# APRIL-ZJU/Gaussian-LIC

Measured on AMD Instinct MI355X. Metric: rendered views/sec (fwd+bwd) at 1080p, 2M Gaussians, higher is better.
Workload: dtype f32; 1 GPU; BASELINE config 3: 2000000 Gaussians (random scene, seed 0), 1920x1080, SH degree 3, render fwd + 0.8*L1+0.2*(1-fused-SSIM) + bwd + sparse Adam per view (fused entry points: activations and loss inside the kernels); learning rates x0.01 (stationary synthetic scene); map rows kept in Morton order by the library (bit-identical results; `insertion_order` beside it with --extras); mode=train, parallelism=single, math=strict, map_order=morton, binning=atomic (auto)

## Files before the change

gaussian-lic_amd/_lib.py:

```python
import ctypes
import os

import torch

_HERE = os.path.dirname(os.path.abspath(__file__))
LIB_PATH = os.environ.get("GSLIC_HIP_LIB") or os.path.join(_HERE, "libgslic_hip.so")

ALLOC_FN = ctypes.CFUNCTYPE(ctypes.c_void_p, ctypes.c_void_p, ctypes.c_size_t)


class RasterParams(ctypes.Structure):
    _fields_ = [("P", ctypes.c_int32), ("D", ctypes.c_int32), ("M", ctypes.c_int32), ("width", ctypes.c_int32),
                ("height", ctypes.c_int32), ("tan_fovx", ctypes.c_float), ("tan_fovy", ctypes.c_float),
                ("limx_neg", ctypes.c_float), ("limx_pos", ctypes.c_float), ("limy_neg", ctypes.c_float),
                ("limy_pos", ctypes.c_float), ("scale_modifier", ctypes.c_float), ("prefiltered", ctypes.c_int32),
                ("debug", ctypes.c_int32), ("no_color", ctypes.c_int32), ("raw_params", ctypes.c_int32), ("tie_rank", ctypes.c_void_p)]


class AdamGroup(ctypes.Structure):
    _fields_ = [("param", ctypes.c_void_p), ("grad", ctypes.c_void_p), ("exp_avg", ctypes.c_void_p),
                ("exp_avg_sq", ctypes.c_void_p), ("lr", ctypes.c_float), ("M", ctypes.c_uint32)]


class AdamFused(ctypes.Structure):
    _fields_ = [("param", ctypes.c_void_p * 6), ("exp_avg", ctypes.c_void_p * 6), ("exp_avg_sq", ctypes.c_void_p * 6),
                ("lr", ctypes.c_float * 6), ("b1", ctypes.c_float), ("b2", ctypes.c_float), ("eps", ctypes.c_float), ("visible_out", ctypes.c_void_p)]


EXPORTS = [
    "gslic_rasterize_forward", "gslic_rasterize_backward", "gslic_rasterize_backward_adam", "gslic_rasterize_backward_camera", "gslic_adam_update", "gslic_adam_update_groups",
    "gslic_fusedssim_forward", "gslic_fusedssim_backward", "gslic_knn_mean_dist2", "gslic_abi_version",
    "gslic_last_error", "gslic_geom_bytes", "gslic_img_bytes", "gslic_binning_bytes", "gslic_sample_bytes",
    "gslic_profile_enable", "gslic_profile_reset", "gslic_profile_collect", "gslic_profile_num_kernels",
    "gslic_profile_kernel_name", "gslic_profile_get", "gslic_debug_export", "gslic_extend_select", "gslic_extend_emit", "gslic_loss_partials_count", "gslic_l1_ssim_loss_forward", "gslic_l1_ssim_loss_forward_backward",
    "gslic_l1_ssim_loss_backward", "gslic_set_math_mode", "gslic_set_binning_mode", "gslic_rasterize_forward_capacity", "gslic_rasterize_backward_rgb",
    "gslic_rasterize_backward_rgb_rows", "gslic_sh_grad_from_rgb", "gslic_sh_grad_from_rgb_adam", "gslic_rasterize_backward_rgb_payload",
    "gslic_sh_grad_from_rgb_adam_all", "gslic_get_binning_path", "gslic_scratch_round_up",
    "gslic_rasterize_forward_depth", "gslic_rasterize_backward_depth",
    "gslic_rasterize_forward_depth_capacity", "gslic_rasterize_backward_depth_adam", "gslic_depth_l1_loss_partials_count",
    "gslic_depth_l1_loss_forward_backward", "gslic_img_bytes_depth", "gslic_binning_bytes_depth", "gslic_sample_bytes_depth",
    "gslic_rasterize_backward_depth_camera",
]

_lib = None


class GslicError(RuntimeError):
    pass


def lib():
    global _lib
    if _lib is not None:
        return _lib
    if not os.path.exists(LIB_PATH):
        raise GslicError(f"{LIB_PATH} is missing: run `python gaussian-lic_amd/build.py` (hipcc, gfx950). "
                         "There is no CPU fallback.")
    L = ctypes.CDLL(LIB_PATH, mode=ctypes.RTLD_GLOBAL)
    vp, i32, f32, u32 = ctypes.c_void_p, ctypes.c_int32, ctypes.c_float, ctypes.c_uint32
    L.gslic_last_error.restype = ctypes.c_char_p
    L.gslic_profile_kernel_name.restype = ctypes.c_char_p
    L.gslic_profile_kernel_name.argtypes = [i32]
    L.gslic_profile_get.argtypes = [i32, ctypes.POINTER(ctypes.c_double), ctypes.POINTER(ctypes.c_int64)]
    for n in ("gslic_geom_bytes", "gslic_img_bytes", "gslic_binning_bytes", "gslic_sample_bytes", "gslic_img_bytes_depth", "gslic_binning_bytes_depth",
              "gslic_sample_bytes_depth"):
        getattr(L, n).restype = ctypes.c_size_t
    L.gslic_geom_bytes.argtypes = [i32]
    L.gslic_img_bytes.argtypes = [i32, i32]
    L.gslic_binning_bytes.argtypes = [i32, i32]
    L.gslic_sample_bytes.argtypes = [i32]
    L.gslic_img_bytes_depth.argtypes = [i32, i32]
    L.gslic_binning_bytes_depth.argtypes = [i32]
    L.gslic_sample_bytes_depth.argtypes = [i32]
    L.gslic_rasterize_forward_depth_capacity.argtypes = (
        [ctypes.POINTER(RasterParams)] + [vp, ctypes.c_size_t] * 4 + [vp] * 12 + [vp, vp, vp, vp] +
        [ctypes.POINTER(i32), ctypes.POINTER(i32), vp, vp])
    L.gslic_rasterize_backward_depth_adam.argtypes = (
        [ctypes.POINTER(RasterParams), i32, i32] + [vp] * 12 + [vp] * 4 + [vp, vp] + [vp] * 6 + [f32, ctypes.POINTER(AdamFused), vp])
    L.gslic_depth_l1_loss_partials_count.restype = ctypes.c_int64
    L.gslic_depth_l1_loss_partials_count.argtypes = [i32, i32]
    L.gslic_depth_l1_loss_forward_backward.argtypes = [i32, i32, f32, vp, vp, vp, vp, vp, vp]
    L.gslic_rasterize_forward.argtypes = (
        [ctypes.POINTER(RasterParams)] + [ALLOC_FN, vp] * 4 + [vp] * 12 + [vp, vp, vp] +
        [ctypes.POINTER(i32), ctypes.POINTER(i32), vp])
    L.gslic_rasterize_forward_capacity.argtypes = (
        [ctypes.POINTER(RasterParams)] + [vp, ctypes.c_size_t] * 4 + [vp] * 12 + [vp, vp, vp] +
        [ctypes.POINTER(i32), ctypes.POINTER(i32), vp, vp])
    L.gslic_rasterize_backward.argtypes = (
        [ctypes.POINTER(RasterParams), i32, i32] + [vp] * 12 + [vp] * 4 + [vp] + [vp] * 10 + [f32, vp])
    L.gslic_rasterize_forward_depth.argtypes = (
        [ctypes.POINTER(RasterParams)] + [ALLOC_FN, vp] * 4 + [vp] * 12 + [vp, vp, vp, vp] +
        [ctypes.POINTER(i32), ctypes.POINTER(i32), vp])
    L.gslic_rasterize_backward_depth.argtypes = (
        [ctypes.POINTER(RasterParams), i32, i32] + [vp] * 12 + [vp] * 4 + [vp, vp] + [vp] * 10 + [f32, vp])
    L.gslic_rasterize_backward_adam.argtypes = (
        [ctypes.POINTER(RasterParams), i32, i32] + [vp] * 12 + [vp] * 4 + [vp] + [vp] * 6 + [f32, ctypes.POINTER(AdamFused), vp])
    L.gslic_rasterize_backward_camera.argtypes = (
        [ctypes.POINTER(RasterParams), i32, i32] + [vp] * 12 + [vp] * 4 + [vp] + [vp] * 10 + [f32, vp, vp, vp, vp])
    L.gslic_rasterize_backward_depth_camera.argtypes = (
        [ctypes.POINTER(RasterParams), i32, i32] + [vp] * 12 + [vp] * 4 + [vp, vp] + [vp] * 10 + [f32, vp, vp, vp, vp])
    L.gslic_rasterize_backward_rgb.argtypes = (
        [ctypes.POINTER(RasterParams), i32, i32] + [vp] * 12 + [vp] * 4 + [vp] + [vp] * 5 + [f32, vp])
    L.gslic_rasterize_backward_rgb_rows.argtypes = (
        [ctypes.POINTER(RasterParams), i32, i32] + [vp] * 12 + [vp] * 4 + [vp] + [vp] * 5 + [f32, i32, i32, i32, vp])
    L.gslic_rasterize_backward_rgb_payload.argtypes = (
        [ctypes.POINTER(RasterParams), i32, i32] + [vp] * 12 + [vp] * 4 + [vp] + [vp] * 5 + [f32, vp, vp, vp])
    L.gslic_sh_grad_from_rgb_adam_all.argtypes = [i32, i32, i32, i32, vp, vp, vp, i32, vp, ctypes.c_int64, vp, ctypes.POINTER(AdamFused), vp, vp, vp, vp,
                                                  ctypes.c_int64, vp]
    L.gslic_sh_grad_from_rgb.argtypes = [i32, i32, i32, i32, vp, vp, vp, i32, vp, vp, ctypes.c_int64, vp]
    L.gslic_sh_grad_from_rgb_adam.argtypes = [i32, i32, i32, i32, vp, vp, vp, i32, vp, ctypes.POINTER(AdamFused), vp, vp, ctypes.c_int64, vp]
    L.gslic_adam_update.argtypes = [vp, vp, vp, vp, vp, f32, f32, f32, f32, u32, u32, vp]
    L.gslic_adam_update_groups.argtypes = [ctypes.POINTER(AdamGroup), i32, vp, f32, f32, f32, u32, vp]
    L.gslic_fusedssim_forward.argtypes = [i32, i32, i32, i32, f32, f32] + [vp] * 6 + [vp]
    L.gslic_fusedssim_backward.argtypes = [i32, i32, i32, i32, f32, f32] + [vp] * 7 + [vp]
    L.gslic_knn_mean_dist2.argtypes = [i32, vp, vp, ALLOC_FN, vp, vp]
    L.gslic_extend_select.argtypes = [i32, vp, vp, vp, vp, f32, f32, f32, f32, i32, i32, vp, ALLOC_FN, vp,
                                      ctypes.POINTER(vp), ctypes.POINTER(vp), ctypes.POINTER(i32), vp]
    L.gslic_extend_emit.argtypes = [i32, vp, vp, vp, vp, vp, f32, f32, i32, vp, vp, vp, vp, vp, vp, vp]
    L.gslic_debug_export.argtypes = [ctypes.POINTER(RasterParams), i32, i32] + [vp] * 4 + [vp] * 10 + [vp]
    L.gslic_loss_partials_count.restype = ctypes.c_int64
    L.gslic_loss_partials_count.argtypes = [i32, i32, i32, i32]
    L.gslic_l1_ssim_loss_forward.argtypes = [i32, i32, i32, i32, f32, f32] + [vp] * 7 + [vp]
    L.gslic_l1_ssim_loss_backward.argtypes = [i32, i32, i32, i32, f32] + [vp] * 6 + [vp]
    L.gslic_l1_ssim_loss_forward_backward.argtypes = [i32, i32, i32, i32, f32, f32, f32] + [vp] * 8 + [vp]
    L.gslic_set_math_mode.argtypes = [i32]
    L.gslic_set_binning_mode.argtypes = [i32]
    L.gslic_get_binning_path.argtypes = [ctypes.POINTER(u32), ctypes.POINTER(u32)]
    L.gslic_scratch_round_up.restype = ctypes.c_size_t
    L.gslic_scratch_round_up.argtypes = [ctypes.c_size_t]
    if L.gslic_abi_version() != 8:
        raise GslicError("libgslic_hip.so ABI version mismatch")
    _lib = L
    return L


def set_math_mode(strict):
    return bool(lib().gslic_set_math_mode(int(bool(strict))))


def set_binning_mode(mode):
    names = ("auto", "radix", "atomic")
    return names[lib().gslic_set_binning_mode(names.index(mode))]


def binning_path():
    a, n = ctypes.c_uint32(0), ctypes.c_uint32(0)
    path = lib().gslic_get_binning_path(ctypes.byref(a), ctypes.byref(n))
    return ("none", "radix", "atomic")[path], a.value, n.value


def check(rc):
    if rc != 0:
        raise GslicError(f"libgslic_hip error {rc}: {lib().gslic_last_error().decode()}")


def ptr(t):
    if t is None or t.numel() == 0:
        return None
    return ctypes.c_void_p(t.data_ptr())


def current_stream_ptr():
    return ctypes.c_void_p(torch.cuda.current_stream().cuda_stream)


class _AllocBox:
    __slots__ = ("device", "tensor", "__weakref__")

    def __init__(self, device):
        self.device = device
        self.tensor = torch.empty(0, dtype=torch.uint8, device=device)


class TensorAllocator:

    GRANULE = 32 << 20

    def __init__(self, device):
        box = self._box = _AllocBox(device)
        round_up = lib().gslic_scratch_round_up

        def _alloc(_ctx, nbytes):
            box.tensor = torch.empty(int(round_up(int(nbytes))), dtype=torch.uint8, device=box.device)
            return box.tensor.data_ptr()

        self.cb = ALLOC_FN(_alloc)

    @property
    def device(self):
        return self._box.device

    @property
    def tensor(self):
        return self._box.tensor


def profile_enable(on=True, only=None):
    L = lib()
    if not on:
        check(L.gslic_profile_enable(0))
        return
    if only is None:
        check(L.gslic_profile_enable(1))
        return
    names = [L.gslic_profile_kernel_name(i).decode() for i in range(L.gslic_profile_num_kernels())]
    mask = 0
    for n in only:
        mask |= 1 << names.index(n)
    check(L.gslic_profile_enable(mask if mask not in (0, 1) else (mask | (1 << 30))))


def profile_reset():
    check(lib().gslic_profile_reset())


def profile_collect():
    L = lib()
    check(L.gslic_profile_collect())
    out = {}
    for i in range(L.gslic_profile_num_kernels()):
        ms, n = ctypes.c_double(0), ctypes.c_int64(0)
        check(L.gslic_profile_get(i, ctypes.byref(ms), ctypes.byref(n)))
        if n.value:
            out[L.gslic_profile_kernel_name(i).decode()] = (ms.value, n.value)
    return out
# ... 1 lines not shown
```

gaussian-lic_amd/build.py:

```python
import os
import subprocess
import sys
from concurrent.futures import ThreadPoolExecutor

HERE = os.path.dirname(os.path.abspath(__file__))
CSRC = os.path.join(HERE, "csrc")
OBJ = os.path.join(CSRC, "build")
LIB = os.path.join(HERE, "libgslic_hip.so")
HIPCC = os.environ.get("HIPCC", "/opt/rocm/bin/hipcc")
ARCH = "gfx950"

SOURCES = {
    "api.hip": [],
    "scan.hip": [],
    "radix_sort.hip": [],
    "tile_bin.hip": [],
    "preprocess.hip": ["-ffp-contract=off"],
    "render.hip": ["-fno-slp-vectorize"],
    "render_bwd_scan.hip": ["-fno-slp-vectorize"],
    "preprocess_bwd.hip": [],
    "adam.hip": [],
    "ssim.hip": ["-ffp-contract=off"],
    "depth_loss.hip": [],
    "knn.hip": [],
    "extend.hip": ["-ffp-contract=off"],
}
COMMON = [f"--offload-arch={ARCH}", "-O3", "-std=c++17", "-fPIC", "-fno-fast-math", "-Wno-inline-asm",
          "-fhip-fp32-correctly-rounded-divide-sqrt", "-Wall", "-Wno-unused-function"]
HEADERS = ["gslic_common.h", "kernels.h", "render_fwd_body.inc", "preprocess_bwd_body.inc", os.path.join("..", "..", "include", "gslic_hip.h")]


def _newer(a, b):
    return (not os.path.exists(b)) or os.path.getmtime(a) > os.path.getmtime(b)


def build(force=False, verbose=False):
    global OBJ, LIB
    extra_all = os.environ.get("GSLIC_BUILD_EXTRA", "").split()
    if os.environ.get("GSLIC_BUILD_LIB"):
        LIB = os.path.abspath(os.environ["GSLIC_BUILD_LIB"])
        OBJ = os.path.join(CSRC, "build_" + os.path.splitext(os.path.basename(LIB))[0])
        force = True
    os.makedirs(OBJ, exist_ok=True)
    hdr_paths = [os.path.join(CSRC, h) for h in HEADERS] + [os.path.abspath(__file__)]
    jobs = []
    for src, extra in SOURCES.items():
        s = os.path.join(CSRC, src)
        o = os.path.join(OBJ, src.replace(".hip", ".o"))
        if force or _newer(s, o) or any(_newer(h, o) for h in hdr_paths):
            jobs.append((s, o, [HIPCC] + COMMON + extra + extra_all + ["-c", s, "-o", o]))

    def run(job):
        s, o, cmd = job
        if verbose:
            print(" ".join(cmd), flush=True)
        r = subprocess.run(cmd, capture_output=True, text=True)
        return s, r

    with ThreadPoolExecutor(max_workers=min(8, max(1, len(jobs)))) as ex:
        for s, r in ex.map(run, jobs):
            if r.returncode != 0:
                sys.stderr.write(r.stdout + r.stderr)
                raise RuntimeError(f"hipcc failed on {s}")
            if verbose and r.stderr.strip():
                sys.stderr.write(r.stderr)
    objs = [os.path.join(OBJ, s.replace(".hip", ".o")) for s in SOURCES]
    if force or jobs or not os.path.exists(LIB):
        cmd = [HIPCC, f"--offload-arch={ARCH}", "-shared", "-fPIC", "-o", LIB] + objs
        if verbose:
            print(" ".join(cmd), flush=True)
        r = subprocess.run(cmd, capture_output=True, text=True)
        if r.returncode != 0:
            sys.stderr.write(r.stdout + r.stderr)
            raise RuntimeError("link of libgslic_hip.so failed")
    return LIB


if __name__ == "__main__":
    print(build(force="--force" in sys.argv, verbose="--verbose" in sys.argv))
```

gaussian-lic_amd/csrc/api.hip:

```cpp
#include "gslic_common.h"
#include "kernels.h"
#include <atomic>
#include <chrono>
#include <mutex>

#include <stdarg.h>
#include <stdio.h>
#include <stdlib.h>
#include <string.h>
#include <vector>

namespace gslic {

static thread_local char g_err[512] = "";
int set_error(int code, const char* fmt, ...)
{
    va_list ap;
    va_start(ap, fmt);
    vsnprintf(g_err, sizeof(g_err), fmt, ap);
    va_end(ap);
    return code;
}

bool g_prof_on = false;
int g_strict_math = [] {
    const char* s = getenv("GSLIC_STRICT_MATH");
    if (s) return atoi(s) != 0 ? 1 : 0;
    const char* f = getenv("GSLIC_FAST_MATH");
    return (f && atoi(f) != 0) ? 0 : 1;
}();
static uint32_t g_prof_mask = 0xffffffffu;
static bool g_prof_cur_on = false;
static const char* const k_names[K_COUNT] = {
    "preprocess", "scan_reduce", "scan_spine", "scan_apply", "keybuild", "sort_hist", "sort_scatter", "finalize_lists",
    "bucket_count", "render_fwd", "render_bwd", "preprocess_bwd", "adam", "ssim_fwd", "ssim_bwd", "knn_minmax", "knn_morton",
    "knn_boxes", "knn_search", "debug_export", "extend", "dsort_hist", "dsort_scatter", "sh_grad_from_rgb", "tile_lsort", "tile_hist", "tile_bin", "tile_scan", "tile_lsort_long", "depth_loss"};
uint32_t g_lds_pad[K_COUNT] = {0};
static const bool g_lds_pad_parsed = [] {
    const char* e = getenv("GSLIC_LDS_PAD");
    while (e && *e) {
        const char* eq = strchr(e, '=');
        if (!eq) break;
        for (int k = 0; k < K_COUNT; k++)
            if (strlen(k_names[k]) == (size_t)(eq - e) && strncmp(k_names[k], e, (size_t)(eq - e)) == 0) g_lds_pad[k] = (uint32_t)atoi(eq + 1);
        const char* c = strchr(eq, ',');
        e = c ? c + 1 : nullptr;
    }
    return true;
}();
struct ProfRec { int id; hipEvent_t a, b; };
static std::vector<ProfRec> g_pending;
static std::vector<hipEvent_t> g_pool;
static double g_total_ms[K_COUNT];
static int64_t g_launches[K_COUNT];
static hipEvent_t g_cur = nullptr;

static hipEvent_t ev_get()
{
    if (!g_pool.empty()) { hipEvent_t e = g_pool.back(); g_pool.pop_back(); return e; }
    hipEvent_t e = nullptr;
    (void)hipEventCreate(&e);
    return e;
}
void prof_begin(int id, hipStream_t s)
{
    g_prof_cur_on = (g_prof_mask >> id) & 1u;
    if (!g_prof_cur_on) return;
    g_cur = ev_get();
    (void)hipEventRecord(g_cur, s);
}
void prof_end(int id, hipStream_t s)
{
    if (!g_prof_cur_on) return;
    hipEvent_t b = ev_get();
    (void)hipEventRecord(b, s);
    g_pending.push_back({id, g_cur, b});
    g_cur = nullptr;
}

GeomState GeomState::carve(const void* base, size_t P, size_t* bytes)
{
    Carver c(base);
    GeomState g;
    g.rec = c.take<float4>(GS_REC_F4 * P);
    g.tiles_touched = c.take<uint32_t>(P);
    g.cam_scratch = c.take<float>(128 * ((P + 255) / 256) + 64);
    g.point_offsets = c.take<uint32_t>(P);
    g.gauss_start = c.take<uint32_t>(P);
    g.flags = c.take<uint32_t>(64);
    g.scan_state = c.take<char>(scan_state_bytes(P));
    g.zero_bytes = 64 * sizeof(uint32_t) + scan_state_bytes(P);
    if (bytes) *bytes = c.used(base) + 256;
    return g;
}
ImageState ImageState::carve(const void* base, size_t T, size_t* bytes, bool depth)
{
    Carver c(base);
    ImageState g;
    g.ranges = c.take<uint2>(T);
    g.bucket_offsets = c.take<uint32_t>(T);
    g.max_contrib = c.take<uint32_t>(T);
    g.pix_final = c.take<float4>(T * GS_TILE_PIX);
    g.pix_depth = depth ? c.take<float>(T * GS_TILE_PIX) : nullptr;
    if (bytes) *bytes = c.used(base) + 256;
    return g;
}
BinningState BinningState::carve(const void* base, size_t R, int end_bit, bool no_color, size_t* bytes, bool depth)
{
    Carver c(base);
    BinningState g;
    g.plan = sort_plan(R, end_bit);
    for (int i = 0; i < 2; i++) {
        g.tile_keys[i] = c.take<uint32_t>(R);
        g.slots[i] = c.take<uint32_t>(R);
        g.gauss[i] = c.take<uint32_t>(R);
    }
    g.sort_scratch = c.take<char>(sort_scratch_bytes(g.plan));
    g.partials = no_color ? nullptr : c.take<float>((size_t)GS_PROW * R);
    g.dead = no_color ? nullptr : c.take<uint8_t>(R);
    uint32_t* const ls = no_color ? c.take<uint32_t>(4 * R) : reinterpret_cast<uint32_t*>(g.partials);
    for (int i = 0; i < 4; i++) g.lsort[i] = ls + (size_t)i * R;
    g.partials_z = depth ? c.take<float>(R) : nullptr;
    if (bytes) *bytes = c.used(base) + 256;
    return g;
}
SampleState SampleState::carve(const void* base, size_t B, size_t* bytes, bool depth)
{
    Carver c(base);
    SampleState g;
    g.bucket_to_tile = c.take<uint32_t>(B);
    g.ckpt = c.take<float4>(B * GS_TILE_PIX);
    g.hit = c.take<uint64_t>(B * GS_TILE_PIX);
    g.ckpt_depth = depth ? c.take<float>(B * GS_TILE_PIX) : nullptr;
    if (bytes) *bytes = c.used(base) + 256;
    return g;
}

struct Mailbox {
    volatile uint32_t* host = nullptr;
    uint32_t* dev = nullptr;
    uint32_t seq = 0;
};
static constexpr int kMaxDevices = 16;
struct MailboxSet {
    Mailbox box[kMaxDevices];
    ~MailboxSet()
    {
        for (auto& m : box)
            if (m.host) (void)hipHostFree(const_cast<uint32_t*>(m.host));
    }
};
static thread_local MailboxSet t_mbox;
static uint32_t* g_status_word[kMaxDevices];
uint32_t* device_status_word()
{
    int dev = 0;
    if (hipGetDevice(&dev) != hipSuccess || dev < 0 || dev >= kMaxDevices) return nullptr;
    uint32_t* w = __atomic_load_n(&g_status_word[dev], __ATOMIC_ACQUIRE);
    if (w) return w;
    void* p = nullptr;
    if (hipMalloc(&p, 256) != hipSuccess || !p) { (void)hipGetLastError(); return nullptr; }
    (void)hipMemset(p, 0, 256);
    uint32_t* expected = nullptr;
    if (!__atomic_compare_exchange_n(&g_status_word[dev], &expected, static_cast<uint32_t*>(p), false, __ATOMIC_ACQ_REL, __ATOMIC_ACQUIRE)) {
        (void)hipFree(p);
        return expected;
    }
    return static_cast<uint32_t*>(p);
}
__global__ void publish_kernel(const uint32_t* __restrict__ v0, const uint32_t* __restrict__ v1, const uint32_t* __restrict__ v2, uint32_t* status,
                               uint32_t* box, uint32_t seq)
{
    const uint32_t st = status ? atomicExch(status, 0u) : 0u;
    __hip_atomic_store(box + 0, v0 ? *v0 : 0u, __ATOMIC_RELAXED, __HIP_MEMORY_SCOPE_SYSTEM);
// ... 328 lines not shown
        t_last_path = use_bin ? GSLIC_BINNING_PATH_ATOMIC : GSLIC_BINNING_PATH_RADIX;
        t_last_sample[0] = t_last_sample[1] = 0u;
        const int pp = bin.plan.passes & 1;
        KeybuildArgs ka;
        ka.P = P; ka.gx = gx; ka.gy = gy; ka.rec = geom.rec; ka.order = nullptr; ka.offsets = geom.point_offsets;
        ka.gauss_start = geom.gauss_start; ka.cap = R; ka.status = geom.flags;
        ka.tile_keys = bin.tile_keys[0];
        ka.gauss = use_bin ? bin.gauss[pp] : bin.gauss[0];
        ka.depth = use_bin ? bin.slots[pp] : bin.lsort[0];
        GS_TRY(launch_keybuild(ka, s));
        DEBUG_SYNC(prm, s);
        TileDepthSortArgs ts;
        ts.T = T; ts.ranges = img.ranges; ts.tie_rank = prm->tie_rank; ts.status = geom.flags; ts.long_tiles = img.bucket_offsets;
        ts.gauss_out = bin.gauss[pp ^ 1]; ts.slot_out = bin.slots[pp ^ 1];
        if (use_bin) {
            TileBinArgs tb;
            tb.T = T; tb.n_cap = R; tb.n_dev = R_dev; tb.tile = ka.tile_keys; tb.gid = ka.gauss; tb.depth = ka.depth; tb.tie_rank = prm->tie_rank;
            tb.ranges = img.ranges; tb.binned = bin.binned(); tb.dead = bin.dead; tb.status = geom.flags;
            tb.bucket_offsets = no_color ? nullptr : img.bucket_offsets; tb.max_contrib = img.max_contrib;
            ts.long_tiles = reinterpret_cast<uint32_t*>(bin.sort_scratch);
            GS_TRY(launch_tile_bin(tb, s));
            DEBUG_SYNC(prm, s);
            ts.binned = bin.binned(); ts.depth = nullptr; ts.gauss_in = nullptr; ts.slot_in = nullptr;
            ts.key_a = bin.tile_keys[0]; ts.key_b = bin.tile_keys[1]; ts.idx_a = bin.gauss[pp]; ts.idx_b = bin.slots[pp];
        } else {
            SortBuffers sb;
            for (int i = 0; i < 2; i++) { sb.keys[i] = bin.tile_keys[i]; sb.v0[i] = bin.slots[i]; sb.v1[i] = bin.gauss[i]; sb.v2[i] = bin.lsort[i]; }
            sb.v0_identity = true;
            GS_TRY(radix_sort_u32(sb, bin.plan, bin.sort_scratch, (onesweep_mask() & 2) != 0, K_SORT_HIST, K_SORT_SCATTER, s, R_dev, geom.flags + GS_FLAG_FAULT));
            DEBUG_SYNC(prm, s);
            GS_TRY(launch_finalize_ranges(R, R_dev, bin.tile_keys[pp], img.ranges, bin.dead, s));
            DEBUG_SYNC(prm, s);
            ts.binned = nullptr; ts.depth = bin.lsort[pp]; ts.gauss_in = bin.gauss[pp]; ts.slot_in = bin.slots[pp];
            ts.key_a = bin.lsort[pp ^ 1]; ts.key_b = bin.tile_keys[pp ^ 1]; ts.idx_a = bin.lsort[2]; ts.idx_b = bin.lsort[3];
        }
        GS_TRY(launch_tile_depth_sort(ts, s));
        DEBUG_SYNC(prm, s);
    }

    SampleState smp;
    memset(&smp, 0, sizeof(smp));
    uint32_t B = 0;
    if (!no_color) {
        if (!use_bin) GS_TRY(launch_bucket_scan(T, img.ranges, img.bucket_offsets, img.max_contrib, s));
        if (cap) {
            B = capacity_for(cap->sample_bytes, [&](uint32_t b) { size_t n; SampleState::carve(nullptr, (size_t)b, &n, depth); return n; });
        } else {
            uint32_t bin_sample[2] = {0, 0};
            GS_TRY(fetch_counts(img.bucket_offsets + (T - 1), nullptr, hostbuf, s, geom.flags + GS_FLAG_FAULT,
                                use_bin ? geom.flags + GS_FLAG_BIN_ATOMICS : nullptr, bin_sample));
            if (hostbuf[1] & 2u) return set_error(GSLIC_ERR_HIP, "a sort look-back / chained-scan wait timed out (device preempted?): the forward was abandoned");
            B = hostbuf[0];
            binning_feedback(prm->tie_rank != nullptr, use_bin, bin_sample[0], bin_sample[1]);
        }
        size_t smp_bytes;
        SampleState::carve(nullptr, (size_t)B, &smp_bytes, depth);
        char* smp_base = cap ? cap->sample : sample_alloc(sample_ctx, smp_bytes);
        if (!smp_base) return set_error(GSLIC_ERR_ALLOC, "sample allocator returned NULL for %zu bytes", smp_bytes);
        smp = SampleState::carve(align256(smp_base), (size_t)B, nullptr, depth);
    }

    RenderFwdArgs ra;
    ra.W = prm->width; ra.H = prm->height; ra.gx = gx; ra.gy = gy; ra.no_color = prm->no_color;
    ra.ranges = img.ranges; ra.point_list = bin.point_list(); ra.rec = geom.rec; ra.bucket_offsets = img.bucket_offsets;
    ra.bucket_to_tile = smp.bucket_to_tile; ra.ckpt = smp.ckpt; ra.hit = smp.hit; ra.pix_final = img.pix_final; ra.max_contrib = img.max_contrib;
    ra.out_color = out_color; ra.out_final_T = out_final_T; ra.capB = B; ra.status = geom.flags; ra.tail4_from = T;
    ra.out_depth = depth ? out_depth : nullptr; ra.ckpt_depth = smp.ckpt_depth; ra.pix_depth = img.pix_depth;
    GS_TRY(launch_render_fwd(ra, s));
    note_depth(geom.flags, depth);
    DEBUG_SYNC(prm, s);
    if (cap) {
        hipLaunchKernelGGL(forward_status_kernel, dim3(1), dim3(1), 0, s, (const uint32_t*)(geom.point_offsets + (P - 1)),
                           no_color ? (const uint32_t*)nullptr : (const uint32_t*)(img.bucket_offsets + (T - 1)), geom.flags, geom.flags + GS_FLAG_FAULT,
                           cap->status_out);
        GS_HIP(hipGetLastError());
    }

    *num_rendered = (int32_t)R;
    *num_buckets = (int32_t)B;
    return GSLIC_OK;
}

extern "C" {
int gslic_set_binning_mode(int32_t mode)
{
    if (mode < 0 || mode > 2) return g_binning_mode.load(std::memory_order_relaxed);
    const int old = g_binning_mode.exchange(mode, std::memory_order_relaxed);
    g_binning_epoch.fetch_add(1u, std::memory_order_release);
    return old;
}
int gslic_get_binning_path(uint32_t* sampled_atomics, uint32_t* sampled_instances)
{
    if (sampled_atomics) *sampled_atomics = t_last_sample[0];
    if (sampled_instances) *sampled_instances = t_last_sample[1];
    return t_last_path;
}
size_t gslic_scratch_round_up(size_t n)
{
    if (n <= (size_t(1) << 20)) return n;
    size_t g = size_t(32) << 20;
    if (n > (size_t(64) << 20)) {
        size_t p = 1;
        while ((p << 1) <= n && (p << 1) != 0) p <<= 1;
        const size_t half = p >> 1, cap = size_t(256) << 20;
        g = half > cap ? cap : (half > g ? half : g);
    }
    return (n + g - 1) / g * g;
}
int gslic_rasterize_forward(const gslic_raster_params* prm, gslic_alloc_fn geom_alloc, void* geom_ctx, gslic_alloc_fn binning_alloc,
                            void* binning_ctx, gslic_alloc_fn img_alloc, void* img_ctx, gslic_alloc_fn sample_alloc,
                            void* sample_ctx, const float* background, const float* means3D, const float* dc, const float* shs,
                            const float* colors_precomp, const float* opacities, const float* scales, const float* rotations,
                            const float* cov3D_precomp, const float* viewmatrix, const float* projmatrix, const float* cam_pos,
                            float* out_color, float* out_final_T, int32_t* radii, int32_t* num_rendered, int32_t* num_buckets,
                            void* stream)
{
    return rasterize_forward_impl(prm, geom_alloc, geom_ctx, binning_alloc, binning_ctx, img_alloc, img_ctx, sample_alloc, sample_ctx, nullptr,
                                  background, means3D, dc, shs, colors_precomp, opacities, scales, rotations, cov3D_precomp, viewmatrix, projmatrix,
                                  cam_pos, out_color, out_final_T, radii, num_rendered, num_buckets, stream);
}

int gslic_rasterize_forward_depth(const gslic_raster_params* prm, gslic_alloc_fn geom_alloc, void* geom_ctx, gslic_alloc_fn binning_alloc,
                                  void* binning_ctx, gslic_alloc_fn img_alloc, void* img_ctx, gslic_alloc_fn sample_alloc,
                                  void* sample_ctx, const float* background, const float* means3D, const float* dc, const float* shs,
                                  const float* colors_precomp, const float* opacities, const float* scales, const float* rotations,
                                  const float* cov3D_precomp, const float* viewmatrix, const float* projmatrix, const float* cam_pos,
                                  float* out_color, float* out_final_T, float* out_depth, int32_t* radii, int32_t* num_rendered,
                                  int32_t* num_buckets, void* stream)
{
    return rasterize_forward_impl(prm, geom_alloc, geom_ctx, binning_alloc, binning_ctx, img_alloc, img_ctx, sample_alloc, sample_ctx, nullptr,
                                  background, means3D, dc, shs, colors_precomp, opacities, scales, rotations, cov3D_precomp, viewmatrix, projmatrix,
                                  cam_pos, out_color, out_final_T, radii, num_rendered, num_buckets, stream, out_depth, true);
}

int gslic_rasterize_forward_capacity(const gslic_raster_params* prm, char* geom_buffer, size_t geom_bytes, char* binning_buffer,
                                     size_t binning_bytes, char* img_buffer, size_t img_bytes, char* sample_buffer, size_t sample_bytes,
                                     const float* background, const float* means3D, const float* dc, const float* shs,
                                     const float* colors_precomp, const float* opacities, const float* scales, const float* rotations,
                                     const float* cov3D_precomp, const float* viewmatrix, const float* projmatrix, const float* cam_pos,
                                     float* out_color, float* out_final_T, int32_t* radii, int32_t* capacity_R, int32_t* capacity_B,
                                     uint32_t* status, void* stream)
{
    ForwardCapacity cap{geom_buffer, binning_buffer, img_buffer, sample_buffer, geom_bytes, binning_bytes, img_bytes, sample_bytes, status};
    return rasterize_forward_impl(prm, nullptr, nullptr, nullptr, nullptr, nullptr, nullptr, nullptr, nullptr, &cap, background, means3D, dc, shs,
                                  colors_precomp, opacities, scales, rotations, cov3D_precomp, viewmatrix, projmatrix, cam_pos, out_color,
                                  out_final_T, radii, capacity_R, capacity_B, stream);
}

int gslic_rasterize_forward_depth_capacity(const gslic_raster_params* prm, char* geom_buffer, size_t geom_bytes, char* binning_buffer,
                                           size_t binning_bytes, char* img_buffer, size_t img_bytes, char* sample_buffer, size_t sample_bytes,
                                           const float* background, const float* means3D, const float* dc, const float* shs,
                                           const float* colors_precomp, const float* opacities, const float* scales, const float* rotations,
                                           const float* cov3D_precomp, const float* viewmatrix, const float* projmatrix, const float* cam_pos,
                                           float* out_color, float* out_final_T, float* out_depth, int32_t* radii, int32_t* capacity_R,
                                           int32_t* capacity_B, uint32_t* status, void* stream)
{
    ForwardCapacity cap{geom_buffer, binning_buffer, img_buffer, sample_buffer, geom_bytes, binning_bytes, img_bytes, sample_bytes, status};
    return rasterize_forward_impl(prm, nullptr, nullptr, nullptr, nullptr, nullptr, nullptr, nullptr, nullptr, &cap, background, means3D, dc, shs,
                                  colors_precomp, opacities, scales, rotations, cov3D_precomp, viewmatrix, projmatrix, cam_pos, out_color,
                                  out_final_T, radii, capacity_R, capacity_B, stream, out_depth, true);
}

static int rasterize_backward_impl(const gslic_raster_params* prm, int32_t R, int32_t B, const float* background, const float* means3D,
                             const float* dc, const float* shs, const float* colors_precomp, const float* scales,
                             const float* rotations, const float* cov3D_precomp, const float* viewmatrix, const float* projmatrix,
                             const float* cam_pos, const int32_t* radii, char* geom_buffer, char* binning_buffer, char* img_buffer,
                             char* sample_buffer, const float* dL_dpix, float* dL_dmean2D, float* dL_dconic, float* dL_dopacity,
                             float* dL_dcolor, float* dL_dmean3D, float* dL_dcov3D, float* dL_ddc, float* dL_dsh, float* dL_dscale,
                             float* dL_drot, float lambda_erank, const gslic_adam_fused* adam, float* const dL_dcam[3], void* stream,
                             float* dL_drgb = nullptr, int32_t row_begin = 0, int32_t row_end = -1, bool skip_blend = false, uint8_t* vis_out = nullptr,
                             float* campos_out = nullptr, const float* dL_ddepth = nullptr)
{
    (void)background; (void)dc;
    GS_TRY(check_params(prm));
    const int P = prm->P;
    if (P == 0) return GSLIC_OK;
    if (colors_precomp || cov3D_precomp)
        return set_error(GSLIC_ERR_UNSUPPORTED, "colors_precomp / cov3D_precomp are not supported");
    if (prm->no_color) return set_error(GSLIC_ERR_INVALID_ARG, "backward of a no_color forward is undefined (no checkpoints were stored)");
    if (R < 0 || B < 0) return set_error(GSLIC_ERR_INVALID_ARG, "negative R / B");
    if (!means3D || !scales || !rotations || !viewmatrix || !projmatrix || !cam_pos || !radii || !geom_buffer || !binning_buffer ||
        !img_buffer || !sample_buffer || !dL_dpix || (prm->M > 0 && !shs))
        return set_error(GSLIC_ERR_INVALID_ARG, "required tensor pointer is NULL");
    if (!adam && !dL_drgb && (!dL_dopacity || !dL_dmean3D || !dL_ddc || !dL_dscale || !dL_drot || (prm->M > 0 && !dL_dsh)))
        return set_error(GSLIC_ERR_INVALID_ARG, "required gradient output pointer is NULL");
    if (dL_drgb && (adam || dL_ddc || dL_dsh || !dL_dopacity || !dL_dmean3D || !dL_dscale || !dL_drot))
        return set_error(GSLIC_ERR_INVALID_ARG, "dL_drgb mode: dL_ddc / dL_dsh / adam must be NULL, the four other parameter gradients are required");
    if (adam) {
        if (!prm->raw_params) return set_error(GSLIC_ERR_INVALID_ARG, "fused Adam needs raw_params = 1 (it updates the raw parameters)");
        for (int g = 0; g < 6; g++) {
            if (g == 2 && prm->M == 0) continue;
            if (!adam->param[g] || !adam->exp_avg[g] || !adam->exp_avg_sq[g]) return set_error(GSLIC_ERR_INVALID_ARG, "fused Adam: group %d has a NULL pointer", g);
        }
        if (adam->param[0] != means3D || adam->param[4] != scales || adam->param[5] != rotations || (prm->M > 0 && adam->param[2] != shs))
            return set_error(GSLIC_ERR_INVALID_ARG, "fused Adam: param[] must alias the tensors passed as means3D / shs / scales / rotations");
    }
    {
        const int re = row_end < 0 ? P : row_end;
        if (row_begin < 0 || re > P || row_begin > re || (row_begin & 63))
            return set_error(GSLIC_ERR_INVALID_ARG, "row range [%d, %d) of %d Gaussians (row_begin must be a multiple of 64)", row_begin, re, P);
    }
    hipStream_t s = (hipStream_t)stream;
    int gx, gy;
    const int T = tile_grid(prm->width, prm->height, gx, gy);
    const bool depth = dL_ddepth != nullptr;
    GeomState geom = GeomState::carve(align256(geom_buffer), (size_t)P, nullptr);
    if (depth) {
        int known = known_depth(geom.flags);
        if (known < 0) {
            uint32_t depth_flag = 0u;
            GS_HIP(hipMemcpyAsync(&depth_flag, geom.flags + GS_FLAG_DEPTH, sizeof(uint32_t), hipMemcpyDeviceToHost, s));
            GS_HIP(hipStreamSynchronize(s));
            known = depth_flag == 1u ? 1 : 0;
        }
        if (known != 1)
            return set_error(GSLIC_ERR_INVALID_ARG, "depth backward: these buffers come from a forward that rendered no depth (use gslic_rasterize_forward_depth)");
    }
    ImageState img = ImageState::carve(align256(img_buffer), (size_t)T, nullptr, depth);
    BinningState bin = BinningState::carve(align256(binning_buffer), (size_t)R, sort_end_bit(T), false, nullptr, depth);
    SampleState smp = SampleState::carve(align256(sample_buffer), (size_t)B, nullptr, depth);

    RenderBwdArgs rb;
    rb.W = prm->width; rb.H = prm->height; rb.gx = gx; rb.B = B;
    rb.ranges = img.ranges; rb.point_list = bin.point_list(); rb.inst_slot = bin.inst_slot(); rb.rec = geom.rec;
    rb.bucket_offsets = img.bucket_offsets; rb.bucket_to_tile = smp.bucket_to_tile; rb.ckpt = smp.ckpt; rb.hit = smp.hit; rb.pix_final = img.pix_final;
    rb.max_contrib = img.max_contrib; rb.dL_dpix = dL_dpix; rb.partials = bin.partials; rb.dead = bin.dead; rb.status = geom.flags; rb.T = T;
    rb.dL_ddepth = dL_ddepth; rb.ckpt_depth = smp.ckpt_depth; rb.pix_depth = img.pix_depth; rb.partials_z = bin.partials_z;
    if (!skip_blend) GS_TRY(launch_render_bwd(rb, s));
    DEBUG_SYNC(prm, s);

    PreprocessBwdArgs pb;
    pb.P = P; pb.D = prm->D; pb.M = prm->M; pb.W = prm->width; pb.H = prm->height; pb.raw = prm->raw_params;
    pb.row_begin = row_begin; pb.row_end = row_end < 0 ? P : row_end;
    pb.focal_y = prm->height / (2.0f * prm->tan_fovy);
    pb.focal_x = prm->width / (2.0f * prm->tan_fovx);
    pb.limx_neg = prm->limx_neg; pb.limx_pos = prm->limx_pos; pb.limy_neg = prm->limy_neg; pb.limy_pos = prm->limy_pos;
    pb.scale_modifier = prm->scale_modifier; pb.lambda_erank = lambda_erank;
    pb.means = means3D; pb.scales = scales; pb.rots = rotations; pb.dc = dc; pb.shs = shs; pb.view = viewmatrix; pb.proj = projmatrix;
    pb.campos = cam_pos; pb.radii = radii; pb.rec = geom.rec; pb.tiles_touched = geom.tiles_touched; pb.gauss_start = geom.gauss_start; pb.partials = bin.partials; pb.dead = bin.dead;
    pb.dL_dmean2D = dL_dmean2D; pb.dL_dconic = dL_dconic; pb.dL_dopacity = dL_dopacity; pb.dL_dcolor = dL_dcolor;
    pb.dL_dmean3D = dL_dmean3D; pb.dL_dcov3D = dL_dcov3D; pb.dL_ddc = dL_ddc; pb.dL_dsh = dL_dsh; pb.dL_dscale = dL_dscale;
    pb.dL_drot = dL_drot; pb.dL_drgb = dL_drgb;
    memset(&pb.adam, 0, sizeof(pb.adam));
    if (adam) {
        for (int g = 0; g < 6; g++) { pb.adam.p[g] = adam->param[g]; pb.adam.m[g] = adam->exp_avg[g]; pb.adam.v[g] = adam->exp_avg_sq[g]; pb.adam.lr[g] = adam->lr[g]; }
        pb.adam.b1 = adam->b1; pb.adam.b2 = adam->b2; pb.adam.eps = adam->eps; pb.adam.on = 1;
    }
    pb.status = geom.flags;
    pb.cam_partials = nullptr; pb.cam_out = nullptr;
    pb.partials_z = depth ? bin.partials_z : nullptr;
    pb.vis_out = vis_out; pb.campos_out = campos_out;
    if (dL_dcam) {
        pb.cam_partials = geom.cam_scratch;
        pb.cam_out = geom.cam_scratch + 128 * (((size_t)P + 255) / 256);
    }
    GS_TRY(launch_preprocess_bwd(pb, s));
    if (dL_dcam) {
        GS_HIP(hipMemcpyAsync(dL_dcam[0], pb.cam_out, 16 * sizeof(float), hipMemcpyDeviceToDevice, s));
        GS_HIP(hipMemcpyAsync(dL_dcam[1], pb.cam_out + 16, 16 * sizeof(float), hipMemcpyDeviceToDevice, s));
        GS_HIP(hipMemcpyAsync(dL_dcam[2], pb.cam_out + 32, 3 * sizeof(float), hipMemcpyDeviceToDevice, s));
    }
    DEBUG_SYNC(prm, s);
    return GSLIC_OK;
}

int gslic_rasterize_backward(const gslic_raster_params* prm, int32_t R, int32_t B, const float* background, const float* means3D,
                             const float* dc, const float* shs, const float* colors_precomp, const float* scales,
                             const float* rotations, const float* cov3D_precomp, const float* viewmatrix, const float* projmatrix,
                             const float* cam_pos, const int32_t* radii, char* geom_buffer, char* binning_buffer, char* img_buffer,
                             char* sample_buffer, const float* dL_dpix, float* dL_dmean2D, float* dL_dconic, float* dL_dopacity,
                             float* dL_dcolor, float* dL_dmean3D, float* dL_dcov3D, float* dL_ddc, float* dL_dsh, float* dL_dscale,
                             float* dL_drot, float lambda_erank, void* stream)
{
    return rasterize_backward_impl(prm, R, B, background, means3D, dc, shs, colors_precomp, scales, rotations, cov3D_precomp, viewmatrix,
                                   projmatrix, cam_pos, radii, geom_buffer, binning_buffer, img_buffer, sample_buffer, dL_dpix, dL_dmean2D,
                                   dL_dconic, dL_dopacity, dL_dcolor, dL_dmean3D, dL_dcov3D, dL_ddc, dL_dsh, dL_dscale, dL_drot,
                                   lambda_erank, nullptr, nullptr, stream);
}

int gslic_rasterize_backward_depth(const gslic_raster_params* prm, int32_t R, int32_t B, const float* background, const float* means3D,
                                   const float* dc, const float* shs, const float* colors_precomp, const float* scales,
                                   const float* rotations, const float* cov3D_precomp, const float* viewmatrix, const float* projmatrix,
                                   const float* cam_pos, const int32_t* radii, char* geom_buffer, char* binning_buffer, char* img_buffer,
                                   char* sample_buffer, const float* dL_dpix, const float* dL_ddepth, float* dL_dmean2D, float* dL_dconic,
                                   float* dL_dopacity, float* dL_dcolor, float* dL_dmean3D, float* dL_dcov3D, float* dL_ddc, float* dL_dsh,
                                   float* dL_dscale, float* dL_drot, float lambda_erank, void* stream)
{
    GS_TRY(check_params(prm));
    if (prm->P == 0) return GSLIC_OK;
    if (prm->no_color) return set_error(GSLIC_ERR_INVALID_ARG, "depth backward: no_color = 1 (no depth forward renders without colour)");
    if (!dL_ddepth) return set_error(GSLIC_ERR_INVALID_ARG, "depth backward: dL_ddepth is NULL (gslic_rasterize_backward is the colour-only backward)");
    return rasterize_backward_impl(prm, R, B, background, means3D, dc, shs, colors_precomp, scales, rotations, cov3D_precomp, viewmatrix,
                                   projmatrix, cam_pos, radii, geom_buffer, binning_buffer, img_buffer, sample_buffer, dL_dpix, dL_dmean2D,
                                   dL_dconic, dL_dopacity, dL_dcolor, dL_dmean3D, dL_dcov3D, dL_ddc, dL_dsh, dL_dscale, dL_drot,
                                   lambda_erank, nullptr, nullptr, stream, nullptr, 0, -1, false, nullptr, nullptr, dL_ddepth);
}

int gslic_rasterize_backward_rgb(const gslic_raster_params* prm, int32_t R, int32_t B, const float* background, const float* means3D,
                                 const float* dc, const float* shs, const float* colors_precomp, const float* scales,
                                 const float* rotations, const float* cov3D_precomp, const float* viewmatrix, const float* projmatrix,
                                 const float* cam_pos, const int32_t* radii, char* geom_buffer, char* binning_buffer, char* img_buffer,
                                 char* sample_buffer, const float* dL_dpix, float* dL_dopacity, float* dL_dmean3D, float* dL_drgb,
                                 float* dL_dscale, float* dL_drot, float lambda_erank, void* stream)
{
    if (!dL_drgb) return set_error(GSLIC_ERR_INVALID_ARG, "gslic_rasterize_backward_rgb: dL_drgb is NULL");
    return rasterize_backward_impl(prm, R, B, background, means3D, dc, shs, colors_precomp, scales, rotations, cov3D_precomp, viewmatrix,
                                   projmatrix, cam_pos, radii, geom_buffer, binning_buffer, img_buffer, sample_buffer, dL_dpix, nullptr,
                                   nullptr, dL_dopacity, nullptr, dL_dmean3D, nullptr, nullptr, nullptr, dL_dscale, dL_drot, lambda_erank,
                                   nullptr, nullptr, stream, dL_drgb);
}

int gslic_rasterize_backward_rgb_payload(const gslic_raster_params* prm, int32_t R, int32_t B, const float* background, const float* means3D,
                                         const float* dc, const float* shs, const float* colors_precomp, const float* scales,
                                         const float* rotations, const float* cov3D_precomp, const float* viewmatrix, const float* projmatrix,
                                         const float* cam_pos, const int32_t* radii, char* geom_buffer, char* binning_buffer, char* img_buffer,
                                         char* sample_buffer, const float* dL_dpix, float* dL_dopacity, float* dL_dmean3D, float* dL_drgb,
                                         float* dL_dscale, float* dL_drot, float lambda_erank, uint8_t* vis_out, float* campos_out, void* stream)
{
    if (!dL_drgb) return set_error(GSLIC_ERR_INVALID_ARG, "gslic_rasterize_backward_rgb_payload: dL_drgb is NULL");
    return rasterize_backward_impl(prm, R, B, background, means3D, dc, shs, colors_precomp, scales, rotations, cov3D_precomp, viewmatrix,
                                   projmatrix, cam_pos, radii, geom_buffer, binning_buffer, img_buffer, sample_buffer, dL_dpix, nullptr,
                                   nullptr, dL_dopacity, nullptr, dL_dmean3D, nullptr, nullptr, nullptr, dL_dscale, dL_drot, lambda_erank,
                                   nullptr, nullptr, stream, dL_drgb, 0, -1, false, vis_out, campos_out);
}

int gslic_rasterize_backward_rgb_rows(const gslic_raster_params* prm, int32_t R, int32_t B, const float* background, const float* means3D,
                                      const float* dc, const float* shs, const float* colors_precomp, const float* scales,
                                      const float* rotations, const float* cov3D_precomp, const float* viewmatrix, const float* projmatrix,
                                      const float* cam_pos, const int32_t* radii, char* geom_buffer, char* binning_buffer, char* img_buffer,
                                      char* sample_buffer, const float* dL_dpix, float* dL_dopacity, float* dL_dmean3D, float* dL_drgb,
                                      float* dL_dscale, float* dL_drot, float lambda_erank, int32_t row_begin, int32_t row_end, int32_t skip_blend,
                                      void* stream)
{
    if (!dL_drgb) return set_error(GSLIC_ERR_INVALID_ARG, "gslic_rasterize_backward_rgb_rows: dL_drgb is NULL");
// ... 396 lines not shown
```

gaussian-lic_amd/csrc/gslic_common.h:

```cpp
#pragma once
#include <hip/hip_runtime.h>
#include <stdint.h>
#include <stddef.h>
#include "../../include/gslic_hip.h"

#define GS_TILE 16
#define GS_TILE_PIX 256
#ifndef GS_REC_F4
#define GS_REC_F4 3
#endif
#ifndef GS_PROW
#define GS_PROW 9
#endif
#define GS_BUCKET 64
#define GS_WAVE 64

namespace gslic {

int set_error(int code, const char* fmt, ...);
#define GS_HIP(call)                                                                                       \
    do {                                                                                                   \
        hipError_t e__ = (call);                                                                           \
        if (e__ != hipSuccess)                                                                             \
            return ::gslic::set_error(GSLIC_ERR_HIP, "%s: %s (%s:%d)", #call, hipGetErrorString(e__),      \
                                      __FILE__, __LINE__);                                                 \
    } while (0)
#define GS_TRY(expr)                                                                                       \
    do {                                                                                                   \
        int rc__ = (expr);                                                                                 \
        if (rc__ != GSLIC_OK) return rc__;                                                                 \
    } while (0)

enum KernelId {
    K_PREPROCESS = 0,
    K_SCAN_REDUCE,
    K_SCAN_SPINE,
    K_SCAN_APPLY,
    K_KEYBUILD,
    K_SORT_HIST,
    K_SORT_SCATTER,
    K_FINALIZE_LISTS,
    K_BUCKET_COUNT,
    K_RENDER_FWD,
    K_RENDER_BWD,
    K_PREPROCESS_BWD,
    K_ADAM,
    K_SSIM_FWD,
    K_SSIM_BWD,
    K_KNN_MINMAX,
    K_KNN_MORTON,
    K_KNN_BOXES,
    K_KNN_SEARCH,
    K_DEBUG_EXPORT,
    K_EXTEND,
    K_DSORT_HIST,
    K_DSORT_SCATTER,
    K_SH_REBUILD,
    K_TILE_LSORT,
    K_TILE_HIST,
    K_TILE_BIN,
    K_TILE_SCAN,
    K_TILE_LSORT_LONG,
    K_DEPTH_LOSS,
    K_COUNT
};
void prof_begin(int id, hipStream_t s);
void prof_end(int id, hipStream_t s);
extern bool g_prof_on;
#define GS_FLAG_HITBITS 4
#define GS_FLAG_DEPTH 12
#define GS_FLAG_BIN_ATOMICS 10
#define GS_FLAG_LONG 9
#define GS_FLAG_FAULT 8
extern int g_strict_math;

extern uint32_t g_lds_pad[];
#define GS_LAUNCH(id, kernel, grid, block, shmem, stream, ...)                                             \
    do {                                                                                                   \
        if (::gslic::g_prof_on) ::gslic::prof_begin(id, stream);                                           \
        hipLaunchKernelGGL(kernel, grid, block, (shmem) + ::gslic::g_lds_pad[id], stream, __VA_ARGS__);    \
        if (::gslic::g_prof_on) ::gslic::prof_end(id, stream);                                             \
        GS_HIP(hipGetLastError());                                                                         \
    } while (0)

struct Carver {
    uintptr_t p;
    explicit Carver(const void* base) : p(reinterpret_cast<uintptr_t>(base)) {}
    template <typename T>
    T* take(size_t count)
    {
        p = (p + 255) & ~uintptr_t(255);
        T* r = reinterpret_cast<T*>(p);
        p += count * sizeof(T);
        return r;
    }
    size_t used(const void* base) const { return p - reinterpret_cast<uintptr_t>(base); }
};

static inline int div_up(int a, int b) { return (a + b - 1) / b; }
static inline size_t div_up_sz(size_t a, size_t b) { return (a + b - 1) / b; }

static inline uint32_t higher_msb(uint32_t n)
{
    uint32_t bits = 0;
    while (bits < 32 && (n >> bits) != 0) ++bits;
    return bits == 0 ? 1 : bits;
}

uint32_t* device_status_word();

size_t scan_temp_elems(size_t n);
int scan_u32(const uint32_t* in, uint32_t* out, size_t n, bool exclusive, uint32_t* temp, hipStream_t s);
size_t scan_state_bytes(size_t n);
int scan_u32_chained(const uint32_t* in, const uint32_t* gather, uint32_t* out, size_t n, bool exclusive, void* zeroed_state, hipStream_t s,
                     uint32_t* fault = nullptr);

#define GS_SORT_ITEMS 16
#define GS_SORT_BLOCK 256
#define GS_SORT_TILE (GS_SORT_ITEMS * GS_SORT_BLOCK)
struct SortPlan {
    size_t n;
    int passes;
    size_t nblk;
    size_t hist_elems;
};
SortPlan sort_plan(size_t n, int end_bit);
struct SortBuffers {
    uint32_t* keys[2];
    uint32_t* v0[2];
    uint32_t* v1[2];
    uint32_t* v2[2];
    bool v0_identity;
};
size_t sort_scratch_bytes(const SortPlan& plan);
int radix_sort_u32(const SortBuffers& b, const SortPlan& plan, void* scratch, bool onesweep, int id_hist, int id_scatter, hipStream_t s,
                   const uint32_t* n_dev = nullptr, uint32_t* fault = nullptr);
struct TileBinArgs {
    int T;
    uint32_t n_cap;
    const uint32_t* n_dev;
    const uint32_t* tile;
    const uint32_t* gid;
    const uint32_t* depth;
    const uint32_t* tie_rank;
    uint2* ranges;
    uint4* binned;
    uint8_t* dead;
    uint32_t* bucket_offsets;
    uint32_t* max_contrib;
    uint32_t* status;
};
static constexpr int GS_TILE_BIN_MAX_T = 36864;
int launch_tile_bin(const TileBinArgs& a, hipStream_t s);
bool tile_bin_lds_ok(int T);

struct TileDepthSortArgs {
    int T;
    const uint2* ranges;
    const uint4* binned;
    const uint32_t* depth;
    uint32_t* key_a;
    uint32_t* key_b;
    uint32_t* idx_a;
    uint32_t* idx_b;
    const uint32_t* gauss_in;
    const uint32_t* slot_in;
    uint32_t* gauss_out;
    uint32_t* slot_out;
    const uint32_t* tie_rank;
    uint32_t* status;
    uint32_t* long_tiles;
};
int launch_tile_depth_sort(const TileDepthSortArgs& a, hipStream_t s);

struct GeomState {
    float4* rec;
    uint32_t* tiles_touched;
    float* cam_scratch;
    uint32_t* point_offsets;
    uint32_t* gauss_start;
    uint32_t* flags;
    void* scan_state;
    size_t zero_bytes;
    static GeomState carve(const void* base, size_t P, size_t* bytes);
};
struct ImageState {
    uint2* ranges;
    uint32_t* bucket_offsets;
    uint32_t* max_contrib;
    float4* pix_final;
    float* pix_depth;
    static ImageState carve(const void* base, size_t T, size_t* bytes, bool depth = false);
};
struct BinningState {
    uint32_t* tile_keys[2];
    uint32_t* slots[2];
    uint32_t* gauss[2];
    uint32_t* lsort[4];
    void* sort_scratch;
    float* partials;
    uint8_t* dead;
    float* partials_z;
    SortPlan plan;
    uint32_t* point_list() const { return gauss[(plan.passes & 1) ^ 1]; }
    uint32_t* inst_slot() const { return slots[(plan.passes & 1) ^ 1]; }
    uint4* binned() const { return reinterpret_cast<uint4*>(lsort[0]); }
    static BinningState carve(const void* base, size_t R, int end_bit, bool no_color, size_t* bytes, bool depth = false);
};
struct SampleState {
    uint32_t* bucket_to_tile;
    float4* ckpt;
    uint64_t* hit;
    float* ckpt_depth;
    static SampleState carve(const void* base, size_t B, size_t* bytes, bool depth = false);
};

}

#if defined(__HIPCC__)
namespace gslic {

__device__ __forceinline__ int lane_id() { return __builtin_amdgcn_mbcnt_hi(~0u, __builtin_amdgcn_mbcnt_lo(~0u, 0u)); }

__device__ __forceinline__ int tile_pix_x(int i) { return ((i >> 6) & 1) * 8 + (i & 7); }
__device__ __forceinline__ int tile_pix_y(int i) { return (i >> 7) * 8 + ((i >> 3) & 7); }
__device__ __forceinline__ int tile_pix_index(int x, int y) { return ((y >> 3) * 2 + (x >> 3)) * 64 + (y & 7) * 8 + (x & 7); }


__device__ __forceinline__ uint32_t wave_inclusive_scan(uint32_t v)
{
    const int lane = lane_id();
#pragma unroll
    for (int d = 1; d < 64; d <<= 1) {
        uint32_t o = __shfl_up(v, d, 64);
        if (lane >= d) v += o;
    }
    return v;
}
__device__ __forceinline__ uint32_t block256_exclusive_prefix(uint32_t thread_sum, uint32_t& block_total, uint32_t* lds)
{
    const int lane = threadIdx.x & 63, wave = threadIdx.x >> 6;
    const uint32_t inc = wave_inclusive_scan(thread_sum);
    if (lane == 63) lds[wave] = inc;
    __syncthreads();
    uint32_t wave_base = 0, total = 0;
#pragma unroll
    for (int w = 0; w < 4; w++) {
        const uint32_t s = lds[w];
        if (w < wave) wave_base += s;
        total += s;
    }
    __syncthreads();
    block_total = total;
    return wave_base + inc - thread_sum;
}
__device__ __forceinline__ float readlane_f(float v, int l) { return __int_as_float(__builtin_amdgcn_readlane(__float_as_int(v), l)); }
__device__ __forceinline__ uint32_t readlane_u(uint32_t v, int l) { return (uint32_t)__builtin_amdgcn_readlane((int)v, l); }
#ifndef GSLIC_NT
#define GSLIC_NT 1
#endif
typedef float gs_v4f __attribute__((ext_vector_type(4)));
typedef float gs_v4f_u __attribute__((ext_vector_type(4), aligned(4)));
__device__ __forceinline__ float4 ld_stream(const float4* p)
{
#if GSLIC_NT
// ... 97 lines not shown
```

gaussian-lic_amd/csrc/kernels.h:

```cpp
#pragma once
#include "gslic_common.h"

namespace gslic {

struct PreprocessArgs {
    int P, D, M, W, H, gx, gy;
    float focal_x, focal_y;
    float limx_neg, limx_pos, limy_neg, limy_pos, scale_modifier;
    int prefiltered, no_color, raw;
    const float *means, *scales, *rots, *opac, *dc, *shs, *view, *proj, *campos;
    int32_t* radii;
    float4* rec;
    uint32_t* tiles_touched;
    uint32_t* depth_keys;
    uint2* ranges;
    uint32_t* flags;
};
int launch_preprocess(const PreprocessArgs& a, hipStream_t s);

struct KeybuildArgs {
    int P, gx, gy;
    const float4* rec;
    const uint32_t* order;
    const uint32_t* offsets;
// ... 5 lines not shown
    uint32_t* status;
};
int launch_keybuild(const KeybuildArgs& a, hipStream_t s);
int launch_finalize_ranges(uint32_t R, const uint32_t* R_dev, const uint32_t* sorted_tiles, uint2* ranges, uint8_t* dead, hipStream_t s);
int launch_bucket_scan(int T, const uint2* ranges, uint32_t* bucket_offsets, uint32_t* max_contrib , hipStream_t s);

struct RenderFwdArgs {
    int W, H, gx, gy, no_color;
    const uint2* ranges;
    const uint32_t* point_list;
    const float4* rec;
    const uint32_t* bucket_offsets;
    uint32_t* bucket_to_tile;
    float4* ckpt;
    uint64_t* hit;
    float4* pix_final;
    uint32_t* max_contrib;
    float* out_color;
    float* out_final_T;
    uint32_t capB;
    uint32_t* status;
    int tail4_from;
    float* out_depth;
    float* ckpt_depth;
    float* pix_depth;
};
int launch_render_fwd(const RenderFwdArgs& a, hipStream_t s);

struct RenderBwdArgs {
    int W, H, gx, B;
    const uint2* ranges;
    const uint32_t* point_list;
    const uint32_t* inst_slot;
    const float4* rec;
    const uint32_t* bucket_offsets;
    const uint32_t* bucket_to_tile;
    const float4* ckpt;
    const uint64_t* hit;
    const float4* pix_final;
    const uint32_t* max_contrib;
    const float* dL_dpix;
    float* partials;
    uint8_t* dead;
    const uint32_t* status;
    int T;
    int xcd_lg;
    int skip_if_bits;
    const float* dL_ddepth;
    const float* ckpt_depth;
    const float* pix_depth;
    float* partials_z;
};
int launch_render_bwd(const RenderBwdArgs& a, hipStream_t s);
int launch_render_bwd_scan(const RenderBwdArgs& b, unsigned grid, hipStream_t s);

struct AdamFusedArgs {
    float *p[6], *m[6], *v[6];
    float lr[6];
    float b1, b2, eps;
    int on;
};

struct PreprocessBwdArgs {
    int P, D, M, W, H, raw;
    int row_begin, row_end;
    float focal_x, focal_y;
    float limx_neg, limx_pos, limy_neg, limy_pos, scale_modifier, lambda_erank;
    const float *means, *scales, *rots, *dc, *shs, *view, *proj, *campos;
    const int32_t* radii;
    const float4* rec;
    const uint32_t* tiles_touched;
    const uint32_t* gauss_start;
    const float* partials;
    const uint8_t* dead;
    float *dL_dmean2D, *dL_dconic, *dL_dopacity, *dL_dcolor, *dL_dmean3D, *dL_dcov3D, *dL_ddc, *dL_dsh, *dL_dscale, *dL_drot;
    float* dL_drgb;
    AdamFusedArgs adam;
    const uint32_t* status;
    uint8_t* vis_out;
    float* campos_out;
    float* cam_partials;
    float* cam_out;
    const float* partials_z;
};
int launch_preprocess_bwd(const PreprocessBwdArgs& a, hipStream_t s);

struct ShGradFromRgbArgs {
    int P, D, M, n_views, input_is_ddc;
    size_t rgb_stride, campos_stride;
    const float *means3D, *campos_all, *rgb_all;
    float *dL_ddc, *dL_dsh;
    const uint8_t* visible;
    size_t vis_stride;
    uint8_t* vis_out;
    const float* g_small[4];
    AdamFusedArgs adam;
};
int launch_sh_grad_from_rgb(const ShGradFromRgbArgs& a, hipStream_t s);

}
```

gaussian-lic_amd/csrc/preprocess_bwd.hip:

```cpp
#include "gslic_common.h"
#include "kernels.h"
#include <stdlib.h>

namespace gslic {

#define SHC0 0.28209479177387814f
#define SHC1 0.4886025119029199f
__constant__ float b_SH_C2[5] = {1.0925484305920792f, -1.0925484305920792f, 0.31539156525252005f, -1.0925484305920792f,
                                 0.5462742152960396f};
__constant__ float b_SH_C3[7] = {-0.5900435899266435f, 2.890611442640554f, -0.4570457994644658f, 0.3731763325901154f,
                                 -0.4570457994644658f, 1.445305721320277f, -0.5900435899266435f};

__device__ __forceinline__ void sh_dir(float px, float py, float pz, const float* __restrict__ campos, float& dox, float& doy, float& doz, float& x,
                                       float& y, float& z)
{
#pragma clang fp contract(off)
    dox = px - campos[0]; doy = py - campos[1]; doz = pz - campos[2];
    const float len = sqrtf(dox * dox + doy * doy + doz * doz);
    x = dox / len; y = doy / len; z = doz / len;
}

__device__ __forceinline__ void sh_coefs(int D, float x, float y, float z, float (&c)[15])
{
#pragma clang fp contract(off)
#pragma unroll
    for (int k = 0; k < 15; k++) c[k] = 0.f;
    if (D > 0) {
        c[0] = -SHC1 * y; c[1] = SHC1 * z; c[2] = -SHC1 * x;
        if (D > 1) {
            const float xx = x * x, yy = y * y, zz = z * z, xy = x * y, yz = y * z, xz = x * z;
            c[3] = b_SH_C2[0] * xy; c[4] = b_SH_C2[1] * yz; c[5] = b_SH_C2[2] * (2.f * zz - xx - yy);
            c[6] = b_SH_C2[3] * xz; c[7] = b_SH_C2[4] * (xx - yy);
            if (D > 2) {
                c[8] = b_SH_C3[0] * y * (3.f * xx - yy); c[9] = b_SH_C3[1] * xy * z; c[10] = b_SH_C3[2] * y * (4.f * zz - xx - yy);
                c[11] = b_SH_C3[3] * z * (2.f * zz - 3.f * xx - 3.f * yy); c[12] = b_SH_C3[4] * x * (4.f * zz - xx - yy);
                c[13] = b_SH_C3[5] * z * (xx - yy); c[14] = b_SH_C3[6] * x * (xx - 3.f * yy);
            }
        }
    }
}

struct ShOut {
    float x, y, z, dR, dG, dB;
    bool on;
};

struct PartialSums { float mx, my, cx, cy, cw, op, r, g, b; };

__device__ __forceinline__ bool bwd_gather(const PreprocessBwdArgs& a, const int idx, const bool staged, PartialSums& ps);
template <bool CAM, bool DEFER_XYZ = false>
__device__ __forceinline__ void bwd_rest(const PreprocessBwdArgs& a, const int idx, const PartialSums& ps, const float* sh_row, const float* sk_row,
                                         ShOut& so, float* sg, float* cg);

template <int BS, bool DEFER_XYZ = false>
__device__ __forceinline__ void small_groups_sink(const AdamFusedArgs& A, float* const (&gout)[5], const float* lds_g, const uint8_t* lds_vis, int row0,
                                                  int rows)
{
    constexpr int NG = 5;
    constexpr int gid[NG] = {0, 1, 3, 4, 5};
    constexpr int wid[NG] = {3, 3, 1, 3, 4};
    constexpr int off[NG] = {0, 3 * BS, 6 * BS, 7 * BS, 10 * BS};
    const int t = threadIdx.x;
    if (rows == BS) {
        float4 g[NG], p[NG], m[NG], v[NG];
        bool on[NG], vis[NG][4];
#pragma unroll
        for (int k = 0; k < NG; k++) {
            on[k] = false;
            if (t < BS * wid[k] / 4) {
                g[k] = reinterpret_cast<const float4*>(lds_g + off[k])[t];
                if (gout[k]) reinterpret_cast<float4*>(gout[k] + (size_t)row0 * wid[k])[t] = g[k];
                if (A.on && !(DEFER_XYZ && k == 0)) {
                    const int e = 4 * t;
#pragma unroll
                    for (int c = 0; c < 4; c++) vis[k][c] = lds_vis[(e + c) / wid[k]];
                    on[k] = vis[k][0] | vis[k][1] | vis[k][2] | vis[k][3];
                }
            }
            if (on[k]) {
                const size_t base = (size_t)row0 * wid[k];
                p[k] = reinterpret_cast<const float4*>(A.p[gid[k]] + base)[t];
                m[k] = ld_stream(reinterpret_cast<const float4*>(A.m[gid[k]] + base) + t);
                v[k] = ld_stream(reinterpret_cast<const float4*>(A.v[gid[k]] + base) + t);
            }
        }
#pragma unroll
        for (int k = 0; k < NG; k++) {
            if (!on[k]) continue;
            const float lr = A.lr[gid[k]];
            if (vis[k][0]) adam_scalar(p[k].x, g[k].x, m[k].x, v[k].x, lr, A.b1, A.b2, A.eps);
            if (vis[k][1]) adam_scalar(p[k].y, g[k].y, m[k].y, v[k].y, lr, A.b1, A.b2, A.eps);
            if (vis[k][2]) adam_scalar(p[k].z, g[k].z, m[k].z, v[k].z, lr, A.b1, A.b2, A.eps);
            if (vis[k][3]) adam_scalar(p[k].w, g[k].w, m[k].w, v[k].w, lr, A.b1, A.b2, A.eps);
            const size_t base = (size_t)row0 * wid[k];
            st_stream(reinterpret_cast<float4*>(A.p[gid[k]] + base) + t, p[k]);
            st_stream(reinterpret_cast<float4*>(A.m[gid[k]] + base) + t, m[k]);
            st_stream(reinterpret_cast<float4*>(A.v[gid[k]] + base) + t, v[k]);
        }
    } else {
#pragma unroll
        for (int k = 0; k < NG; k++) {
            const size_t base = (size_t)row0 * wid[k];
            for (int i = t; i < rows * wid[k]; i += BS) {
                if (gout[k]) gout[k][base + i] = lds_g[off[k] + i];
                if (A.on && !(DEFER_XYZ && k == 0) && lds_vis[i / wid[k]])
                    adam_scalar(A.p[gid[k]][base + i], lds_g[off[k] + i], A.m[gid[k]][base + i], A.v[gid[k]][base + i], A.lr[gid[k]], A.b1, A.b2, A.eps);
            }
        }
    }
}

#ifndef GS_PBWD_U
#define GS_PBWD_U 4
#endif
#ifndef GS_SHT
#define GS_SHT 19
#endif
static constexpr int SHT = GS_SHT;

__device__ __forceinline__ int div3_small(int rem) { return (rem * 43) >> 7; }

template <int BS>
__device__ __forceinline__ void sh_columns_pass(const PreprocessBwdArgs& a, const float* __restrict__ tab, float* __restrict__ sk,
                                                const uint8_t* __restrict__ lds_vis, const int row0)
{
#pragma clang fp contract(off)
    constexpr int NE = BS * 45, NV = NE / 4, U = GS_PBWD_U;
    const AdamFusedArgs& A = a.adam;
    const size_t base = (size_t)row0 * 45;
    const float* __restrict__ P = a.shs + base;
    const bool store_g = a.dL_dsh != nullptr;
    for (int i0 = threadIdx.x; i0 < NV; i0 += BS * U) {
        float4 x[U], m[U], v[U];
        float2 nx[U];
        int r0[U], rem0[U];
        bool any[U], upd[U], vis[U][4];
#pragma unroll
        for (int u = 0; u < U; u++) {
            const int i = i0 + BS * u;
            any[u] = upd[u] = false;
            if (i < NV) {
                const int e = 4 * i;
                r0[u] = e / 45; rem0[u] = e - 45 * r0[u];
                const int r1 = (r0[u] + 1 < BS) ? r0[u] + 1 : r0[u];
                const bool v0 = lds_vis[r0[u]] != 0, v1 = lds_vis[r1] != 0;
#pragma unroll
                for (int c = 0; c < 4; c++) vis[u][c] = (rem0[u] + c < 45) ? v0 : v1;
                any[u] = v0 | v1;
                upd[u] = A.on & (vis[u][0] | vis[u][3]);
                x[u] = make_float4(0.f, 0.f, 0.f, 0.f); nx[u] = make_float2(0.f, 0.f);
                if (any[u]) {
                    x[u] = reinterpret_cast<const float4*>(P)[i];
                    if (e + 4 < NE) nx[u] = *reinterpret_cast<const float2*>(P + e + 4);
                }
                if (upd[u]) {
                    m[u] = ld_stream(reinterpret_cast<const float4*>(A.m[2] + base) + i);
                    v[u] = ld_stream(reinterpret_cast<const float4*>(A.v[2] + base) + i);
                }
            }
        }
#pragma unroll
        for (int u = 0; u < U; u++) {
            const int i = i0 + BS * u;
            if (i >= NV) continue;
            const float xe[6] = {x[u].x, x[u].y, x[u].z, x[u].w, nx[u].x, nx[u].y};
            float pr[6], g[4];
#pragma unroll
            for (int c = 0; c < 6; c++) {
                int r = r0[u], rem = rem0[u] + c;
                if (rem >= 45) { rem -= 45; r += 1; }
                if (r >= BS) r = BS - 1;
                const int k = div3_small(rem), ch = rem - 3 * k;
                const float d = tab[r * SHT + 15 + ch];
                pr[c] = xe[c] * d;
                if (c < 4) g[c] = tab[r * SHT + k] * d;
            }
            const int ch0 = rem0[u] - 3 * div3_small(rem0[u]);
            const int c0 = ch0 == 0 ? 0 : 3 - ch0;
            const float t0 = c0 == 0 ? pr[0] : (c0 == 1 ? pr[1] : pr[2]);
            const float t1 = c0 == 0 ? pr[1] : (c0 == 1 ? pr[2] : pr[3]);
            const float t2 = c0 == 0 ? pr[2] : (c0 == 1 ? pr[3] : pr[4]);
            const int f = (4 * i + c0) / 3;
            sk[f] = (t0 + t1) + t2;
            if (c0 == 0) sk[f + 1] = (pr[3] + pr[4]) + pr[5];
            const float4 g4 = make_float4(g[0], g[1], g[2], g[3]);
            if (store_g) reinterpret_cast<float4*>(a.dL_dsh + base)[i] = g4;
            if (upd[u]) {
                if (vis[u][0]) adam_scalar(x[u].x, g4.x, m[u].x, v[u].x, A.lr[2], A.b1, A.b2, A.eps);
                if (vis[u][1]) adam_scalar(x[u].y, g4.y, m[u].y, v[u].y, A.lr[2], A.b1, A.b2, A.eps);
                if (vis[u][2]) adam_scalar(x[u].z, g4.z, m[u].z, v[u].z, A.lr[2], A.b1, A.b2, A.eps);
                if (vis[u][3]) adam_scalar(x[u].w, g4.w, m[u].w, v[u].w, A.lr[2], A.b1, A.b2, A.eps);
                st_stream(reinterpret_cast<float4*>(A.p[2] + base) + i, x[u]);
                st_stream(reinterpret_cast<float4*>(A.m[2] + base) + i, m[u]);
                st_stream(reinterpret_cast<float4*>(A.v[2] + base) + i, v[u]);
            }
        }
    }
}

#ifndef GS_PBWD_STRICT_CHAIN
#define GS_PBWD_STRICT_CHAIN 0
#endif
#ifndef GS_PBWD_WPE
#define GS_PBWD_WPE 4
#endif
#define GS_PBWD_OCC __attribute__((amdgpu_waves_per_eu(GS_PBWD_WPE, GS_PBWD_WPE)))
template <bool LDS_SH, int BS, bool CAM>
__global__ __launch_bounds__(BS) GS_PBWD_OCC void preprocess_bwd_kernel(PreprocessBwdArgs a)
{
    constexpr bool DEFER_XYZ = false;
#include "preprocess_bwd_body.inc"
}
template <bool LDS_SH, int BS>
__global__ __launch_bounds__(BS) GS_PBWD_OCC void preprocess_bwd_defer_xyz_kernel(PreprocessBwdArgs a)
{
    constexpr bool CAM = false;
    constexpr bool DEFER_XYZ = true;
#include "preprocess_bwd_body.inc"
}

__device__ __forceinline__ bool bwd_gather(const PreprocessBwdArgs& a, const int idx, const bool staged, PartialSums& ps)
{
    ps.mx = ps.my = ps.cx = ps.cy = ps.cw = ps.op = ps.r = ps.g = ps.b = 0.f;
    const bool visible = a.radii[idx] > 0;

    if (!visible) {
        if (a.dL_dmean2D) { a.dL_dmean2D[3 * idx] = 0; a.dL_dmean2D[3 * idx + 1] = 0; a.dL_dmean2D[3 * idx + 2] = 0; }
        if (a.dL_dconic) reinterpret_cast<float4*>(a.dL_dconic)[idx] = make_float4(0, 0, 0, 0);
        if (a.dL_dcolor) { a.dL_dcolor[3 * idx] = 0; a.dL_dcolor[3 * idx + 1] = 0; a.dL_dcolor[3 * idx + 2] = 0; }
        if (a.dL_dcov3D)
            for (int k = 0; k < 6; k++) a.dL_dcov3D[6 * idx + k] = 0;
        if (staged) return false;
        if (a.dL_dopacity) a.dL_dopacity[idx] = 0;
        if (a.dL_dmean3D) { a.dL_dmean3D[3 * idx] = 0; a.dL_dmean3D[3 * idx + 1] = 0; a.dL_dmean3D[3 * idx + 2] = 0; }
        if (a.dL_ddc) { a.dL_ddc[3 * idx] = 0; a.dL_ddc[3 * idx + 1] = 0; a.dL_ddc[3 * idx + 2] = 0; }
        if (a.dL_drgb) { a.dL_drgb[3 * idx] = 0; a.dL_drgb[3 * idx + 1] = 0; a.dL_drgb[3 * idx + 2] = 0; }
        if (a.dL_dscale) { a.dL_dscale[3 * idx] = 0; a.dL_dscale[3 * idx + 1] = 0; a.dL_dscale[3 * idx + 2] = 0; }
        if (a.dL_drot) reinterpret_cast<float4*>(a.dL_drot)[idx] = make_float4(0, 0, 0, 0);
        return false;
    }

    float s_mx = 0, s_my = 0, s_cx = 0, s_cy = 0, s_cw = 0, s_op = 0, s_r = 0, s_g = 0, s_b = 0;
    {
        const uint32_t u0 = a.gauss_start[idx];
        const uint32_t u1 = u0 + a.tiles_touched[idx];
        constexpr int UP = 4;
        for (uint32_t u = u0; u < u1; u += UP) {
            uint32_t flags;
            __builtin_memcpy(&flags, a.dead + u, 4);
            bool live[UP];
#pragma unroll
            for (int j = 0; j < UP; j++) live[j] = (u + j < u1) & (((flags >> (8 * j)) & 0xffu) == 0u);
            gs_v4f_u q0[UP], q1[UP];
            float q2[UP];
#pragma unroll
            for (int j = 0; j < UP; j++) {
                if (live[j]) {
                    const float* p = a.partials + GS_PROW * (size_t)(u + j);
                    q0[j] = *reinterpret_cast<const gs_v4f_u*>(p);
                    q1[j] = *reinterpret_cast<const gs_v4f_u*>(p + 4);
                    q2[j] = p[8];
                }
            }
#pragma unroll
            for (int j = 0; j < UP; j++) {
                if (live[j]) {
                    s_mx += q0[j].x; s_my += q0[j].y; s_cx += q0[j].z; s_cy += q0[j].w;
                    s_cw += q1[j].x; s_op += q1[j].y; s_r += q1[j].z; s_g += q1[j].w;
                    s_b += q2[j];
                }
            }
        }
    }
    if (a.dL_dmean2D) { a.dL_dmean2D[3 * idx] = s_mx; a.dL_dmean2D[3 * idx + 1] = s_my; a.dL_dmean2D[3 * idx + 2] = 0; }
    if (a.dL_dconic) reinterpret_cast<float4*>(a.dL_dconic)[idx] = make_float4(s_cx, s_cy, 0.f, s_cw);
    if (a.dL_dcolor) { a.dL_dcolor[3 * idx] = s_r; a.dL_dcolor[3 * idx + 1] = s_g; a.dL_dcolor[3 * idx + 2] = s_b; }
    ps.mx = s_mx; ps.my = s_my; ps.cx = s_cx; ps.cy = s_cy; ps.cw = s_cw; ps.op = s_op; ps.r = s_r; ps.g = s_g; ps.b = s_b;
    return true;
}

template <bool CAM, bool DEFER_XYZ>
__device__ __forceinline__ void bwd_rest(const PreprocessBwdArgs& a, const int idx, const PartialSums& ps, const float* sh_row, const float* sk_row,
                                         ShOut& so, float* sg, float* cg)
{
#if GS_PBWD_STRICT_CHAIN
#pragma clang fp contract(off)
#endif
    const float s_mx = ps.mx, s_my = ps.my, s_cx = ps.cx, s_cy = ps.cy, s_cw = ps.cw, s_op = ps.op, s_r = ps.r, s_g = ps.g, s_b = ps.b;
    const float* __restrict__ V = a.view;
    const float* __restrict__ Pm = a.proj;
    const float mx3 = a.means[3 * idx], my3 = a.means[3 * idx + 1], mz3 = a.means[3 * idx + 2];

    float qr = a.rots[4 * idx], qx = a.rots[4 * idx + 1], qy = a.rots[4 * idx + 2], qz = a.rots[4 * idx + 3];
    const float4 qraw = make_float4(qr, qx, qy, qz);
    if (a.raw) {
        const float nrm = fmaxf(sqrtf(qr * qr + qx * qx + qy * qy + qz * qz), 1e-12f);
        qr = qr / nrm; qx = qx / nrm; qy = qy / nrm; qz = qz / nrm;
    }
    float Rm[3][3];
    Rm[0][0] = 1.f - 2.f * (qy * qy + qz * qz); Rm[0][1] = 2.f * (qx * qy - qr * qz); Rm[0][2] = 2.f * (qx * qz + qr * qy);
    Rm[1][0] = 2.f * (qx * qy + qr * qz); Rm[1][1] = 1.f - 2.f * (qx * qx + qz * qz); Rm[1][2] = 2.f * (qy * qz - qr * qx);
    Rm[2][0] = 2.f * (qx * qz - qr * qy); Rm[2][1] = 2.f * (qy * qz + qr * qx); Rm[2][2] = 1.f - 2.f * (qx * qx + qy * qy);
    float sc[3] = {a.scales[3 * idx], a.scales[3 * idx + 1], a.scales[3 * idx + 2]};
    if (a.raw) { sc[0] = expf(sc[0]); sc[1] = expf(sc[1]); sc[2] = expf(sc[2]); }
    const float s[3] = {a.scale_modifier * sc[0], a.scale_modifier * sc[1], a.scale_modifier * sc[2]};
    float Mk[3][3];
#pragma unroll
// ... 294 lines not shown
                                                           const float* __restrict__ V, const uint32_t* __restrict__ status, float* __restrict__ dL_dmean3D,
                                                           AdamFusedArgs A)
{
    if (status[2] != 0u) return;
    const int idx = row_begin + (int)(blockIdx.x * 256u + threadIdx.x);
    if (idx >= row_end || radii[idx] <= 0) return;
    depth_mean3d_row<ADAM>(idx, gauss_start, tiles_touched, dead, partials_z, V, dL_dmean3D, A);
}

__global__ __launch_bounds__(256) void depth_mean3d_cam_kernel(int row_begin, int row_end, const int32_t* __restrict__ radii,
                                                               const uint32_t* __restrict__ gauss_start, const uint32_t* __restrict__ tiles_touched,
                                                               const uint8_t* __restrict__ dead, const float* __restrict__ partials_z,
                                                               const float* __restrict__ V, const uint32_t* __restrict__ status, const float* __restrict__ means,
                                                               float* __restrict__ dL_dmean3D, float* __restrict__ cam_partials)
{
#pragma clang fp contract(off)
    if (status[2] != 0u) return;
    const int idx = row_begin + (int)(blockIdx.x * 256u + threadIdx.x);
    float c[4] = {0.f, 0.f, 0.f, 0.f};
    if (idx < row_end && radii[idx] > 0) {
        AdamFusedArgs none;
        none.on = 0;
        const float dz = depth_mean3d_row<false>(idx, gauss_start, tiles_touched, dead, partials_z, V, dL_dmean3D, none);
        c[0] = dz * means[3 * idx]; c[1] = dz * means[3 * idx + 1]; c[2] = dz * means[3 * idx + 2]; c[3] = dz;
    }
#pragma unroll
    for (int k = 0; k < 4; k++) {
        float v = c[k];
#pragma unroll
        for (int d = 32; d >= 1; d >>= 1) v += __shfl_xor(v, d, 64);
        c[k] = v;
    }
    if ((threadIdx.x & 63) == 0) {
        float* row = cam_partials + 32 * ((size_t)blockIdx.x * 4 + (threadIdx.x >> 6));
#pragma unroll
        for (int k = 0; k < 4; k++) row[27 + k] = c[k];
    }
}

__global__ __launch_bounds__(256) void cam_reduce_depth_kernel(size_t rows, const float* __restrict__ partials, const uint32_t* __restrict__ status,
                                                               float* __restrict__ out)
{
    __shared__ float red[256], redz[256];
    if (status[2] != 0u) return;
    const int k = blockIdx.x;
    const bool direct = k < 12 && (k % 3) == 2;
    const int kz = 27 + k / 3;
    float s = 0.f, sz = 0.f;
    for (size_t r = threadIdx.x; r < rows; r += 256) {
        s += partials[32 * r + k];
        if (direct) sz += partials[32 * r + kz];
    }
    red[threadIdx.x] = s;
    redz[threadIdx.x] = sz;
    __syncthreads();
    for (int d = 128; d >= 1; d >>= 1) {
        if ((int)threadIdx.x < d) {
            red[threadIdx.x] += red[threadIdx.x + d];
            redz[threadIdx.x] += redz[threadIdx.x + d];
        }
        __syncthreads();
    }
    if (threadIdx.x == 0) {
        int dst;
        if (k < 12) dst = 4 * (k / 3) + (k % 3);
        else if (k < 24) { const int kk = k - 12; const int r = kk % 3; dst = 16 + 4 * (kk / 3) + (r == 2 ? 3 : r); }
        else dst = 32 + (k - 24);
        out[dst] = direct ? red[0] + redz[0] : red[0];
    }
}

int launch_preprocess_bwd(const PreprocessBwdArgs& a, hipStream_t s)
{
    if (a.partials_z && (a.dL_drgb || !a.dL_dmean3D))
        return set_error(GSLIC_ERR_INVALID_ARG, "depth backward: no dL_drgb output, and dL_dmean3D is required");
    if (a.partials_z && a.cam_partials && (a.adam.on || a.row_begin != 0))
        return set_error(GSLIC_ERR_INVALID_ARG, "depth camera backward: no fused Adam and no row range");
    const bool defer = a.partials_z && a.adam.on;
    const bool cam = a.cam_partials != nullptr;
    const int nrows = a.row_end - a.row_begin;
    if (nrows <= 0) return GSLIC_OK;
    if (cam) GS_HIP(hipMemsetAsync(a.cam_out, 0, 35 * sizeof(float), s));
    if (a.M == 15 && a.shs && (a.dL_dsh || a.adam.on || a.dL_drgb)) {
        if (cam) GS_LAUNCH(K_PREPROCESS_BWD, (preprocess_bwd_kernel<true, 64, true>), dim3(div_up(nrows, 64)), dim3(64), 0, s, a);
        else if (defer) GS_LAUNCH(K_PREPROCESS_BWD, (preprocess_bwd_defer_xyz_kernel<true, 64>), dim3(div_up(nrows, 64)), dim3(64), 0, s, a);
        else GS_LAUNCH(K_PREPROCESS_BWD, (preprocess_bwd_kernel<true, 64, false>), dim3(div_up(nrows, 64)), dim3(64), 0, s, a);
    } else {
        if (cam) GS_LAUNCH(K_PREPROCESS_BWD, (preprocess_bwd_kernel<false, 256, true>), dim3(div_up(nrows, 256)), dim3(256), 0, s, a);
        else if (defer) GS_LAUNCH(K_PREPROCESS_BWD, (preprocess_bwd_defer_xyz_kernel<false, 256>), dim3(div_up(nrows, 256)), dim3(256), 0, s, a);
        else GS_LAUNCH(K_PREPROCESS_BWD, (preprocess_bwd_kernel<false, 256, false>), dim3(div_up(nrows, 256)), dim3(256), 0, s, a);
    }
    if (defer)
        GS_LAUNCH(K_PREPROCESS_BWD, depth_mean3d_kernel<true>, dim3(div_up(nrows, 256)), dim3(256), 0, s, a.row_begin, a.row_end, a.radii, a.gauss_start,
                  a.tiles_touched, a.dead, a.partials_z, a.view, a.status, a.dL_dmean3D, a.adam);
    else if (a.partials_z && cam)
        GS_LAUNCH(K_PREPROCESS_BWD, depth_mean3d_cam_kernel, dim3(div_up(nrows, 256)), dim3(256), 0, s, a.row_begin, a.row_end, a.radii, a.gauss_start,
                  a.tiles_touched, a.dead, a.partials_z, a.view, a.status, a.means, a.dL_dmean3D, a.cam_partials);
    else if (a.partials_z)
        GS_LAUNCH(K_PREPROCESS_BWD, depth_mean3d_kernel<false>, dim3(div_up(nrows, 256)), dim3(256), 0, s, a.row_begin, a.row_end, a.radii, a.gauss_start,
                  a.tiles_touched, a.dead, a.partials_z, a.view, a.status, a.dL_dmean3D, a.adam);
    if (cam) {
        const size_t rows = (a.M == 15 && a.shs && (a.dL_dsh || a.adam.on || a.dL_drgb)) ? (size_t)div_up(a.P, 64) : (size_t)div_up(a.P, 256) * 4;
        if (a.partials_z) GS_LAUNCH(K_PREPROCESS_BWD, cam_reduce_depth_kernel, dim3(27), dim3(256), 0, s, rows, (const float*)a.cam_partials, a.status, a.cam_out);
        else GS_LAUNCH(K_PREPROCESS_BWD, cam_reduce_kernel, dim3(27), dim3(256), 0, s, rows, (const float*)a.cam_partials, a.cam_out);
    }
    return GSLIC_OK;
}

static constexpr int SGR = 32;
template <bool ADAM>
__global__ __launch_bounds__(64) void sh_grad_from_rgb_kernel(ShGradFromRgbArgs a)
{
#pragma clang fp contract(off)
    __shared__ __attribute__((aligned(16))) float lds_rows[SGR * 48];
    const int t = threadIdx.x;
    const int row0 = blockIdx.x * SGR;
    const int idx = t < SGR ? row0 + t : a.P;
    const int rows = (a.P - row0) < SGR ? (a.P - row0) : SGR;
    float acc[45], adc[3] = {0.f, 0.f, 0.f};
#pragma unroll
    for (int k = 0; k < 45; k++) acc[k] = 0.f;
    if (idx < a.P) {
        const float px = a.means3D[3 * (size_t)idx], py = a.means3D[3 * (size_t)idx + 1], pz = a.means3D[3 * (size_t)idx + 2];
        for (int v = 0; v < a.n_views; v++) {
            const float* g = a.rgb_all + (size_t)v * a.rgb_stride + (size_t)idx * 3;
            float d[3] = {g[0], g[1], g[2]};
            if (d[0] == 0.f && d[1] == 0.f && d[2] == 0.f) continue;
            float dc_v[3];
            if (a.input_is_ddc) {
#pragma unroll
                for (int ch = 0; ch < 3; ch++) { dc_v[ch] = d[ch]; d[ch] = d[ch] * (1.0f / SHC0); }
            } else {
#pragma unroll
                for (int ch = 0; ch < 3; ch++) dc_v[ch] = SHC0 * d[ch];
            }
            float dox, doy, doz, x, y, z, c[15];
            sh_dir(px, py, pz, a.campos_all + (size_t)v * a.campos_stride, dox, doy, doz, x, y, z);
            sh_coefs(a.D, x, y, z, c);
#pragma unroll
            for (int ch = 0; ch < 3; ch++) adc[ch] = adc[ch] + dc_v[ch];
#pragma unroll
            for (int k = 0; k < 15; k++) {
#pragma unroll
                for (int ch = 0; ch < 3; ch++) {
                    const float prod = c[k] * d[ch];
                    acc[3 * k + ch] = acc[3 * k + ch] + prod;
                }
            }
        }
    }
    if (t < SGR) {
#pragma unroll
        for (int ch = 0; ch < 3; ch++) lds_rows[3 * t + ch] = adc[ch];
#pragma unroll
        for (int k = 0; k < 45; k++) lds_rows[3 * SGR + 45 * t + k] = acc[k];
    }
    __builtin_amdgcn_fence(__ATOMIC_RELEASE, "wavefront");
    __builtin_amdgcn_wave_barrier();
    if (a.dL_ddc)
        for (int i = t; i < rows * 3; i += 64) a.dL_ddc[(size_t)row0 * 3 + i] = lds_rows[i];
    if (a.dL_dsh) {
        if (a.M == 15) {
            for (int i = t; i < rows * 45; i += 64) a.dL_dsh[(size_t)row0 * 45 + i] = lds_rows[3 * SGR + i];
        } else if (a.M > 0 && idx < a.P) {
            for (int k = 0; k < 3 * a.M; k++) a.dL_dsh[(size_t)3 * a.M * idx + k] = k < 45 ? lds_rows[3 * SGR + 45 * t + k] : 0.f;
        }
    }
    if constexpr (ADAM) {
        __shared__ uint8_t lds_vis[64];
        uint8_t myvis = 0;
// ... 86 lines not shown
```

gaussian-lic_amd/csrc/preprocess_bwd_body.inc:

```
    __shared__ __attribute__((aligned(16))) float lds_tab[LDS_SH ? BS * SHT : 4];
    __shared__ float lds_sk[LDS_SH ? BS * 15 : 4];
    __shared__ uint8_t lds_vis[BS];
    float* const lds_g = lds_tab;
    if (a.status[2] != 0u) return;
    const int idx = a.row_begin + blockIdx.x * BS + threadIdx.x;
    const int M = a.M;
    const int row0 = a.row_begin + blockIdx.x * BS;
    const int rows = (a.row_end - row0) < BS ? (a.row_end - row0) : BS;
    ShOut so;
    so.x = so.y = so.z = so.dR = so.dG = so.dB = 0.f;
    so.on = false;
    float sg[14];
#pragma unroll
    for (int k = 0; k < 14; k++) sg[k] = 0.f;
    float cg[CAM ? 27 : 1];
    if constexpr (CAM) {
#pragma unroll
        for (int k = 0; k < 27; k++) cg[k] = 0.f;
    }
    PartialSums ps;
    bool visible = false;
    if (idx < a.row_end) visible = bwd_gather(a, idx, LDS_SH, ps);
    lds_vis[threadIdx.x] = visible ? 1 : 0;
    if (a.vis_out && idx < a.row_end) a.vis_out[idx] = visible ? 1 : 0;
    if (a.campos_out && blockIdx.x == 0 && threadIdx.x < 3) a.campos_out[threadIdx.x] = a.campos[threadIdx.x];
    if constexpr (LDS_SH) {
        float trow[18];
#pragma unroll
        for (int k = 0; k < 18; k++) trow[k] = 0.f;
        if (visible) {
            const uint32_t clamp_bits = __float_as_uint(a.rec[GS_REC_F4 * (size_t)idx + 2].z);
            float dox, doy, doz, x, y, z;
            sh_dir(a.means[3 * idx], a.means[3 * idx + 1], a.means[3 * idx + 2], a.campos, dox, doy, doz, x, y, z);
            float c[15];
            sh_coefs(a.D, x, y, z, c);
#pragma unroll
            for (int k = 0; k < 15; k++) trow[k] = c[k];
            trow[15] = (clamp_bits & 1u) ? 0.f : ps.r; trow[16] = (clamp_bits & 2u) ? 0.f : ps.g; trow[17] = (clamp_bits & 4u) ? 0.f : ps.b;
        }
#pragma unroll
        for (int k = 0; k < 18; k++) lds_tab[threadIdx.x * SHT + k] = trow[k];
        __syncthreads();
        const bool sh_sink = a.dL_dsh || a.adam.on;
        if (rows == BS) {
            sh_columns_pass<BS>(a, lds_tab, lds_sk, lds_vis, row0);
        } else {
            const size_t base = (size_t)row0 * 45;
            if ((int)threadIdx.x < rows) {
#pragma clang fp contract(off)
                const float* __restrict__ sh = a.shs + base + 45 * threadIdx.x;
                const float* __restrict__ tr = lds_tab + threadIdx.x * SHT;
#pragma unroll
                for (int k = 0; k < 15; k++) lds_sk[threadIdx.x * 15 + k] = (sh[3 * k] * tr[15] + sh[3 * k + 1] * tr[16]) + sh[3 * k + 2] * tr[17];
            }
            __syncthreads();
            const AdamFusedArgs& A = a.adam;
            if (sh_sink)
                for (int i = threadIdx.x; i < rows * 45; i += BS) {
                    const int r = i / 45, rem = i - 45 * r, k = rem / 3, ch = rem - 3 * k;
                    const float g = lds_tab[r * SHT + k] * lds_tab[r * SHT + 15 + ch];
                    if (a.dL_dsh) a.dL_dsh[base + i] = g;
                    if (A.on && lds_vis[r]) adam_scalar(A.p[2][base + i], g, A.m[2][base + i], A.v[2][base + i], A.lr[2], A.b1, A.b2, A.eps);
                }
        }
        __syncthreads();
        if (visible) bwd_rest<CAM, DEFER_XYZ>(a, idx, ps, nullptr, lds_sk + threadIdx.x * 15, so, sg, cg);
    } else {
        const float* sh_row = a.shs ? a.shs + (size_t)3 * M * idx : nullptr;
        if (visible) bwd_rest<CAM, DEFER_XYZ>(a, idx, ps, sh_row, nullptr, so, nullptr, cg);
    }
    if constexpr (CAM) {
#pragma unroll
        for (int k = 0; k < 27; k++) {
            float v = cg[k];
#pragma unroll
            for (int d = 32; d >= 1; d >>= 1) v += __shfl_xor(v, d, 64);
            cg[k] = v;
        }
        if ((threadIdx.x & 63) == 0) {
            float* row = a.cam_partials + 32 * ((size_t)blockIdx.x * (BS / 64) + (threadIdx.x >> 6));
#pragma unroll
            for (int k = 0; k < 27; k++) row[k] = cg[k];
        }
    }
    if constexpr (LDS_SH) {
        const int t = threadIdx.x;
        lds_g[3 * t] = sg[0]; lds_g[3 * t + 1] = sg[1]; lds_g[3 * t + 2] = sg[2];
        lds_g[3 * BS + 3 * t] = sg[3]; lds_g[3 * BS + 3 * t + 1] = sg[4]; lds_g[3 * BS + 3 * t + 2] = sg[5];
        lds_g[6 * BS + t] = sg[6];
        lds_g[7 * BS + 3 * t] = sg[7]; lds_g[7 * BS + 3 * t + 1] = sg[8]; lds_g[7 * BS + 3 * t + 2] = sg[9];
        reinterpret_cast<float4*>(lds_g + 10 * BS)[t] = make_float4(sg[10], sg[11], sg[12], sg[13]);
        __syncthreads();
        float* const gout[5] = {a.dL_dmean3D, a.dL_drgb ? a.dL_drgb : a.dL_ddc, a.dL_dopacity, a.dL_dscale, a.dL_drot};
        small_groups_sink<BS, DEFER_XYZ>(a.adam, gout, lds_g, lds_vis, row0, rows);
    } else if (idx < a.row_end && M > 0 && (a.dL_dsh || a.adam.on)) {
        const AdamFusedArgs& A = a.adam;
        float c[15];
        sh_coefs(a.D, so.x, so.y, so.z, c);
        const int nk = M < 15 ? M : 15;
        const float dR[3] = {so.dR, so.dG, so.dB};
        const size_t rb = (size_t)3 * M * idx;
        for (int k = 0; k < 3 * M; k++) {
            const float g = (so.on && k < 3 * nk) ? c[k / 3] * dR[k % 3] : 0.f;
            if (a.dL_dsh) a.dL_dsh[rb + k] = g;
            if (A.on && lds_vis[threadIdx.x]) adam_scalar(A.p[2][rb + k], g, A.m[2][rb + k], A.v[2][rb + k], A.lr[2], A.b1, A.b2, A.eps);
        }
// ... 2 lines not shown
```

gaussian-lic_amd/csrc/render.hip:

```cpp
#include "gslic_common.h"
#include "kernels.h"
#include <stdlib.h>
#include <mutex>

namespace gslic {

__device__ __forceinline__ float strip_max_p2(float hA, float hC, float nB, float gx, float gy, float x0, float x1, float y0, float y1)
{
    const bool in_x = gx >= x0 && gx <= x1, in_y = gy >= y0 && gy <= y1;
    if (in_x && in_y) return 0.0f;
    float best = -3.0e38f;
    if (!in_y) {
        const float ye = gy < y0 ? y0 : y1;
        const float dy = gy - ye;
        float dx = -(nB * dy) / (2.0f * hA);
        dx = fminf(fmaxf(dx, gx - x1), gx - x0);
        best = fmaxf(best, (hA * dx) * dx + (hC * dy) * dy + (nB * dx) * dy);
    }
    if (!in_x) {
        const float xe = gx < x0 ? x0 : x1;
        const float dx = gx - xe;
        float dy = -(nB * dx) / (2.0f * hC);
        dy = fminf(fmaxf(dy, gy - y1), gy - y0);
        best = fmaxf(best, (hA * dx) * dx + (hC * dy) * dy + (nB * dx) * dy);
    }
    const float DX = fmaxf(fabsf(gx - x0), fabsf(gx - x1)), DY = fmaxf(fabsf(gy - y0), fabsf(gy - y1));
    return best + 1.0e-5f * (fabsf(hA) * DX * DX + fabsf(hC) * DY * DY + fabsf(nB) * DX * DY) + 1.0e-6f;
}

#ifndef GS_FWD_SKIP
#define GS_FWD_SKIP 0
#endif
#ifndef GS_FWD_TAIL4_DEFAULT
#define GS_FWD_TAIL4_DEFAULT 0.10f
#endif
#ifndef GS_FWD_WAVES
#define GS_FWD_WAVES 7
#endif
#ifndef GS_FWD_WAVES_DEPTH
#define GS_FWD_WAVES_DEPTH 6
#endif
template <bool STRICT, int SPLIT, bool DEPTH>
__global__ __launch_bounds__(64, SPLIT >= 2 ? (DEPTH ? GS_FWD_WAVES_DEPTH : GS_FWD_WAVES) : 5) void render_fwd_kernel(RenderFwdArgs a)
{
    __shared__ float4 s_rec[3 * GS_BUCKET];
    const uint32_t grp = blockIdx.x / (8u * SPLIT), rem = blockIdx.x % (8u * SPLIT);
    const int tile = (int)(grp * 8u + (rem & 7u));
    if (tile >= a.gx * a.gy) return;
    const int q0 = (int)(rem >> 3) * (4 / SPLIT);
#define GS_BODY_SPLIT SPLIT
#include "render_fwd_body.inc"
#undef GS_BODY_SPLIT
}

template <bool STRICT, bool DEPTH>
__global__ __launch_bounds__(64, DEPTH ? GS_FWD_WAVES_DEPTH : GS_FWD_WAVES) void render_fwd_tail_kernel(RenderFwdArgs a)
{
    __shared__ float4 s_rec[3 * GS_BUCKET];
    const uint32_t n2 = 2u * (uint32_t)a.tail4_from;
    if (blockIdx.x < n2) {
        const uint32_t grp = blockIdx.x / 16u, rem = blockIdx.x % 16u;
        const int tile = (int)(grp * 8u + (rem & 7u));
        const int q0 = (int)(rem >> 3) * 2;
#define GS_BODY_SPLIT 2
#include "render_fwd_body.inc"
#undef GS_BODY_SPLIT
    } else {
        const uint32_t bb = blockIdx.x - n2, grp = bb / 32u, rem = bb % 32u;
        const int tile = a.tail4_from + (int)(grp * 8u + (rem & 7u));
        if (tile >= a.gx * a.gy) return;
        const int q0 = (int)(rem >> 3);
#define GS_BODY_SPLIT 4
#include "render_fwd_body.inc"
#undef GS_BODY_SPLIT
    }
}

typedef float v2f __attribute__((ext_vector_type(2)));
typedef float v4f __attribute__((ext_vector_type(4)));
#define GS_PK_FMA(a, b, c) __builtin_elementwise_fma((a), (b), (c))
#define GS_SPLAT(x) ((v2f){(x), (x)})

struct BwdLane {
    v2f d0, hAC, col_rg;
    float nB, lop, colb;
// ... 204 lines not shown
    v2f acc_S = {0.f, 0.f}, acc_cxy = {0.f, 0.f}, acc_rg = {0.f, 0.f};
    float acc_cw = 0, acc_op = 0, acc_b = 0, acc_z = 0;
    float T1 = 0.f, A1 = 0.f, T2, A2;
    float4 Ra, Rb;
    uint2 Ha = make_uint2(0u, 0u), Hb = make_uint2(0u, 0u);
    float Ga = 0.f, Gb = 0.f;
    int off = -8 * lane, kzero_i = 0, khi = 8 * (int)ninj, keight = 8;
    asm volatile("" : "+v"(off), "+v"(kzero_i), "+v"(khi), "+v"(keight));
#define GS_BW_LOOP(USE_BITS)                                                                                         \
    GS_BW_PREFETCH(USE_BITS, T2, A2, Ra, Ha, Ga);                                                                    \
    for (uint32_t sidx = 0; sidx < nsteps; sidx += 2) {                                                              \
        GS_BW_SHIFT_INJ(T2, A2, T1, A1);                                                          \
        GS_BW_PREFETCH(USE_BITS, T1, A1, Rb, Hb, Gb);                                                                \
        GS_BW_BODY(USE_BITS, T2, A2, Ra, Ha, Ga);                                                                    \
        GS_BW_SHIFT_INJ(T1, A1, T2, A2);                                                          \
        GS_BW_PREFETCH(USE_BITS, T2, A2, Ra, Ha, Ga);                                                                \
        GS_BW_BODY(USE_BITS, T1, A1, Rb, Hb, Gb);                                                                    \
    }
    if (use_bits) { GS_BW_LOOP(true) } else { GS_BW_LOOP(false) }
#undef GS_BW_LOOP

    if (valid) {
        const float kx = 0.5f * (float)a.W / LOG2E, ky = 0.5f * (float)a.H / LOG2E;
        const float gx = __builtin_fmaf(2.0f * L.hAC.x, acc_S.x, L.nB * acc_S.y) * kx;
        const float gy = __builtin_fmaf(2.0f * L.hAC.y, acc_S.y, L.nB * acc_S.x) * ky;
        float* o = a.partials + GS_PROW * (size_t)slot;
        *reinterpret_cast<gs_v4f_u*>(o) = (gs_v4f_u){gx, gy, -0.5f * acc_cxy.x, -0.5f * acc_cxy.y};
        *reinterpret_cast<gs_v4f_u*>(o + 4) = (gs_v4f_u){-0.5f * acc_cw, acc_op * rop, acc_rg.x, acc_rg.y};
        o[8] = acc_b;
        if constexpr (DEPTH) a.partials_z[slot] = acc_z;
    }
}

static std::mutex g_fwd_note_mu;
static struct { const void* hit; bool strict; } g_fwd_note[64];
static unsigned g_fwd_note_next = 0;
static void note_forward(const void* hit, bool strict)
{
    std::lock_guard<std::mutex> lk(g_fwd_note_mu);
    for (auto& e : g_fwd_note)
        if (e.hit == hit) { e.strict = strict; return; }
    g_fwd_note[g_fwd_note_next++ & 63u] = {hit, strict};
}
static bool forward_known_strict(const void* hit)
{
    std::lock_guard<std::mutex> lk(g_fwd_note_mu);
    for (auto& e : g_fwd_note)
        if (e.hit == hit) return e.strict;
    return false;
}

template <bool DEPTH>
static int launch_render_fwd_t(const RenderFwdArgs& a, hipStream_t s)
{
    if (!a.no_color && a.hit) note_forward(a.hit, g_strict_math != 0);
    static const int forced = [] { const char* e = getenv("GSLIC_FWD_SPLIT"); const int v = e ? atoi(e) : 0; return (v == 1 || v == 2 || v == 4) ? v : 0; }();
    const unsigned T = (unsigned)(a.gx * a.gy);
    const int split = forced ? forced : 2;
    const unsigned groups = (T + 7u) / 8u;
    static const float tail4 = [] { const char* e = getenv("GSLIC_FWD_TAIL4"); const float v = e ? (float)atof(e) : GS_FWD_TAIL4_DEFAULT; return v < 0.f ? 0.f : (v > 1.f ? 1.f : v); }();
    if (split == 2 && tail4 > 0.f) {
        RenderFwdArgs b = a;
        static const bool tail4_env = getenv("GSLIC_FWD_TAIL4") != nullptr;
        unsigned tail_tiles = (unsigned)(tail4 * (float)T);
        if (!tail4_env && tail_tiles > 896u) tail_tiles = 896u;
        b.tail4_from = (int)(T - tail_tiles) & ~7;
        const unsigned grid = 2u * (unsigned)b.tail4_from + 32u * ((T - (unsigned)b.tail4_from + 7u) / 8u);
        if (g_strict_math) GS_LAUNCH(K_RENDER_FWD, (render_fwd_tail_kernel<true, DEPTH>), dim3(grid), dim3(64), 0, s, b);
        else GS_LAUNCH(K_RENDER_FWD, (render_fwd_tail_kernel<false, DEPTH>), dim3(grid), dim3(64), 0, s, b);
        return GSLIC_OK;
    }
    if (g_strict_math && split == 1) GS_LAUNCH(K_RENDER_FWD, (render_fwd_kernel<true, 1, DEPTH>), dim3(groups * 8u), dim3(64), 0, s, a);
    else if (g_strict_math && split == 4) GS_LAUNCH(K_RENDER_FWD, (render_fwd_kernel<true, 4, DEPTH>), dim3(groups * 32u), dim3(64), 0, s, a);
    else if (g_strict_math) GS_LAUNCH(K_RENDER_FWD, (render_fwd_kernel<true, 2, DEPTH>), dim3(groups * 16u), dim3(64), 0, s, a);
    else if (split == 1) GS_LAUNCH(K_RENDER_FWD, (render_fwd_kernel<false, 1, DEPTH>), dim3(groups * 8u), dim3(64), 0, s, a);
    else if (split == 4) GS_LAUNCH(K_RENDER_FWD, (render_fwd_kernel<false, 4, DEPTH>), dim3(groups * 32u), dim3(64), 0, s, a);
    else GS_LAUNCH(K_RENDER_FWD, (render_fwd_kernel<false, 2, DEPTH>), dim3(groups * 16u), dim3(64), 0, s, a);
    return GSLIC_OK;
}
int launch_render_fwd(const RenderFwdArgs& a, hipStream_t s)
{
    return a.out_depth ? launch_render_fwd_t<true>(a, s) : launch_render_fwd_t<false>(a, s);
}
int launch_render_bwd(const RenderBwdArgs& a, hipStream_t s)
{
    const bool depth = a.dL_ddepth != nullptr;
    if (a.B <= 0) return GSLIC_OK;
    static const int xcd_lg = [] {
        const char* e = getenv("GSLIC_BWD_XCD_RUN");
        const int v = e ? atoi(e) : 16;
        int lg = -1;
        for (int k = 0; k < 12; k++) if (v == (1 << k)) lg = k;
        return lg;
    }();
    static const bool use_scan = [] { const char* e = getenv("GSLIC_BWD_SCAN"); return !(e && atoi(e) == 0); }();
    RenderBwdArgs b = a;
    b.xcd_lg = xcd_lg;
    b.skip_if_bits = 0;
    unsigned grid = (unsigned)a.B;
    if (xcd_lg >= 0) { const unsigned unit = 8u << xcd_lg; grid = (grid + unit - 1u) / unit * unit; }
    if (g_strict_math && use_scan) {
        launch_render_bwd_scan(b, grid, s);
        if (forward_known_strict(a.hit)) return GSLIC_OK;
        b.skip_if_bits = 1;
    }
    if (depth) {
        if (g_strict_math) GS_LAUNCH(K_RENDER_BWD, (render_bwd_kernel<true, true>), dim3(grid), dim3(64), 0, s, b);
        else GS_LAUNCH(K_RENDER_BWD, (render_bwd_kernel<false, true>), dim3(grid), dim3(64), 0, s, b);
        return GSLIC_OK;
    }
    if (g_strict_math) GS_LAUNCH(K_RENDER_BWD, (render_bwd_kernel<true, false>), dim3(grid), dim3(64), 0, s, b);
    else GS_LAUNCH(K_RENDER_BWD, (render_bwd_kernel<false, false>), dim3(grid), dim3(64), 0, s, b);
    return GSLIC_OK;
}

}
```

gaussian-lic_amd/csrc/render_bwd_scan.hip:

```cpp
#include "gslic_common.h"
#include "kernels.h"
#include <stdlib.h>

#ifndef GS_SCAN_SKIP
#define GS_SCAN_SKIP 0
#endif

namespace gslic {

typedef float v2f_s __attribute__((ext_vector_type(2)));

template <int CTRL, int ROW_MASK = 0xf>
__device__ __forceinline__ float dpp_f(float old, float src)
{
    return __int_as_float(__builtin_amdgcn_update_dpp(__float_as_int(old), __float_as_int(src), CTRL, ROW_MASK, 0xf, false));
}
template <int CTRL, int ROW_MASK = 0xf>
__device__ __forceinline__ uint32_t dpp_u(uint32_t old, uint32_t src)
{
    return (uint32_t)__builtin_amdgcn_update_dpp((int)old, (int)src, CTRL, ROW_MASK, 0xf, false);
}
#ifdef GS_SCAN_SAFE
__device__ __forceinline__ float row_scan_mul(float x)
{
    const int i = lane_id() & 15;
#pragma unroll
    for (int d = 1; d < 16; d <<= 1) { const float o = __shfl_up(x, d, 16); if (i >= d) x *= o; }
    return x;
}
__device__ __forceinline__ float row_scan_add(float x)
{
    const int i = lane_id() & 15;
#pragma unroll
    for (int d = 1; d < 16; d <<= 1) { const float o = __shfl_up(x, d, 16); if (i >= d) x += o; }
    return x;
}
__device__ __forceinline__ float row_last(float x) { return __shfl(x, 15, 16); }
__device__ __forceinline__ uint32_t wave_or(uint32_t v)
{
#pragma unroll
    for (int d = 32; d >= 1; d >>= 1) v |= (uint32_t)__shfl_xor((int)v, d, 64);
    return readlane_u(v, 0);
}
#else
#ifndef GS_DPP_WAIT
#define GS_DPP_WAIT "s_nop 1\n\t"
#endif
__device__ __forceinline__ float row_scan_mul(float x)
{
    asm(GS_DPP_WAIT "v_mul_f32_dpp %0, %0, %0 row_shr:1 row_mask:0xf bank_mask:0xf\n\t"
        GS_DPP_WAIT "v_mul_f32_dpp %0, %0, %0 row_shr:2 row_mask:0xf bank_mask:0xf\n\t"
        GS_DPP_WAIT "v_mul_f32_dpp %0, %0, %0 row_shr:4 row_mask:0xf bank_mask:0xf\n\t"
        GS_DPP_WAIT "v_mul_f32_dpp %0, %0, %0 row_shr:8 row_mask:0xf bank_mask:0xf"
        : "+v"(x));
    return x;
}
__device__ __forceinline__ float row_scan_add(float x)
{
    asm(GS_DPP_WAIT "v_add_f32_dpp %0, %0, %0 row_shr:1 row_mask:0xf bank_mask:0xf\n\t"
        GS_DPP_WAIT "v_add_f32_dpp %0, %0, %0 row_shr:2 row_mask:0xf bank_mask:0xf\n\t"
        GS_DPP_WAIT "v_add_f32_dpp %0, %0, %0 row_shr:4 row_mask:0xf bank_mask:0xf\n\t"
        GS_DPP_WAIT "v_add_f32_dpp %0, %0, %0 row_shr:8 row_mask:0xf bank_mask:0xf"
        : "+v"(x));
    return x;
}
__device__ __forceinline__ float row_last(float x) { return dpp_f<0x15f>(x, x); }
__device__ __forceinline__ uint32_t wave_or(uint32_t v)
{
    v |= dpp_u<0x111>(0u, v);
    v |= dpp_u<0x112>(0u, v);
    v |= dpp_u<0x114>(0u, v);
    v |= dpp_u<0x118>(0u, v);
    v |= dpp_u<0x142, 0xa>(0u, v);
    v |= dpp_u<0x143, 0xc>(0u, v);
    return readlane_u(v, 63);
}
#endif

__device__ __forceinline__ void half_or(uint32_t v, uint32_t& lo_half, uint32_t& hi_half)
{
#ifdef GS_SCAN_SAFE
#pragma unroll
    for (int d = 16; d >= 1; d >>= 1) v |= (uint32_t)__shfl_xor((int)v, d, 64);
    lo_half = readlane_u(v, 0); hi_half = readlane_u(v, 32);
#else
    v |= dpp_u<0x111>(0u, v);
    v |= dpp_u<0x112>(0u, v);
    v |= dpp_u<0x114>(0u, v);
    v |= dpp_u<0x118>(0u, v);
    v |= dpp_u<0x142, 0xa>(0u, v);
    lo_half = readlane_u(v, 31); hi_half = readlane_u(v, 63);
#endif
}

struct ScanEntry {
    float d0x, d0y;
    float hA, hC, nB;
    float lop;
    float cr, cg, cb;
    float z;
};

constexpr int SC_HALF = 32 + 1;
constexpr int SC_NENT = 2 * SC_HALF;
constexpr int SC_ENT_F4 = 3;

struct ScanLds {
    float4 ent[64 * SC_ENT_F4];
    float acc[64 * 9];
    uint32_t list[2 * 64];
    float2 ta[SC_NENT], rg[SC_NENT], bx[SC_NENT], py[SC_NENT];
    uint2 hm[SC_NENT];
};

template <int NG, bool DEPTH>
__device__ __forceinline__ void block_pass(ScanLds& S, float* accz, const int lane, const int rb, const int lb, const int npx_, const int ne, float c099)
{
    const int npx = rb + npx_;
    const int slot_i = lane & 15, row = lane >> 4;
    ScanEntry E[NG];
    uint32_t ent[NG], kbit[NG], klo[NG];
    v2f_s acc_S[NG], acc_cxy[NG], acc_rg[NG];
    float acc_cw[NG], acc_op[NG], acc_b[NG], acc_z[NG];
#pragma unroll
    for (int g = 0; g < NG; g++) {
        acc_S[g] = acc_cxy[g] = acc_rg[g] = (v2f_s){0.f, 0.f};
        acc_cw[g] = acc_op[g] = acc_b[g] = acc_z[g] = 0.f;
        E[g] = {0.f, 0.f, 0.f, 0.f, 0.f, -__builtin_inff(), 0.f, 0.f, 0.f, 0.f};
        ent[g] = 0u; kbit[g] = 0u; klo[g] = 0u;
        const int k = 16 * g + slot_i;
        if (k < ne) {
            const uint32_t e = S.list[lb + k];
            const float4 e0 = S.ent[SC_ENT_F4 * e], e1 = S.ent[SC_ENT_F4 * e + 1], e2 = S.ent[SC_ENT_F4 * e + 2];
            E[g] = {e0.x, e0.y, e0.z, e0.w, e1.x, e1.y, e1.z, e1.w, e2.x, DEPTH ? e2.w : 0.f};
            ent[g] = e; kbit[g] = e & 31u; klo[g] = e < 32u ? 0xffffffffu : 0u;
        }
    }
    const int nchunk = ((GS_SCAN_SKIP & 4) && c099 > 0.f) ? 0 : (npx_ + 3) >> 2;
    int off = rb + row;
    for (int c = 0; c < nchunk; c++, off += 4) {
        const int idx = off < npx ? off : npx;
        const float2 ta = S.ta[idx], rg = S.rg[idx], bx = S.bx[idx], pyv = S.py[idx];
        const uint2 hm = S.hm[idx];
        float Tin = ta.x, Ain = ta.y;
        const float pxf = bx.y, pyf = pyv.x, gD = pyv.y;
#pragma unroll
        for (int g = 0; g < NG; g++) {
            const float dx = E[g].d0x - pxf, dy = E[g].d0y - pyf;
            float p2 = __builtin_fmaf(__builtin_fmaf(E[g].hA, dx, E[g].nB * dy), dx, E[g].lop);
            p2 = __builtin_fmaf(E[g].hC * dy, dy, p2);
            const float araw = __builtin_amdgcn_exp2f(p2);
            uint32_t sel_, m_;
            asm("v_bfi_b32 %0, %1, %2, %3" : "=v"(sel_) : "v"(klo[g]), "v"(hm.x), "v"(hm.y));
            asm("v_bfe_i32 %0, %1, %2, 1" : "=v"(m_) : "v"(sel_), "v"(kbit[g]));
            const float ah = __uint_as_float(__float_as_uint(araw) & m_);
            float alpha;
            asm("v_min_f32 %0, %1, %2" : "=v"(alpha) : "v"(ah), "v"(c099));
            const float om = 1.0f - alpha;
            const float rinv = __builtin_amdgcn_rcpf(om);
            const float Tincl = Tin * row_scan_mul(om);
            const float Ti = Tincl * rinv;
            const float Ta = Ti * alpha;
            float cgd = E[g].cr * rg.x;
            cgd = __builtin_fmaf(E[g].cg, rg.y, cgd);
            cgd = __builtin_fmaf(E[g].cb, bx.x, cgd);
            if constexpr (DEPTH) cgd = __builtin_fmaf(E[g].z, gD, cgd);
            const float Ap = Ain + row_scan_add(Ta * cgd);
            const float dLda = __builtin_fmaf(rinv, Ap, Ti * cgd);
            const float w = ah * dLda;
            acc_rg[g] = __builtin_elementwise_fma((v2f_s){Ta, Ta}, (v2f_s){rg.x, rg.y}, acc_rg[g]);
            acc_b[g] = __builtin_fmaf(Ta, bx.x, acc_b[g]);
            if constexpr (DEPTH) acc_z[g] = __builtin_fmaf(Ta, gD, acc_z[g]);
            const v2f_s d = {dx, dy};
            const v2f_s wd = (v2f_s){w, w} * d;
            acc_S[g] += wd;
            acc_cxy[g] = __builtin_elementwise_fma((v2f_s){wd.x, wd.x}, d, acc_cxy[g]);
            acc_cw[g] = __builtin_fmaf(wd.y, dy, acc_cw[g]);
            acc_op[g] += w;
            if (g + 1 < NG) { Tin = row_last(Tincl); Ain = row_last(Ap); }
        }
    }
#pragma unroll
    for (int g = 0; g < NG; g++) {
        float v[9] = {acc_S[g].x, acc_S[g].y, acc_cxy[g].x, acc_cxy[g].y, acc_cw[g], acc_op[g], acc_rg[g].x, acc_rg[g].y, acc_b[g]};
#pragma unroll
        for (int k = 0; k < 9; k++) {
            v[k] += __shfl_xor(v[k], 16, 64);
            v[k] += __shfl_xor(v[k], 32, 64);
        }
        if (row == 0 && 16 * g + slot_i < ne) {
#pragma unroll
            for (int k = 0; k < 9; k++) S.acc[9 * ent[g] + k] += v[k];
        }
        if constexpr (DEPTH) {
            float vz = acc_z[g];
            vz += __shfl_xor(vz, 16, 64);
            vz += __shfl_xor(vz, 32, 64);
            if (row == 0 && 16 * g + slot_i < ne) accz[ent[g]] += vz;
        }
    }
}

#ifndef GS_SCAN_WAVES
#define GS_SCAN_WAVES 4
#endif
#ifndef GS_SCAN_WAVES_DEPTH
#define GS_SCAN_WAVES_DEPTH GS_SCAN_WAVES
#endif
template <bool DEPTH>
__global__ __launch_bounds__(64, DEPTH ? GS_SCAN_WAVES_DEPTH : GS_SCAN_WAVES) void render_bwd_scan_kernel(RenderBwdArgs a)
{
    __shared__ ScanLds S;
    __shared__ float s_accz[DEPTH ? 64 : 1];
    const int lane = threadIdx.x;
    uint32_t bucket = blockIdx.x;
    if (a.xcd_lg >= 0) {
        const uint32_t x = bucket & 7u, j = bucket >> 3;
        bucket = ((((j >> a.xcd_lg) << 3) + x) << a.xcd_lg) + (j & ((1u << a.xcd_lg) - 1u));
    }
    if (a.status[2] != 0u || bucket >= a.bucket_offsets[a.T - 1]) return;
    if (a.status[GS_FLAG_HITBITS] == 0u) return;
    const uint32_t tile = a.bucket_to_tile[bucket];
    const uint2 range = a.ranges[tile];
    const uint32_t n = range.y - range.x;
    const uint32_t bbm = (tile == 0) ? 0u : a.bucket_offsets[tile - 1];
    const uint32_t bstart = (bucket - bbm) * GS_BUCKET;
    const uint32_t kit = bstart + (uint32_t)lane;
    const bool valid = kit < n;
    const uint32_t slot = valid ? a.inst_slot[range.x + kit] : 0u;
    if (bstart >= a.max_contrib[tile]) {
        if (valid && !((GS_SCAN_SKIP & 8) && a.T > -1)) a.dead[slot] = 1;
        return;
    }
    const int tx0 = (int)(tile % (uint32_t)a.gx) * GS_TILE, ty0 = (int)(tile / (uint32_t)a.gx) * GS_TILE;
    const size_t plane = (size_t)a.H * a.W;

    const float LOG2E = 1.4426950408889634f;
    {
    ScanEntry L = {0.f, 0.f, 0.f, 0.f, 0.f, -__builtin_inff(), 0.f, 0.f, 0.f, 0.f};
    float rop = 0.f;
    if (valid && !((GS_SCAN_SKIP & 32) && a.T > -1)) {
        const uint32_t g = a.point_list[range.x + kit];
        const float4* rp = a.rec + GS_REC_F4 * (size_t)g;
        const float4 r0 = rp[0], r1 = rp[1], r2 = rp[2];
        L.d0x = r0.x - (float)tx0; L.d0y = r0.y - (float)ty0;
        L.hA = -0.5f * LOG2E * r0.z; L.nB = -LOG2E * r0.w; L.hC = -0.5f * LOG2E * r1.x;
        L.lop = __builtin_amdgcn_logf(r1.y);
        rop = r1.y > 0.f ? 1.0f / r1.y : 0.f;
        L.cr = r1.z; L.cg = r1.w; L.cb = r2.x;
        if constexpr (DEPTH) L.z = r2.y;
    }
    S.ent[SC_ENT_F4 * lane] = make_float4(L.d0x, L.d0y, L.hA, L.hC);
    S.ent[SC_ENT_F4 * lane + 1] = make_float4(L.nB, L.lop, L.cr, L.cg);
    S.ent[SC_ENT_F4 * lane + 2] = make_float4(L.cb, rop, __uint_as_float(slot), DEPTH ? L.z : 0.f);
#pragma unroll
    for (int k = 0; k < 9; k++) S.acc[9 * lane + k] = 0.f;
    if constexpr (DEPTH) s_accz[lane] = 0.f;
    }

    float c099 = 0.99f;
    asm volatile("" : "+v"(c099));

    struct PixIn { uint64_t hm; float4 pf, ck; float g0, g1, g2, ckd, pfd, gd; };
    auto load_pix = [&](int q) {
        PixIn r;
        const int pidx = q * 64 + lane;
        r.hm = a.hit[(size_t)bucket * GS_TILE_PIX + pidx];
        r.pf = a.pix_final[(size_t)tile * GS_TILE_PIX + pidx];
        r.ck = a.ckpt[(size_t)bucket * GS_TILE_PIX + pidx];
        const int px = tx0 + tile_pix_x(pidx), py = ty0 + tile_pix_y(pidx);
        r.g0 = r.g1 = r.g2 = 0.f;
        r.ckd = r.pfd = r.gd = 0.f;
        if constexpr (DEPTH) { r.ckd = a.ckpt_depth[(size_t)bucket * GS_TILE_PIX + pidx]; r.pfd = a.pix_depth[(size_t)tile * GS_TILE_PIX + pidx]; }
        if (px < a.W && py < a.H) {
            const size_t pid = (size_t)py * a.W + px;
            r.g0 = a.dL_dpix[pid]; r.g1 = a.dL_dpix[plane + pid]; r.g2 = a.dL_dpix[2 * plane + pid];
            if constexpr (DEPTH) r.gd = a.dL_ddepth[pid];
        }
        return r;
    };
#ifndef GS_SCAN_PREFETCH
#define GS_SCAN_PREFETCH 0
#endif
#if GS_SCAN_PREFETCH
    PixIn nxt = load_pix(0);
#endif
    uint32_t any_lo = 0u, any_hi = 0u;
    for (int q = 0; q < (((GS_SCAN_SKIP & 2) && a.T > -1) ? 0 : 4); q++) {
#if GS_SCAN_PREFETCH
        const PixIn cur = nxt;
        if (q < 3) nxt = load_pix(q + 1);
#else
        const PixIn cur = load_pix(q);
#endif
        const int pidx = q * 64 + lane;
        const uint64_t hm64 = cur.hm;
        const int lx = tile_pix_x(pidx), ly = tile_pix_y(pidx);
        const int px = tx0 + lx, py = ty0 + ly;
        const float4 pf = cur.pf;
        const bool active = px < a.W && py < a.H && __float_as_uint(pf.w) > bstart && hm64 != 0ull;
        const uint64_t bal = __ballot(active);
        if (bal == 0ull) continue;
        const uint32_t mlo = active ? (uint32_t)hm64 : 0u, mhi = active ? (uint32_t)(hm64 >> 32) : 0u;
        uint32_t S_lo[2], S_hi[2];
        half_or(mlo, S_lo[0], S_lo[1]);
        half_or(mhi, S_hi[0], S_hi[1]);
        any_lo |= S_lo[0] | S_lo[1]; any_hi |= S_hi[0] | S_hi[1];
        const uint32_t balh[2] = {(uint32_t)bal, (uint32_t)(bal >> 32)};
        const int half = lane >> 5;
        __builtin_amdgcn_fence(__ATOMIC_RELEASE, "wavefront");
        __builtin_amdgcn_wave_barrier();
        if (active) {
            const float4 ck = cur.ck;
            const float g0 = cur.g0, g1 = cur.g1, g2 = cur.g2;
            float A0 = (ck.y - pf.x) * g0;
            A0 = __builtin_fmaf(ck.z - pf.y, g1, A0);
            A0 = __builtin_fmaf(ck.w - pf.z, g2, A0);
            if constexpr (DEPTH) A0 = __builtin_fmaf(cur.ckd - cur.pfd, cur.gd, A0);
            const uint32_t pos = half ? (uint32_t)SC_HALF + __builtin_amdgcn_mbcnt_hi(balh[1], 0u) : __builtin_amdgcn_mbcnt_lo(balh[0], 0u);
            S.ta[pos] = make_float2(ck.x, A0);
            S.rg[pos] = make_float2(g0, g1);
            S.bx[pos] = make_float2(g2, (float)lx);
            S.py[pos] = make_float2((float)ly, DEPTH ? cur.gd : 0.f);
            S.hm[pos] = make_uint2(mlo, mhi);
        }
        if ((lane & 31) == 0) {
            const int z = half * SC_HALF + __popc(half ? balh[1] : balh[0]);
            S.ta[z] = S.rg[z] = S.bx[z] = S.py[z] = make_float2(0.f, 0.f);
            S.hm[z] = make_uint2(0u, 0u);
        }
#pragma unroll
        for (int h = 0; h < 2; h++) {
            const bool mine = lane < 32 ? ((S_lo[h] >> lane) & 1u) : ((S_hi[h] >> (lane - 32)) & 1u);
            const uint32_t k = __builtin_amdgcn_mbcnt_hi(S_hi[h], __builtin_amdgcn_mbcnt_lo(S_lo[h], 0u));
            if (mine) S.list[64 * h + k] = (uint32_t)lane;
        }
        __builtin_amdgcn_fence(__ATOMIC_RELEASE, "wavefront");
        __builtin_amdgcn_wave_barrier();
        for (int h = 0; h < 2; h++) {
            const int npx = __popc(h ? balh[1] : balh[0]);
            if (npx == 0 || ((GS_SCAN_SKIP & 1) && a.T > -1)) continue;
            const int ne = h ? __popc(S_lo[1]) + __popc(S_hi[1]) : __popc(S_lo[0]) + __popc(S_hi[0]);
            switch ((ne + 15) >> 4) {
            case 1: block_pass<1, DEPTH>(S, s_accz, lane, h * SC_HALF, 64 * h, npx, ne, c099); break;
            case 2: block_pass<2, DEPTH>(S, s_accz, lane, h * SC_HALF, 64 * h, npx, ne, c099); break;
            case 3: block_pass<3, DEPTH>(S, s_accz, lane, h * SC_HALF, 64 * h, npx, ne, c099); break;
            default: block_pass<4, DEPTH>(S, s_accz, lane, h * SC_HALF, 64 * h, npx, ne, c099); break;
            }
        }
    }
    __builtin_amdgcn_fence(__ATOMIC_RELEASE, "wavefront");
    __builtin_amdgcn_wave_barrier();

#ifndef GS_SCAN_ZERO_ROWS
#define GS_SCAN_ZERO_ROWS 0
#endif
    const bool blended = GS_SCAN_ZERO_ROWS || (lane < 32 ? ((any_lo >> lane) & 1u) : ((any_hi >> (lane - 32)) & 1u));
    if (valid && !blended && !((GS_SCAN_SKIP & 8) && a.T > -1)) a.dead[slot] = 1;
    if (valid && blended && !((GS_SCAN_SKIP & 16) && a.T > -1)) {
        const float4 e0 = S.ent[SC_ENT_F4 * lane], e1 = S.ent[SC_ENT_F4 * lane + 1], e2 = S.ent[SC_ENT_F4 * lane + 2];
        const ScanEntry L = {e0.x, e0.y, e0.z, e0.w, e1.x, e1.y, e1.z, e1.w, e2.x};
        const float rop = e2.y;
        const uint32_t slot = __float_as_uint(e2.z);
        const float* s = S.acc + 9 * lane;
        const float Sx = s[0], Sy = s[1], cxx = s[2], cxy = s[3], cyy = s[4], op = s[5], cr = s[6], cg = s[7], cb = s[8];
        const float kx = 0.5f * (float)a.W / LOG2E, ky = 0.5f * (float)a.H / LOG2E;
        const float gx = __builtin_fmaf(2.0f * L.hA, Sx, L.nB * Sy) * kx;
        const float gy = __builtin_fmaf(2.0f * L.hC, Sy, L.nB * Sx) * ky;
        float* o = a.partials + GS_PROW * (size_t)slot;
        *reinterpret_cast<gs_v4f_u*>(o) = (gs_v4f_u){gx, gy, -0.5f * cxx, -0.5f * cxy};
        *reinterpret_cast<gs_v4f_u*>(o + 4) = (gs_v4f_u){-0.5f * cyy, op * rop, cr, cg};
        o[8] = cb;
        if constexpr (DEPTH) a.partials_z[slot] = s_accz[lane];
    }
}

int launch_render_bwd_scan(const RenderBwdArgs& b, unsigned grid, hipStream_t s)
{
    if (b.dL_ddepth) GS_LAUNCH(K_RENDER_BWD, render_bwd_scan_kernel<true>, dim3(grid), dim3(64), 0, s, b);
    else GS_LAUNCH(K_RENDER_BWD, render_bwd_scan_kernel<false>, dim3(grid), dim3(64), 0, s, b);
    return GSLIC_OK;
}

}
```

include/gslic_hip.h:

```cpp
#ifndef GSLIC_HIP_H_INCLUDED
#define GSLIC_HIP_H_INCLUDED

#include <stddef.h>
#include <stdint.h>

#ifdef __cplusplus
extern "C" {
#endif

#define GSLIC_ABI_VERSION 8

typedef enum gslic_status {
    GSLIC_OK = 0,
    GSLIC_ERR_INVALID_ARG = -1,
    GSLIC_ERR_UNSUPPORTED = -2,
    GSLIC_ERR_ALLOC = -3,
    GSLIC_ERR_HIP = -4,
    GSLIC_ERR_PREFILTERED = -5
} gslic_status;

typedef char* (*gslic_alloc_fn)(void* ctx, size_t bytes);

typedef struct gslic_raster_params {
    int32_t P;
// ... 215 lines not shown

int gslic_rasterize_backward_camera(
    const gslic_raster_params* prm, int32_t R, int32_t B,
    const float* background, const float* means3D, const float* dc, const float* shs, const float* colors_precomp,
    const float* scales, const float* rotations, const float* cov3D_precomp,
    const float* viewmatrix, const float* projmatrix, const float* cam_pos, const int32_t* radii,
    char* geom_buffer, char* binning_buffer, char* img_buffer, char* sample_buffer, const float* dL_dpix,
    float* dL_dmean2D, float* dL_dconic, float* dL_dopacity, float* dL_dcolor, float* dL_dmean3D, float* dL_dcov3D,
    float* dL_ddc, float* dL_dsh, float* dL_dscale, float* dL_drot, float lambda_erank,
    float* dL_dviewmatrix, float* dL_dprojmatrix, float* dL_dcampos, void* stream);

int gslic_rasterize_backward_depth_camera(
    const gslic_raster_params* prm, int32_t R, int32_t B,
    const float* background, const float* means3D, const float* dc, const float* shs, const float* colors_precomp,
    const float* scales, const float* rotations, const float* cov3D_precomp,
    const float* viewmatrix, const float* projmatrix, const float* cam_pos, const int32_t* radii,
    char* geom_buffer, char* binning_buffer, char* img_buffer, char* sample_buffer, const float* dL_dpix, const float* dL_ddepth,
    float* dL_dmean2D, float* dL_dconic, float* dL_dopacity, float* dL_dcolor, float* dL_dmean3D, float* dL_dcov3D,
    float* dL_ddc, float* dL_dsh, float* dL_dscale, float* dL_drot, float lambda_erank,
    float* dL_dviewmatrix, float* dL_dprojmatrix, float* dL_dcampos, void* stream);

int gslic_adam_update(
    float* param, const float* param_grad, float* exp_avg, float* exp_avg_sq,
    const uint8_t* visible,
    float lr, float b1, float b2, float eps,
    uint32_t N, uint32_t M, void* stream);

typedef struct gslic_adam_group {
    float* param; const float* grad; float* exp_avg; float* exp_avg_sq;
    float lr; uint32_t M;
} gslic_adam_group;
int gslic_adam_update_groups(
    const gslic_adam_group* groups, int32_t n_groups,
    const uint8_t* visible, float b1, float b2, float eps, uint32_t N, void* stream);

int gslic_fusedssim_forward(
    int32_t B, int32_t CH, int32_t H, int32_t W, float C1, float C2,
    const float* img1, const float* img2,
    float* ssim_map, float* dm_dmu1, float* dm_dsigma1_sq, float* dm_dsigma12,
    void* stream);
int gslic_fusedssim_backward(
    int32_t B, int32_t CH, int32_t H, int32_t W, float C1, float C2,
    const float* img1, const float* img2, const float* dL_dmap,
    const float* dm_dmu1, const float* dm_dsigma1_sq, const float* dm_dsigma12,
    float* dL_dimg1, void* stream);

int64_t gslic_loss_partials_count(int32_t B, int32_t CH, int32_t H, int32_t W);
int gslic_l1_ssim_loss_forward(
    int32_t B, int32_t CH, int32_t H, int32_t W, float C1, float C2, const float* img, const float* gt,
    float* dm_dmu1, float* dm_dsigma1_sq, float* dm_dsigma12, float* partials, float* terms , void* stream);
int gslic_l1_ssim_loss_backward(
    int32_t B, int32_t CH, int32_t H, int32_t W, float lambda_dssim, const float* img, const float* gt,
    const float* dm_dmu1, const float* dm_dsigma1_sq, const float* dm_dsigma12, float* dL_dimg, void* stream);
int gslic_l1_ssim_loss_forward_backward(
    int32_t B, int32_t CH, int32_t H, int32_t W, float C1, float C2, float lambda_dssim, const float* img, const float* gt,
    float* dm_dmu1, float* dm_dsigma1_sq, float* dm_dsigma12, float* partials, float* terms , float* dL_dimg, void* stream);

int64_t gslic_depth_l1_loss_partials_count(int32_t H, int32_t W);
int gslic_depth_l1_loss_forward_backward(
    int32_t H, int32_t W, float lambda_depth, const float* depth, const float* gt_depth, float* partials, float* term ,
    float* dL_ddepth, void* stream);

int gslic_knn_mean_dist2(
    int32_t P, const float* points, float* mean_dists,
    gslic_alloc_fn scratch_alloc, void* scratch_ctx, void* stream);

int gslic_extend_select(
    int32_t n, const float* points, const float* depths_rsp, const float* R_cw, const float* t_cw,
    float fx, float fy, float cx, float cy, int32_t width, int32_t height, const float* final_T,
    gslic_alloc_fn scratch_alloc, void* scratch_ctx,
    uint32_t** keep_flags, uint32_t** keep_pos, int32_t* count, void* stream);
int gslic_extend_emit(
    int32_t n, const uint32_t* keep_flags, const uint32_t* keep_pos, const float* points, const float* colors,
    const float* depths_rsp, float scaling_scale, float focal, int32_t M,
    float* xyz, float* dc, float* rest, float* opacity, float* scaling, float* rotation, void* stream);

int gslic_abi_version(void);
const char* gslic_last_error(void);

int gslic_set_math_mode(int32_t strict);

int gslic_set_binning_mode(int32_t mode);

#define GSLIC_BINNING_PATH_NONE 0
#define GSLIC_BINNING_PATH_RADIX 1
#define GSLIC_BINNING_PATH_ATOMIC 2
int gslic_get_binning_path(uint32_t* sampled_atomics, uint32_t* sampled_instances);

size_t gslic_scratch_round_up(size_t bytes);

size_t gslic_geom_bytes(int32_t P);
size_t gslic_img_bytes(int32_t width, int32_t height);
size_t gslic_binning_bytes(int32_t R, int32_t no_color);
size_t gslic_sample_bytes(int32_t B);
size_t gslic_img_bytes_depth(int32_t width, int32_t height);
size_t gslic_binning_bytes_depth(int32_t R);
size_t gslic_sample_bytes_depth(int32_t B);

#define GSLIC_PROFILE_MAX_KERNELS 48
int gslic_profile_enable(int32_t on);
int gslic_profile_reset(void);
int gslic_profile_collect(void);
int gslic_profile_num_kernels(void);
const char* gslic_profile_kernel_name(int32_t id);
int gslic_profile_get(int32_t id, double* total_ms, int64_t* launches);

int gslic_debug_export(
    const gslic_raster_params* prm, int32_t R, int32_t B,
    const char* geom_buffer, const char* binning_buffer, const char* img_buffer, const char* sample_buffer,
    uint32_t* tiles_touched , float* means2D , float* depths ,
    float* conic_opacity , float* rgb ,
    uint64_t* sorted_keys , uint32_t* point_list , uint32_t* ranges ,
    uint32_t* n_contrib , uint32_t* max_contrib ,
    void* stream);

#ifdef __cplusplus
}
#endif
#endif
```

Measured before the change: 568.9 views/s.

## Fuse occluded-Gaussian Adam into backward scan and skip them in preprocess backward

Result: slower. 540.6 views/s (-5.0%).

```diff
diff --git a/gaussian-lic_amd/_lib.py b/gaussian-lic_amd/_lib.py
--- a/gaussian-lic_amd/_lib.py
+++ b/gaussian-lic_amd/_lib.py
@@ -39,7 +39,7 @@
     "gslic_rasterize_forward_depth", "gslic_rasterize_backward_depth",
     "gslic_rasterize_forward_depth_capacity", "gslic_rasterize_backward_depth_adam", "gslic_depth_l1_loss_partials_count",
     "gslic_depth_l1_loss_forward_backward", "gslic_img_bytes_depth", "gslic_binning_bytes_depth", "gslic_sample_bytes_depth",
-    "gslic_rasterize_backward_depth_camera",
+    "gslic_rasterize_backward_depth_camera", "gslic_set_occluded_adam",
 ]
 
 _lib = None
@@ -125,6 +125,7 @@
     L.gslic_l1_ssim_loss_forward_backward.argtypes = [i32, i32, i32, i32, f32, f32, f32] + [vp] * 8 + [vp]
     L.gslic_set_math_mode.argtypes = [i32]
     L.gslic_set_binning_mode.argtypes = [i32]
+    L.gslic_set_occluded_adam.argtypes = [i32]
     L.gslic_get_binning_path.argtypes = [ctypes.POINTER(u32), ctypes.POINTER(u32)]
     L.gslic_scratch_round_up.restype = ctypes.c_size_t
     L.gslic_scratch_round_up.argtypes = [ctypes.c_size_t]
@@ -141,6 +142,10 @@
 def set_binning_mode(mode):
     names = ("auto", "radix", "atomic")
     return names[lib().gslic_set_binning_mode(names.index(mode))]
+
+
+def set_occluded_adam(on):
+    return bool(lib().gslic_set_occluded_adam(-1 if on is None else int(bool(on))))
 
 
 def binning_path():
diff --git a/gaussian-lic_amd/build.py b/gaussian-lic_amd/build.py
--- a/gaussian-lic_amd/build.py
+++ b/gaussian-lic_amd/build.py
@@ -18,6 +18,7 @@
     "preprocess.hip": ["-ffp-contract=off"],
     "render.hip": ["-fno-slp-vectorize"],
     "render_bwd_scan.hip": ["-fno-slp-vectorize"],
+    "render_bwd_scan_adam.hip": ["-fno-slp-vectorize"],
     "preprocess_bwd.hip": [],
     "adam.hip": [],
     "ssim.hip": ["-ffp-contract=off"],
@@ -27,7 +28,7 @@
 }
 COMMON = [f"--offload-arch={ARCH}", "-O3", "-std=c++17", "-fPIC", "-fno-fast-math", "-Wno-inline-asm",
           "-fhip-fp32-correctly-rounded-divide-sqrt", "-Wall", "-Wno-unused-function"]
-HEADERS = ["gslic_common.h", "kernels.h", "render_fwd_body.inc", "preprocess_bwd_body.inc", os.path.join("..", "..", "include", "gslic_hip.h")]
+HEADERS = ["gslic_common.h", "kernels.h", "render_fwd_body.inc", "render_bwd_scan_body.inc", "render_bwd_scan_common.h", "preprocess_bwd_body.inc", os.path.join("..", "..", "include", "gslic_hip.h")]
 
 
 def _newer(a, b):
diff --git a/gaussian-lic_amd/csrc/api.hip b/gaussian-lic_amd/csrc/api.hip
--- a/gaussian-lic_amd/csrc/api.hip
+++ b/gaussian-lic_amd/csrc/api.hip
@@ -34,7 +34,7 @@
 static const char* const k_names[K_COUNT] = {
     "preprocess", "scan_reduce", "scan_spine", "scan_apply", "keybuild", "sort_hist", "sort_scatter", "finalize_lists",
     "bucket_count", "render_fwd", "render_bwd", "preprocess_bwd", "adam", "ssim_fwd", "ssim_bwd", "knn_minmax", "knn_morton",
-    "knn_boxes", "knn_search", "debug_export", "extend", "dsort_hist", "dsort_scatter", "sh_grad_from_rgb", "tile_lsort", "tile_hist", "tile_bin", "tile_scan", "tile_lsort_long", "depth_loss"};
+    "knn_boxes", "knn_search", "debug_export", "extend", "dsort_hist", "dsort_scatter", "sh_grad_from_rgb", "tile_lsort", "tile_hist", "tile_bin", "tile_scan", "tile_lsort_long", "depth_loss", "mark_live"};
 uint32_t g_lds_pad[K_COUNT] = {0};
 static const bool g_lds_pad_parsed = [] {
     const char* e = getenv("GSLIC_LDS_PAD");
@@ -89,7 +89,8 @@
     g.gauss_start = c.take<uint32_t>(P);
     g.flags = c.take<uint32_t>(64);
     g.scan_state = c.take<char>(scan_state_bytes(P));
-    g.zero_bytes = 64 * sizeof(uint32_t) + scan_state_bytes(P);
+    g.live = c.take<uint8_t>(P);
+    g.zero_bytes = (size_t)(reinterpret_cast<const char*>(g.live) + P - reinterpret_cast<const char*>(g.flags));
     if (bytes) *bytes = c.used(base) + 256;
     return g;
 }
@@ -584,6 +585,8 @@
 }
 
 extern "C" {
+int gslic_set_occluded_adam(int32_t on) { return set_occluded_adam(on); }
+
 int gslic_set_binning_mode(int32_t mode)
 {
     if (mode < 0 || mode > 2) return g_binning_mode.load(std::memory_order_relaxed);
@@ -728,7 +731,16 @@
     rb.bucket_offsets = img.bucket_offsets; rb.bucket_to_tile = smp.bucket_to_tile; rb.ckpt = smp.ckpt; rb.hit = smp.hit; rb.pix_final = img.pix_final;
     rb.max_contrib = img.max_contrib; rb.dL_dpix = dL_dpix; rb.partials = bin.partials; rb.dead = bin.dead; rb.status = geom.flags; rb.T = T;
     rb.dL_ddepth = dL_ddepth; rb.ckpt_depth = smp.ckpt_depth; rb.pix_depth = img.pix_depth; rb.partials_z = bin.partials_z;
-    if (!skip_blend) GS_TRY(launch_render_bwd(rb, s));
+    bool occluded_done = false;
+    if (adam && !skip_blend && !depth && !dL_dcam && !dL_drgb && !dL_dmean2D && !dL_dconic && !dL_dopacity && !dL_dcolor && !dL_dmean3D && !dL_dcov3D &&
+        !dL_ddc && !dL_dsh && !dL_dscale && !dL_drot && prm->M == 15 && shs && !(lambda_erank > 0) && row_begin == 0 && (row_end < 0 || row_end == P)) {
+        OccludedAdamArgs oa;
+        oa.P = P; oa.radii = radii; oa.live = geom.live; oa.status = geom.flags; oa.n_scan = oa.n_adam = 1u;
+        for (int g = 0; g < 6; g++) { oa.adam.p[g] = adam->param[g]; oa.adam.m[g] = adam->exp_avg[g]; oa.adam.v[g] = adam->exp_avg_sq[g]; oa.adam.lr[g] = adam->lr[g]; }
+        oa.adam.b1 = adam->b1; oa.adam.b2 = adam->b2; oa.adam.eps = adam->eps; oa.adam.on = 1;
+        occluded_done = launch_render_bwd_occluded_adam(rb, oa, s);
+    }
+    if (!skip_blend && !occluded_done) GS_TRY(launch_render_bwd(rb, s));
     DEBUG_SYNC(prm, s);
 
     PreprocessBwdArgs pb;
@@ -752,6 +764,7 @@
     pb.cam_partials = nullptr; pb.cam_out = nullptr;
     pb.partials_z = depth ? bin.partials_z : nullptr;
     pb.vis_out = vis_out; pb.campos_out = campos_out;
+    pb.live = occluded_done ? geom.live : nullptr;
     if (dL_dcam) {
         pb.cam_partials = geom.cam_scratch;
         pb.cam_out = geom.cam_scratch + 128 * (((size_t)P + 255) / 256);
diff --git a/gaussian-lic_amd/csrc/gslic_common.h b/gaussian-lic_amd/csrc/gslic_common.h
--- a/gaussian-lic_amd/csrc/gslic_common.h
+++ b/gaussian-lic_amd/csrc/gslic_common.h
@@ -62,6 +62,7 @@
     K_TILE_SCAN,
     K_TILE_LSORT_LONG,
     K_DEPTH_LOSS,
+    K_MARK_LIVE,
     K_COUNT
 };
 void prof_begin(int id, hipStream_t s);
@@ -181,6 +182,7 @@
     uint32_t* gauss_start;
     uint32_t* flags;
     void* scan_state;
+    uint8_t* live;
     size_t zero_bytes;
     static GeomState carve(const void* base, size_t P, size_t* bytes);
 };
diff --git a/gaussian-lic_amd/csrc/kernels.h b/gaussian-lic_amd/csrc/kernels.h
--- a/gaussian-lic_amd/csrc/kernels.h
+++ b/gaussian-lic_amd/csrc/kernels.h
@@ -111,8 +111,25 @@
     float* cam_partials;
     float* cam_out;
     const float* partials_z;
+    const uint8_t* live;
 };
 int launch_preprocess_bwd(const PreprocessBwdArgs& a, hipStream_t s);
+
+struct OccludedAdamArgs {
+    int P;
+    const int32_t* radii;
+    uint8_t* live;
+    const uint32_t* status;
+    AdamFusedArgs adam;
+    uint32_t n_scan, n_adam;
+};
+struct RenderBwdAdamArgs {
+    RenderBwdArgs rb;
+    OccludedAdamArgs oa;
+};
+int set_occluded_adam(int on);
+bool launch_render_bwd_occluded_adam(const RenderBwdArgs& a, const OccludedAdamArgs& o, hipStream_t s);
+int launch_render_bwd_scan_adam(const RenderBwdAdamArgs& b, unsigned grid, hipStream_t s);
 
 struct ShGradFromRgbArgs {
     int P, D, M, n_views, input_is_ddc;
diff --git a/gaussian-lic_amd/csrc/preprocess_bwd.hip b/gaussian-lic_amd/csrc/preprocess_bwd.hip
--- a/gaussian-lic_amd/csrc/preprocess_bwd.hip
+++ b/gaussian-lic_amd/csrc/preprocess_bwd.hip
@@ -47,6 +47,7 @@
 
 struct PartialSums { float mx, my, cx, cy, cw, op, r, g, b; };
 
+template <bool SKIP_OCC = false>
 __device__ __forceinline__ bool bwd_gather(const PreprocessBwdArgs& a, const int idx, const bool staged, PartialSums& ps);
 template <bool CAM, bool DEFER_XYZ = false>
 __device__ __forceinline__ void bwd_rest(const PreprocessBwdArgs& a, const int idx, const PartialSums& ps, const float* sh_row, const float* sk_row,
@@ -209,6 +210,7 @@
 __global__ __launch_bounds__(BS) GS_PBWD_OCC void preprocess_bwd_kernel(PreprocessBwdArgs a)
 {
     constexpr bool DEFER_XYZ = false;
+    constexpr bool SKIP_OCC = false;
 #include "preprocess_bwd_body.inc"
 }
 template <bool LDS_SH, int BS>
@@ -216,13 +218,24 @@
 {
     constexpr bool CAM = false;
     constexpr bool DEFER_XYZ = true;
+    constexpr bool SKIP_OCC = false;
 #include "preprocess_bwd_body.inc"
 }
-
+template <bool LDS_SH, int BS>
+__global__ __launch_bounds__(BS) GS_PBWD_OCC void preprocess_bwd_skip_occluded_kernel(PreprocessBwdArgs a)
+{
+    constexpr bool CAM = false;
+    constexpr bool DEFER_XYZ = false;
+    constexpr bool SKIP_OCC = true;
+#include "preprocess_bwd_body.inc"
+}
+
+template <bool SKIP_OCC>
 __device__ __forceinline__ bool bwd_gather(const PreprocessBwdArgs& a, const int idx, const bool staged, PartialSums& ps)
 {
     ps.mx = ps.my = ps.cx = ps.cy = ps.cw = ps.op = ps.r = ps.g = ps.b = 0.f;
-    const bool visible = a.radii[idx] > 0;
+    bool visible = a.radii[idx] > 0;
+    if constexpr (SKIP_OCC) visible = visible && a.live[idx] != 0;
 
     if (!visible) {
         if (a.dL_dmean2D) { a.dL_dmean2D[3 * idx] = 0; a.dL_dmean2D[3 * idx + 1] = 0; a.dL_dmean2D[3 * idx + 2] = 0; }
@@ -683,10 +696,15 @@
     if (nrows <= 0) return GSLIC_OK;
     if (cam) GS_HIP(hipMemsetAsync(a.cam_out, 0, 35 * sizeof(float), s));
     if (a.M == 15 && a.shs && (a.dL_dsh || a.adam.on || a.dL_drgb)) {
+        if (a.live) {
+            if (cam || defer || !a.adam.on) return set_error(GSLIC_ERR_INVALID_ARG, "preprocess_bwd: liveness marks go with the colour-only fused Adam");
+            GS_LAUNCH(K_PREPROCESS_BWD, (preprocess_bwd_skip_occluded_kernel<true, 64>), dim3(div_up(nrows, 64)), dim3(64), 0, s, a);
+        } else
         if (cam) GS_LAUNCH(K_PREPROCESS_BWD, (preprocess_bwd_kernel<true, 64, true>), dim3(div_up(nrows, 64)), dim3(64), 0, s, a);
         else if (defer) GS_LAUNCH(K_PREPROCESS_BWD, (preprocess_bwd_defer_xyz_kernel<true, 64>), dim3(div_up(nrows, 64)), dim3(64), 0, s, a);
         else GS_LAUNCH(K_PREPROCESS_BWD, (preprocess_bwd_kernel<true, 64, false>), dim3(div_up(nrows, 64)), dim3(64), 0, s, a);
     } else {
+        if (a.live) return set_error(GSLIC_ERR_INVALID_ARG, "preprocess_bwd: liveness marks need the 45-float SH rows");
         if (cam) GS_LAUNCH(K_PREPROCESS_BWD, (preprocess_bwd_kernel<false, 256, true>), dim3(div_up(nrows, 256)), dim3(256), 0, s, a);
         else if (defer) GS_LAUNCH(K_PREPROCESS_BWD, (preprocess_bwd_defer_xyz_kernel<false, 256>), dim3(div_up(nrows, 256)), dim3(256), 0, s, a);
         else GS_LAUNCH(K_PREPROCESS_BWD, (preprocess_bwd_kernel<false, 256, false>), dim3(div_up(nrows, 256)), dim3(256), 0, s, a);
diff --git a/gaussian-lic_amd/csrc/preprocess_bwd_body.inc b/gaussian-lic_amd/csrc/preprocess_bwd_body.inc
--- a/gaussian-lic_amd/csrc/preprocess_bwd_body.inc
+++ b/gaussian-lic_amd/csrc/preprocess_bwd_body.inc
@@ -20,8 +20,11 @@
     }
     PartialSums ps;
     bool visible = false;
-    if (idx < a.row_end) visible = bwd_gather(a, idx, LDS_SH, ps);
+    if (idx < a.row_end) visible = bwd_gather<SKIP_OCC>(a, idx, LDS_SH, ps);
     lds_vis[threadIdx.x] = visible ? 1 : 0;
+    if constexpr (SKIP_OCC) {
+        if (a.vis_out && idx < a.row_end) a.vis_out[idx] = a.radii[idx] > 0 ? 1 : 0;
+    } else
     if (a.vis_out && idx < a.row_end) a.vis_out[idx] = visible ? 1 : 0;
     if (a.campos_out && blockIdx.x == 0 && threadIdx.x < 3) a.campos_out[threadIdx.x] = a.campos[threadIdx.x];
     if constexpr (LDS_SH) {
diff --git a/gaussian-lic_amd/csrc/render.hip b/gaussian-lic_amd/csrc/render.hip
--- a/gaussian-lic_amd/csrc/render.hip
+++ b/gaussian-lic_amd/csrc/render.hip
@@ -1,6 +1,7 @@
 #include "gslic_common.h"
 #include "kernels.h"
 #include <stdlib.h>
+#include <atomic>
 #include <mutex>
 
 namespace gslic {
@@ -371,10 +372,8 @@
 {
     return a.out_depth ? launch_render_fwd_t<true>(a, s) : launch_render_fwd_t<false>(a, s);
 }
-int launch_render_bwd(const RenderBwdArgs& a, hipStream_t s)
-{
-    const bool depth = a.dL_ddepth != nullptr;
-    if (a.B <= 0) return GSLIC_OK;
+static int bwd_xcd_lg()
+{
     static const int xcd_lg = [] {
         const char* e = getenv("GSLIC_BWD_XCD_RUN");
         const int v = e ? atoi(e) : 16;
@@ -382,7 +381,38 @@
         for (int k = 0; k < 12; k++) if (v == (1 << k)) lg = k;
         return lg;
     }();
+    return xcd_lg;
+}
+static bool bwd_use_scan()
+{
     static const bool use_scan = [] { const char* e = getenv("GSLIC_BWD_SCAN"); return !(e && atoi(e) == 0); }();
+    return use_scan;
+}
+static std::atomic<int> g_occluded_adam{[] { const char* e = getenv("GSLIC_OCCLUDED_ADAM"); return (e && atoi(e) == 0) ? 0 : 1; }()};
+int set_occluded_adam(int on)
+{
+    if (on < 0) return g_occluded_adam.load(std::memory_order_relaxed);
+    return g_occluded_adam.exchange(on ? 1 : 0, std::memory_order_relaxed);
+}
+bool launch_render_bwd_occluded_adam(const RenderBwdArgs& a, const OccludedAdamArgs& o, hipStream_t s)
+{
+    if (!g_occluded_adam.load(std::memory_order_relaxed) || a.B <= 0 || a.dL_ddepth || !g_strict_math || !bwd_use_scan() || !forward_known_strict(a.hit)) return false;
+    const int xcd_lg = bwd_xcd_lg();
+    RenderBwdAdamArgs b;
+    b.rb = a;
+    b.rb.xcd_lg = xcd_lg;
+    b.rb.skip_if_bits = 0;
+    b.oa = o;
+    unsigned grid = (unsigned)a.B;
+    if (xcd_lg >= 0) { const unsigned unit = 8u << xcd_lg; grid = (grid + unit - 1u) / unit * unit; }
+    return launch_render_bwd_scan_adam(b, grid, s) == GSLIC_OK;
+}
+int launch_render_bwd(const RenderBwdArgs& a, hipStream_t s)
+{
+    const bool depth = a.dL_ddepth != nullptr;
+    if (a.B <= 0) return GSLIC_OK;
+    const int xcd_lg = bwd_xcd_lg();
+    const bool use_scan = bwd_use_scan();
     RenderBwdArgs b = a;
     b.xcd_lg = xcd_lg;
     b.skip_if_bits = 0;
diff --git a/gaussian-lic_amd/csrc/render_bwd_scan.hip b/gaussian-lic_amd/csrc/render_bwd_scan.hip
--- a/gaussian-lic_amd/csrc/render_bwd_scan.hip
+++ b/gaussian-lic_amd/csrc/render_bwd_scan.hip
@@ -1,378 +1,12 @@
-#include "gslic_common.h"
-#include "kernels.h"
-#include <stdlib.h>
-
-#ifndef GS_SCAN_SKIP
-#define GS_SCAN_SKIP 0
-#endif
+#include "render_bwd_scan_common.h"
 
 namespace gslic {
 
-typedef float v2f_s __attribute__((ext_vector_type(2)));
-
-template <int CTRL, int ROW_MASK = 0xf>
-__device__ __forceinline__ float dpp_f(float old, float src)
-{
-    return __int_as_float(__builtin_amdgcn_update_dpp(__float_as_int(old), __float_as_int(src), CTRL, ROW_MASK, 0xf, false));
-}
-template <int CTRL, int ROW_MASK = 0xf>
-__device__ __forceinline__ uint32_t dpp_u(uint32_t old, uint32_t src)
-{
-    return (uint32_t)__builtin_amdgcn_update_dpp((int)old, (int)src, CTRL, ROW_MASK, 0xf, false);
-}
-#ifdef GS_SCAN_SAFE
-__device__ __forceinline__ float row_scan_mul(float x)
-{
-    const int i = lane_id() & 15;
-#pragma unroll
-    for (int d = 1; d < 16; d <<= 1) { const float o = __shfl_up(x, d, 16); if (i >= d) x *= o; }
-    return x;
-}
-__device__ __forceinline__ float row_scan_add(float x)
-{
-    const int i = lane_id() & 15;
-#pragma unroll
-    for (int d = 1; d < 16; d <<= 1) { const float o = __shfl_up(x, d, 16); if (i >= d) x += o; }
-    return x;
-}
-__device__ __forceinline__ float row_last(float x) { return __shfl(x, 15, 16); }
-__device__ __forceinline__ uint32_t wave_or(uint32_t v)
-{
-#pragma unroll
-    for (int d = 32; d >= 1; d >>= 1) v |= (uint32_t)__shfl_xor((int)v, d, 64);
-    return readlane_u(v, 0);
-}
-#else
-#ifndef GS_DPP_WAIT
-#define GS_DPP_WAIT "s_nop 1\n\t"
-#endif
-__device__ __forceinline__ float row_scan_mul(float x)
-{
-    asm(GS_DPP_WAIT "v_mul_f32_dpp %0, %0, %0 row_shr:1 row_mask:0xf bank_mask:0xf\n\t"
-        GS_DPP_WAIT "v_mul_f32_dpp %0, %0, %0 row_shr:2 row_mask:0xf bank_mask:0xf\n\t"
-        GS_DPP_WAIT "v_mul_f32_dpp %0, %0, %0 row_shr:4 row_mask:0xf bank_mask:0xf\n\t"
-        GS_DPP_WAIT "v_mul_f32_dpp %0, %0, %0 row_shr:8 row_mask:0xf bank_mask:0xf"
-        : "+v"(x));
-    return x;
-}
-__device__ __forceinline__ float row_scan_add(float x)
-{
-    asm(GS_DPP_WAIT "v_add_f32_dpp %0, %0, %0 row_shr:1 row_mask:0xf bank_mask:0xf\n\t"
-        GS_DPP_WAIT "v_add_f32_dpp %0, %0, %0 row_shr:2 row_mask:0xf bank_mask:0xf\n\t"
-        GS_DPP_WAIT "v_add_f32_dpp %0, %0, %0 row_shr:4 row_mask:0xf bank_mask:0xf\n\t"
-        GS_DPP_WAIT "v_add_f32_dpp %0, %0, %0 row_shr:8 row_mask:0xf bank_mask:0xf"
-        : "+v"(x));
-    return x;
-}
-__device__ __forceinline__ float row_last(float x) { return dpp_f<0x15f>(x, x); }
-__device__ __forceinline__ uint32_t wave_or(uint32_t v)
-{
-    v |= dpp_u<0x111>(0u, v);
-    v |= dpp_u<0x112>(0u, v);
-    v |= dpp_u<0x114>(0u, v);
-    v |= dpp_u<0x118>(0u, v);
-    v |= dpp_u<0x142, 0xa>(0u, v);
-    v |= dpp_u<0x143, 0xc>(0u, v);
-    return readlane_u(v, 63);
-}
-#endif
-
-__device__ __forceinline__ void half_or(uint32_t v, uint32_t& lo_half, uint32_t& hi_half)
-{
-#ifdef GS_SCAN_SAFE
-#pragma unroll
-    for (int d = 16; d >= 1; d >>= 1) v |= (uint32_t)__shfl_xor((int)v, d, 64);
-    lo_half = readlane_u(v, 0); hi_half = readlane_u(v, 32);
-#else
-    v |= dpp_u<0x111>(0u, v);
-    v |= dpp_u<0x112>(0u, v);
-    v |= dpp_u<0x114>(0u, v);
-    v |= dpp_u<0x118>(0u, v);
-    v |= dpp_u<0x142, 0xa>(0u, v);
-    lo_half = readlane_u(v, 31); hi_half = readlane_u(v, 63);
-#endif
-}
-
-struct ScanEntry {
-    float d0x, d0y;
-    float hA, hC, nB;
-    float lop;
-    float cr, cg, cb;
-    float z;
-};
-
-constexpr int SC_HALF = 32 + 1;
-constexpr int SC_NENT = 2 * SC_HALF;
-constexpr int SC_ENT_F4 = 3;
-
-struct ScanLds {
-    float4 ent[64 * SC_ENT_F4];
-    float acc[64 * 9];
-    uint32_t list[2 * 64];
-    float2 ta[SC_NENT], rg[SC_NENT], bx[SC_NENT], py[SC_NENT];
-    uint2 hm[SC_NENT];
-};
-
-template <int NG, bool DEPTH>
-__device__ __forceinline__ void block_pass(ScanLds& S, float* accz, const int lane, const int rb, const int lb, const int npx_, const int ne, float c099)
-{
-    const int npx = rb + npx_;
-    const int slot_i = lane & 15, row = lane >> 4;
-    ScanEntry E[NG];
-    uint32_t ent[NG], kbit[NG], klo[NG];
-    v2f_s acc_S[NG], acc_cxy[NG], acc_rg[NG];
-    float acc_cw[NG], acc_op[NG], acc_b[NG], acc_z[NG];
-#pragma unroll
-    for (int g = 0; g < NG; g++) {
-        acc_S[g] = acc_cxy[g] = acc_rg[g] = (v2f_s){0.f, 0.f};
-        acc_cw[g] = acc_op[g] = acc_b[g] = acc_z[g] = 0.f;
-        E[g] = {0.f, 0.f, 0.f, 0.f, 0.f, -__builtin_inff(), 0.f, 0.f, 0.f, 0.f};
-        ent[g] = 0u; kbit[g] = 0u; klo[g] = 0u;
-        const int k = 16 * g + slot_i;
-        if (k < ne) {
-            const uint32_t e = S.list[lb + k];
-            const float4 e0 = S.ent[SC_ENT_F4 * e], e1 = S.ent[SC_ENT_F4 * e + 1], e2 = S.ent[SC_ENT_F4 * e + 2];
-            E[g] = {e0.x, e0.y, e0.z, e0.w, e1.x, e1.y, e1.z, e1.w, e2.x, DEPTH ? e2.w : 0.f};
-            ent[g] = e; kbit[g] = e & 31u; klo[g] = e < 32u ? 0xffffffffu : 0u;
-        }
-    }
-    const int nchunk = ((GS_SCAN_SKIP & 4) && c099 > 0.f) ? 0 : (npx_ + 3) >> 2;
-    int off = rb + row;
-    for (int c = 0; c < nchunk; c++, off += 4) {
-        const int idx = off < npx ? off : npx;
-        const float2 ta = S.ta[idx], rg = S.rg[idx], bx = S.bx[idx], pyv = S.py[idx];
-        const uint2 hm = S.hm[idx];
-        float Tin = ta.x, Ain = ta.y;
-        const float pxf = bx.y, pyf = pyv.x, gD = pyv.y;
-#pragma unroll
-        for (int g = 0; g < NG; g++) {
-            const float dx = E[g].d0x - pxf, dy = E[g].d0y - pyf;
-            float p2 = __builtin_fmaf(__builtin_fmaf(E[g].hA, dx, E[g].nB * dy), dx, E[g].lop);
-            p2 = __builtin_fmaf(E[g].hC * dy, dy, p2);
-            const float araw = __builtin_amdgcn_exp2f(p2);
-            uint32_t sel_, m_;
-            asm("v_bfi_b32 %0, %1, %2, %3" : "=v"(sel_) : "v"(klo[g]), "v"(hm.x), "v"(hm.y));
-            asm("v_bfe_i32 %0, %1, %2, 1" : "=v"(m_) : "v"(sel_), "v"(kbit[g]));
-            const float ah = __uint_as_float(__float_as_uint(araw) & m_);
-            float alpha;
-            asm("v_min_f32 %0, %1, %2" : "=v"(alpha) : "v"(ah), "v"(c099));
-            const float om = 1.0f - alpha;
-            const float rinv = __builtin_amdgcn_rcpf(om);
-            const float Tincl = Tin * row_scan_mul(om);
-            const float Ti = Tincl * rinv;
-            const float Ta = Ti * alpha;
-            float cgd = E[g].cr * rg.x;
-            cgd = __builtin_fmaf(E[g].cg, rg.y, cgd);
-            cgd = __builtin_fmaf(E[g].cb, bx.x, cgd);
-            if constexpr (DEPTH) cgd = __builtin_fmaf(E[g].z, gD, cgd);
-            const float Ap = Ain + row_scan_add(Ta * cgd);
-            const float dLda = __builtin_fmaf(rinv, Ap, Ti * cgd);
-            const float w = ah * dLda;
-            acc_rg[g] = __builtin_elementwise_fma((v2f_s){Ta, Ta}, (v2f_s){rg.x, rg.y}, acc_rg[g]);
-            acc_b[g] = __builtin_fmaf(Ta, bx.x, acc_b[g]);
-            if constexpr (DEPTH) acc_z[g] = __builtin_fmaf(Ta, gD, acc_z[g]);
-            const v2f_s d = {dx, dy};
-            const v2f_s wd = (v2f_s){w, w} * d;
-            acc_S[g] += wd;
-            acc_cxy[g] = __builtin_elementwise_fma((v2f_s){wd.x, wd.x}, d, acc_cxy[g]);
-            acc_cw[g] = __builtin_fmaf(wd.y, dy, acc_cw[g]);
-            acc_op[g] += w;
-            if (g + 1 < NG) { Tin = row_last(Tincl); Ain = row_last(Ap); }
-        }
-    }
-#pragma unroll
-    for (int g = 0; g < NG; g++) {
-        float v[9] = {acc_S[g].x, acc_S[g].y, acc_cxy[g].x, acc_cxy[g].y, acc_cw[g], acc_op[g], acc_rg[g].x, acc_rg[g].y, acc_b[g]};
-#pragma unroll
-        for (int k = 0; k < 9; k++) {
-            v[k] += __shfl_xor(v[k], 16, 64);
-            v[k] += __shfl_xor(v[k], 32, 64);
-        }
-        if (row == 0 && 16 * g + slot_i < ne) {
-#pragma unroll
-            for (int k = 0; k < 9; k++) S.acc[9 * ent[g] + k] += v[k];
-        }
-        if constexpr (DEPTH) {
-            float vz = acc_z[g];
-            vz += __shfl_xor(vz, 16, 64);
-            vz += __shfl_xor(vz, 32, 64);
-            if (row == 0 && 16 * g + slot_i < ne) accz[ent[g]] += vz;
-        }
-    }
-}
-
-#ifndef GS_SCAN_WAVES
-#define GS_SCAN_WAVES 4
-#endif
-#ifndef GS_SCAN_WAVES_DEPTH
-#define GS_SCAN_WAVES_DEPTH GS_SCAN_WAVES
-#endif
 template <bool DEPTH>
 __global__ __launch_bounds__(64, DEPTH ? GS_SCAN_WAVES_DEPTH : GS_SCAN_WAVES) void render_bwd_scan_kernel(RenderBwdArgs a)
 {
-    __shared__ ScanLds S;
-    __shared__ float s_accz[DEPTH ? 64 : 1];
-    const int lane = threadIdx.x;
-    uint32_t bucket = blockIdx.x;
-    if (a.xcd_lg >= 0) {
-        const uint32_t x = bucket & 7u, j = bucket >> 3;
-        bucket = ((((j >> a.xcd_lg) << 3) + x) << a.xcd_lg) + (j & ((1u << a.xcd_lg) - 1u));
-    }
-    if (a.status[2] != 0u || bucket >= a.bucket_offsets[a.T - 1]) return;
-    if (a.status[GS_FLAG_HITBITS] == 0u) return;
-    const uint32_t tile = a.bucket_to_tile[bucket];
-    const uint2 range = a.ranges[tile];
-    const uint32_t n = range.y - range.x;
-    const uint32_t bbm = (tile == 0) ? 0u : a.bucket_offsets[tile - 1];
-    const uint32_t bstart = (bucket - bbm) * GS_BUCKET;
-    const uint32_t kit = bstart + (uint32_t)lane;
-    const bool valid = kit < n;
-    const uint32_t slot = valid ? a.inst_slot[range.x + kit] : 0u;
-    if (bstart >= a.max_contrib[tile]) {
-        if (valid && !((GS_SCAN_SKIP & 8) && a.T > -1)) a.dead[slot] = 1;
-        return;
-    }
-    const int tx0 = (int)(tile % (uint32_t)a.gx) * GS_TILE, ty0 = (int)(tile / (uint32_t)a.gx) * GS_TILE;
-    const size_t plane = (size_t)a.H * a.W;
-
-    const float LOG2E = 1.4426950408889634f;
-    {
-    ScanEntry L = {0.f, 0.f, 0.f, 0.f, 0.f, -__builtin_inff(), 0.f, 0.f, 0.f, 0.f};
-    float rop = 0.f;
-    if (valid && !((GS_SCAN_SKIP & 32) && a.T > -1)) {
-        const uint32_t g = a.point_list[range.x + kit];
-        const float4* rp = a.rec + GS_REC_F4 * (size_t)g;
-        const float4 r0 = rp[0], r1 = rp[1], r2 = rp[2];
-        L.d0x = r0.x - (float)tx0; L.d0y = r0.y - (float)ty0;
-        L.hA = -0.5f * LOG2E * r0.z; L.nB = -LOG2E * r0.w; L.hC = -0.5f * LOG2E * r1.x;
-        L.lop = __builtin_amdgcn_logf(r1.y);
-        rop = r1.y > 0.f ? 1.0f / r1.y : 0.f;
-        L.cr = r1.z; L.cg = r1.w; L.cb = r2.x;
-        if constexpr (DEPTH) L.z = r2.y;
-    }
-    S.ent[SC_ENT_F4 * lane] = make_float4(L.d0x, L.d0y, L.hA, L.hC);
-    S.ent[SC_ENT_F4 * lane + 1] = make_float4(L.nB, L.lop, L.cr, L.cg);
-    S.ent[SC_ENT_F4 * lane + 2] = make_float4(L.cb, rop, __uint_as_float(slot), DEPTH ? L.z : 0.f);
-#pragma unroll
-    for (int k = 0; k < 9; k++) S.acc[9 * lane + k] = 0.f;
-    if constexpr (DEPTH) s_accz[lane] = 0.f;
-    }
-
-    float c099 = 0.99f;
-    asm volatile("" : "+v"(c099));
-
-    struct PixIn { uint64_t hm; float4 pf, ck; float g0, g1, g2, ckd, pfd, gd; };
-    auto load_pix = [&](int q) {
-        PixIn r;
-        const int pidx = q * 64 + lane;
-        r.hm = a.hit[(size_t)bucket * GS_TILE_PIX + pidx];
-        r.pf = a.pix_final[(size_t)tile * GS_TILE_PIX + pidx];
-        r.ck = a.ckpt[(size_t)bucket * GS_TILE_PIX + pidx];
-        const int px = tx0 + tile_pix_x(pidx), py = ty0 + tile_pix_y(pidx);
-        r.g0 = r.g1 = r.g2 = 0.f;
-        r.ckd = r.pfd = r.gd = 0.f;
-        if constexpr (DEPTH) { r.ckd = a.ckpt_depth[(size_t)bucket * GS_TILE_PIX + pidx]; r.pfd = a.pix_depth[(size_t)tile * GS_TILE_PIX + pidx]; }
-        if (px < a.W && py < a.H) {
-            const size_t pid = (size_t)py * a.W + px;
-            r.g0 = a.dL_dpix[pid]; r.g1 = a.dL_dpix[plane + pid]; r.g2 = a.dL_dpix[2 * plane + pid];
-            if constexpr (DEPTH) r.gd = a.dL_ddepth[pid];
-        }
-        return r;
-    };
-#ifndef GS_SCAN_PREFETCH
-#define GS_SCAN_PREFETCH 0
-#endif
-#if GS_SCAN_PREFETCH
-    PixIn nxt = load_pix(0);
-#endif
-    uint32_t any_lo = 0u, any_hi = 0u;
-    for (int q = 0; q < (((GS_SCAN_SKIP & 2) && a.T > -1) ? 0 : 4); q++) {
-#if GS_SCAN_PREFETCH
-        const PixIn cur = nxt;
-        if (q < 3) nxt = load_pix(q + 1);
-#else
-        const PixIn cur = load_pix(q);
-#endif
-        const int pidx = q * 64 + lane;
-        const uint64_t hm64 = cur.hm;
-        const int lx = tile_pix_x(pidx), ly = tile_pix_y(pidx);
-        const int px = tx0 + lx, py = ty0 + ly;
-        const float4 pf = cur.pf;
-        const bool active = px < a.W && py < a.H && __float_as_uint(pf.w) > bstart && hm64 != 0ull;
-        const uint64_t bal = __ballot(active);
-        if (bal == 0ull) continue;
-        const uint32_t mlo = active ? (uint32_t)hm64 : 0u, mhi = active ? (uint32_t)(hm64 >> 32) : 0u;
-        uint32_t S_lo[2], S_hi[2];
-        half_or(mlo, S_lo[0], S_lo[1]);
-        half_or(mhi, S_hi[0], S_hi[1]);
-        any_lo |= S_lo[0] | S_lo[1]; any_hi |= S_hi[0] | S_hi[1];
-        const uint32_t balh[2] = {(uint32_t)bal, (uint32_t)(bal >> 32)};
-        const int half = lane >> 5;
-        __builtin_amdgcn_fence(__ATOMIC_RELEASE, "wavefront");
-        __builtin_amdgcn_wave_barrier();
-        if (active) {
-            const float4 ck = cur.ck;
-            const float g0 = cur.g0, g1 = cur.g1, g2 = cur.g2;
-            float A0 = (ck.y - pf.x) * g0;
-            A0 = __builtin_fmaf(ck.z - pf.y, g1, A0);
-            A0 = __builtin_fmaf(ck.w - pf.z, g2, A0);
-            if constexpr (DEPTH) A0 = __builtin_fmaf(cur.ckd - cur.pfd, cur.gd, A0);
-            const uint32_t pos = half ? (uint32_t)SC_HALF + __builtin_amdgcn_mbcnt_hi(balh[1], 0u) : __builtin_amdgcn_mbcnt_lo(balh[0], 0u);
-            S.ta[pos] = make_float2(ck.x, A0);
-            S.rg[pos] = make_float2(g0, g1);
-            S.bx[pos] = make_float2(g2, (float)lx);
-            S.py[pos] = make_float2((float)ly, DEPTH ? cur.gd : 0.f);
-            S.hm[pos] = make_uint2(mlo, mhi);
-        }
-        if ((lane & 31) == 0) {
-            const int z = half * SC_HALF + __popc(half ? balh[1] : balh[0]);
-            S.ta[z] = S.rg[z] = S.bx[z] = S.py[z] = make_float2(0.f, 0.f);
-            S.hm[z] = make_uint2(0u, 0u);
-        }
-#pragma unroll
-        for (int h = 0; h < 2; h++) {
-            const bool mine = lane < 32 ? ((S_lo[h] >> lane) & 1u) : ((S_hi[h] >> (lane - 32)) & 1u);
-            const uint32_t k = __builtin_amdgcn_mbcnt_hi(S_hi[h], __builtin_amdgcn_mbcnt_lo(S_lo[h], 0u));
-            if (mine) S.list[64 * h + k] = (uint32_t)lane;
-        }
-        __builtin_amdgcn_fence(__ATOMIC_RELEASE, "wavefront");
-        __builtin_amdgcn_wave_barrier();
-        for (int h = 0; h < 2; h++) {
-            const int npx = __popc(h ? balh[1] : balh[0]);
-            if (npx == 0 || ((GS_SCAN_SKIP & 1) && a.T > -1)) continue;
-            const int ne = h ? __popc(S_lo[1]) + __popc(S_hi[1]) : __popc(S_lo[0]) + __popc(S_hi[0]);
-            switch ((ne + 15) >> 4) {
-            case 1: block_pass<1, DEPTH>(S, s_accz, lane, h * SC_HALF, 64 * h, npx, ne, c099); break;
-            case 2: block_pass<2, DEPTH>(S, s_accz, lane, h * SC_HALF, 64 * h, npx, ne, c099); break;
-            case 3: block_pass<3, DEPTH>(S, s_accz, lane, h * SC_HALF, 64 * h, npx, ne, c099); break;
-            default: block_pass<4, DEPTH>(S, s_accz, lane, h * SC_HALF, 64 * h, npx, ne, c099); break;
-            }
-        }
-    }
-    __builtin_amdgcn_fence(__ATOMIC_RELEASE, "wavefront");
-    __builtin_amdgcn_wave_barrier();
-
-#ifndef GS_SCAN_ZERO_ROWS
-#define GS_SCAN_ZERO_ROWS 0
-#endif
-    const bool blended = GS_SCAN_ZERO_ROWS || (lane < 32 ? ((any_lo >> lane) & 1u) : ((any_hi >> (lane - 32)) & 1u));
-    if (valid && !blended && !((GS_SCAN_SKIP & 8) && a.T > -1)) a.dead[slot] = 1;
-    if (valid && blended && !((GS_SCAN_SKIP & 16) && a.T > -1)) {
-        const float4 e0 = S.ent[SC_ENT_F4 * lane], e1 = S.ent[SC_ENT_F4 * lane + 1], e2 = S.ent[SC_ENT_F4 * lane + 2];
-        const ScanEntry L = {e0.x, e0.y, e0.z, e0.w, e1.x, e1.y, e1.z, e1.w, e2.x};
-        const float rop = e2.y;
-        const uint32_t slot = __float_as_uint(e2.z);
-        const float* s = S.acc + 9 * lane;
-        const float Sx = s[0], Sy = s[1], cxx = s[2], cxy = s[3], cyy = s[4], op = s[5], cr = s[6], cg = s[7], cb = s[8];
-        const float kx = 0.5f * (float)a.W / LOG2E, ky = 0.5f * (float)a.H / LOG2E;
-        const float gx = __builtin_fmaf(2.0f * L.hA, Sx, L.nB * Sy) * kx;
-        const float gy = __builtin_fmaf(2.0f * L.hC, Sy, L.nB * Sx) * ky;
-        float* o = a.partials + GS_PROW * (size_t)slot;
-        *reinterpret_cast<gs_v4f_u*>(o) = (gs_v4f_u){gx, gy, -0.5f * cxx, -0.5f * cxy};
-        *reinterpret_cast<gs_v4f_u*>(o + 4) = (gs_v4f_u){-0.5f * cyy, op * rop, cr, cg};
-        o[8] = cb;
-        if constexpr (DEPTH) a.partials_z[slot] = s_accz[lane];
-    }
+    const uint32_t scan_block = blockIdx.x;
+#include "render_bwd_scan_body.inc"
 }
 
 int launch_render_bwd_scan(const RenderBwdArgs& b, unsigned grid, hipStream_t s)
diff --git a/gaussian-lic_amd/csrc/render_bwd_scan_adam.hip b/gaussian-lic_amd/csrc/render_bwd_scan_adam.hip
--- /dev/null
+++ b/gaussian-lic_amd/csrc/render_bwd_scan_adam.hip
@@ -0,0 +1,135 @@
+#include "render_bwd_scan_common.h"
+
+namespace gslic {
+
+__global__ __launch_bounds__(256) void mark_live_kernel(int T, const uint2* __restrict__ ranges, const uint32_t* __restrict__ max_contrib,
+                                                        const uint32_t* __restrict__ point_list, const uint32_t* __restrict__ status,
+                                                        uint8_t* __restrict__ live)
+{
+    if (status[2] != 0u) return;
+    const uint32_t tile = blockIdx.x;
+    const uint2 range = ranges[tile];
+    const uint32_t n = range.y - range.x, mc = max_contrib[tile];
+    for (uint32_t kit = threadIdx.x; kit < n; kit += 256u) {
+        const uint32_t bstart = kit & ~(uint32_t)(GS_BUCKET - 1);
+        if (bstart >= mc) break;
+        live[point_list[range.x + kit]] = 1;
+    }
+}
+
+__device__ __forceinline__ void occluded_adam_block(const OccludedAdamArgs& o, const uint32_t blk)
+{
+    if (blk >= (uint32_t)((o.P + 63) >> 6) || o.status[2] != 0u) return;
+    const int lane = threadIdx.x;
+    const int row0 = (int)blk * 64, idx = row0 + lane;
+    const bool mine = idx < o.P && o.radii[idx] > 0 && o.live[idx] == 0;
+    const uint64_t mask = __ballot(mine);
+    if (mask == 0ull) return;
+    const AdamFusedArgs& A = o.adam;
+    const int rows = (o.P - row0) < 64 ? (o.P - row0) : 64;
+    constexpr int NG = 5;
+    constexpr int gid[NG] = {0, 1, 3, 4, 5};
+    constexpr int wid[NG] = {3, 3, 1, 3, 4};
+    if (rows == 64) {
+#pragma unroll
+        for (int k = 0; k < NG; k++) {
+            if (lane >= 16 * wid[k]) continue;
+            const int e = 4 * lane;
+            bool on[4];
+#pragma unroll
+            for (int c = 0; c < 4; c++) on[c] = (mask >> ((e + c) / wid[k])) & 1ull;
+            if (!(on[0] | on[1] | on[2] | on[3])) continue;
+            const size_t base = (size_t)row0 * wid[k];
+            float4 p = reinterpret_cast<const float4*>(A.p[gid[k]] + base)[lane];
+            float4 m = ld_stream(reinterpret_cast<const float4*>(A.m[gid[k]] + base) + lane);
+            float4 v = ld_stream(reinterpret_cast<const float4*>(A.v[gid[k]] + base) + lane);
+            const float lr = A.lr[gid[k]];
+            if (on[0]) adam_scalar(p.x, 0.0f, m.x, v.x, lr, A.b1, A.b2, A.eps);
+            if (on[1]) adam_scalar(p.y, 0.0f, m.y, v.y, lr, A.b1, A.b2, A.eps);
+            if (on[2]) adam_scalar(p.z, 0.0f, m.z, v.z, lr, A.b1, A.b2, A.eps);
+            if (on[3]) adam_scalar(p.w, 0.0f, m.w, v.w, lr, A.b1, A.b2, A.eps);
+            st_stream(reinterpret_cast<float4*>(A.p[gid[k]] + base) + lane, p);
+            st_stream(reinterpret_cast<float4*>(A.m[gid[k]] + base) + lane, m);
+            st_stream(reinterpret_cast<float4*>(A.v[gid[k]] + base) + lane, v);
+        }
+        constexpr int NV = 64 * 45 / 4, U = 4;
+        const size_t base = (size_t)row0 * 45;
+        for (int i0 = lane; i0 < NV; i0 += 64 * U) {
+            float4 x[U], m[U], v[U];
+            bool on[U][4], any[U];
+#pragma unroll
+            for (int u = 0; u < U; u++) {
+                const int i = i0 + 64 * u;
+                any[u] = false;
+                if (i < NV) {
+                    const int e = 4 * i, r0 = e / 45, rem0 = e - 45 * r0;
+                    const int r1 = (r0 + 1 < 64) ? r0 + 1 : r0;
+                    const bool v0 = (mask >> r0) & 1ull, v1 = (mask >> r1) & 1ull;
+#pragma unroll
+                    for (int c = 0; c < 4; c++) on[u][c] = (rem0 + c < 45) ? v0 : v1;
+                    any[u] = on[u][0] | on[u][3];
+                }
+                if (any[u]) {
+                    x[u] = reinterpret_cast<const float4*>(A.p[2] + base)[i];
+                    m[u] = ld_stream(reinterpret_cast<const float4*>(A.m[2] + base) + i);
+                    v[u] = ld_stream(reinterpret_cast<const float4*>(A.v[2] + base) + i);
+                }
+            }
+#pragma unroll
+            for (int u = 0; u < U; u++) {
+                if (!any[u]) continue;
+                const int i = i0 + 64 * u;
+                if (on[u][0]) adam_scalar(x[u].x, 0.0f, m[u].x, v[u].x, A.lr[2], A.b1, A.b2, A.eps);
+                if (on[u][1]) adam_scalar(x[u].y, 0.0f, m[u].y, v[u].y, A.lr[2], A.b1, A.b2, A.eps);
+                if (on[u][2]) adam_scalar(x[u].z, 0.0f, m[u].z, v[u].z, A.lr[2], A.b1, A.b2, A.eps);
+                if (on[u][3]) adam_scalar(x[u].w, 0.0f, m[u].w, v[u].w, A.lr[2], A.b1, A.b2, A.eps);
+                st_stream(reinterpret_cast<float4*>(A.p[2] + base) + i, x[u]);
+                st_stream(reinterpret_cast<float4*>(A.m[2] + base) + i, m[u]);
+                st_stream(reinterpret_cast<float4*>(A.v[2] + base) + i, v[u]);
+            }
+        }
+    } else {
+#pragma unroll
+        for (int k = 0; k < NG; k++) {
+            const size_t base = (size_t)row0 * wid[k];
+            for (int i = lane; i < rows * wid[k]; i += 64)
+                if ((mask >> (i / wid[k])) & 1ull)
+                    adam_scalar(A.p[gid[k]][base + i], 0.0f, A.m[gid[k]][base + i], A.v[gid[k]][base + i], A.lr[gid[k]], A.b1, A.b2, A.eps);
+        }
+        const size_t base = (size_t)row0 * 45;
+        for (int i = lane; i < rows * 45; i += 64)
+            if ((mask >> (i / 45)) & 1ull) adam_scalar(A.p[2][base + i], 0.0f, A.m[2][base + i], A.v[2][base + i], A.lr[2], A.b1, A.b2, A.eps);
+    }
+}
+
+__global__ __launch_bounds__(64, GS_SCAN_WAVES) void render_bwd_scan_adam_kernel(RenderBwdAdamArgs aa)
+{
+    const uint32_t row8 = blockIdx.x >> 3, x = blockIdx.x & 7u;
+    const uint32_t period = aa.oa.n_scan + aa.oa.n_adam;
+    const uint32_t cyc = row8 / period, r = row8 - cyc * period;
+    if (r >= aa.oa.n_scan) {
+        occluded_adam_block(aa.oa, ((cyc * aa.oa.n_adam + (r - aa.oa.n_scan)) << 3) + x);
+        return;
+    }
+    const uint32_t scan_block = ((cyc * aa.oa.n_scan + r) << 3) + x;
+    const RenderBwdArgs& a = aa.rb;
+    constexpr bool DEPTH = false;
+#include "render_bwd_scan_body.inc"
+}
+
+int launch_render_bwd_scan_adam(const RenderBwdAdamArgs& b_, unsigned grid, hipStream_t s)
+{
+    RenderBwdAdamArgs b = b_;
+    const uint32_t rows_scan = (grid + 7u) / 8u, rows_adam = ((uint32_t)div_up(b.oa.P, 64) + 7u) / 8u;
+    static const int forced = [] { const char* e = getenv("GSLIC_OCCLUDED_ADAM_RATIO"); return e ? atoi(e) : 0; }();
+    if (rows_scan >= rows_adam) { b.oa.n_scan = forced > 0 ? (uint32_t)forced : rows_scan / rows_adam; b.oa.n_adam = 1u; }
+    else { b.oa.n_scan = 1u; b.oa.n_adam = (rows_adam + rows_scan - 1u) / rows_scan; }
+    const uint32_t cyc_scan = (rows_scan + b.oa.n_scan - 1u) / b.oa.n_scan, cyc_adam = (rows_adam + b.oa.n_adam - 1u) / b.oa.n_adam;
+    const uint32_t cycles = cyc_scan > cyc_adam ? cyc_scan : cyc_adam;
+    GS_LAUNCH(K_MARK_LIVE, mark_live_kernel, dim3((unsigned)b.rb.T), dim3(256), 0, s, b.rb.T, b.rb.ranges, b.rb.max_contrib, b.rb.point_list, b.rb.status,
+              b.oa.live);
+    GS_LAUNCH(K_RENDER_BWD, render_bwd_scan_adam_kernel, dim3(cycles * (b.oa.n_scan + b.oa.n_adam) * 8u), dim3(64), 0, s, b);
+    return GSLIC_OK;
+}
+
+}
diff --git a/gaussian-lic_amd/csrc/render_bwd_scan_body.inc b/gaussian-lic_amd/csrc/render_bwd_scan_body.inc
--- /dev/null
+++ b/gaussian-lic_amd/csrc/render_bwd_scan_body.inc
@@ -0,0 +1,163 @@
+    __shared__ ScanLds S;
+    __shared__ float s_accz[DEPTH ? 64 : 1];
+    const int lane = threadIdx.x;
+    uint32_t bucket = scan_block;
+    if (a.xcd_lg >= 0) {
+        const uint32_t x = bucket & 7u, j = bucket >> 3;
+        bucket = ((((j >> a.xcd_lg) << 3) + x) << a.xcd_lg) + (j & ((1u << a.xcd_lg) - 1u));
+    }
+    if (a.status[2] != 0u || bucket >= a.bucket_offsets[a.T - 1]) return;
+    if (a.status[GS_FLAG_HITBITS] == 0u) return;
+    const uint32_t tile = a.bucket_to_tile[bucket];
+    const uint2 range = a.ranges[tile];
+    const uint32_t n = range.y - range.x;
+    const uint32_t bbm = (tile == 0) ? 0u : a.bucket_offsets[tile - 1];
+    const uint32_t bstart = (bucket - bbm) * GS_BUCKET;
+    const uint32_t kit = bstart + (uint32_t)lane;
+    const bool valid = kit < n;
+    const uint32_t slot = valid ? a.inst_slot[range.x + kit] : 0u;
+    if (bstart >= a.max_contrib[tile]) {
+        if (valid && !((GS_SCAN_SKIP & 8) && a.T > -1)) a.dead[slot] = 1;
+        return;
+    }
+    const int tx0 = (int)(tile % (uint32_t)a.gx) * GS_TILE, ty0 = (int)(tile / (uint32_t)a.gx) * GS_TILE;
+    const size_t plane = (size_t)a.H * a.W;
+
+    const float LOG2E = 1.4426950408889634f;
+    {
+    ScanEntry L = {0.f, 0.f, 0.f, 0.f, 0.f, -__builtin_inff(), 0.f, 0.f, 0.f, 0.f};
+    float rop = 0.f;
+    if (valid && !((GS_SCAN_SKIP & 32) && a.T > -1)) {
+        const uint32_t g = a.point_list[range.x + kit];
+        const float4* rp = a.rec + GS_REC_F4 * (size_t)g;
+        const float4 r0 = rp[0], r1 = rp[1], r2 = rp[2];
+        L.d0x = r0.x - (float)tx0; L.d0y = r0.y - (float)ty0;
+        L.hA = -0.5f * LOG2E * r0.z; L.nB = -LOG2E * r0.w; L.hC = -0.5f * LOG2E * r1.x;
+        L.lop = __builtin_amdgcn_logf(r1.y);
+        rop = r1.y > 0.f ? 1.0f / r1.y : 0.f;
+        L.cr = r1.z; L.cg = r1.w; L.cb = r2.x;
+        if constexpr (DEPTH) L.z = r2.y;
+    }
+    S.ent[SC_ENT_F4 * lane] = make_float4(L.d0x, L.d0y, L.hA, L.hC);
+    S.ent[SC_ENT_F4 * lane + 1] = make_float4(L.nB, L.lop, L.cr, L.cg);
+    S.ent[SC_ENT_F4 * lane + 2] = make_float4(L.cb, rop, __uint_as_float(slot), DEPTH ? L.z : 0.f);
+#pragma unroll
+    for (int k = 0; k < 9; k++) S.acc[9 * lane + k] = 0.f;
+    if constexpr (DEPTH) s_accz[lane] = 0.f;
+    }
+
+    float c099 = 0.99f;
+    asm volatile("" : "+v"(c099));
+
+    struct PixIn { uint64_t hm; float4 pf, ck; float g0, g1, g2, ckd, pfd, gd; };
+    auto load_pix = [&](int q) {
+        PixIn r;
+        const int pidx = q * 64 + lane;
+        r.hm = a.hit[(size_t)bucket * GS_TILE_PIX + pidx];
+        r.pf = a.pix_final[(size_t)tile * GS_TILE_PIX + pidx];
+        r.ck = a.ckpt[(size_t)bucket * GS_TILE_PIX + pidx];
+        const int px = tx0 + tile_pix_x(pidx), py = ty0 + tile_pix_y(pidx);
+        r.g0 = r.g1 = r.g2 = 0.f;
+        r.ckd = r.pfd = r.gd = 0.f;
+        if constexpr (DEPTH) { r.ckd = a.ckpt_depth[(size_t)bucket * GS_TILE_PIX + pidx]; r.pfd = a.pix_depth[(size_t)tile * GS_TILE_PIX + pidx]; }
+        if (px < a.W && py < a.H) {
+            const size_t pid = (size_t)py * a.W + px;
+            r.g0 = a.dL_dpix[pid]; r.g1 = a.dL_dpix[plane + pid]; r.g2 = a.dL_dpix[2 * plane + pid];
+            if constexpr (DEPTH) r.gd = a.dL_ddepth[pid];
+        }
+        return r;
+    };
+#ifndef GS_SCAN_PREFETCH
+#define GS_SCAN_PREFETCH 0
+#endif
+#if GS_SCAN_PREFETCH
+    PixIn nxt = load_pix(0);
+#endif
+    uint32_t any_lo = 0u, any_hi = 0u;
+    for (int q = 0; q < (((GS_SCAN_SKIP & 2) && a.T > -1) ? 0 : 4); q++) {
+#if GS_SCAN_PREFETCH
+        const PixIn cur = nxt;
+        if (q < 3) nxt = load_pix(q + 1);
+#else
+        const PixIn cur = load_pix(q);
+#endif
+        const int pidx = q * 64 + lane;
+        const uint64_t hm64 = cur.hm;
+        const int lx = tile_pix_x(pidx), ly = tile_pix_y(pidx);
+        const int px = tx0 + lx, py = ty0 + ly;
+        const float4 pf = cur.pf;
+        const bool active = px < a.W && py < a.H && __float_as_uint(pf.w) > bstart && hm64 != 0ull;
+        const uint64_t bal = __ballot(active);
+        if (bal == 0ull) continue;
+        const uint32_t mlo = active ? (uint32_t)hm64 : 0u, mhi = active ? (uint32_t)(hm64 >> 32) : 0u;
+        uint32_t S_lo[2], S_hi[2];
+        half_or(mlo, S_lo[0], S_lo[1]);
+        half_or(mhi, S_hi[0], S_hi[1]);
+        any_lo |= S_lo[0] | S_lo[1]; any_hi |= S_hi[0] | S_hi[1];
+        const uint32_t balh[2] = {(uint32_t)bal, (uint32_t)(bal >> 32)};
+        const int half = lane >> 5;
+        __builtin_amdgcn_fence(__ATOMIC_RELEASE, "wavefront");
+        __builtin_amdgcn_wave_barrier();
+        if (active) {
+            const float4 ck = cur.ck;
+            const float g0 = cur.g0, g1 = cur.g1, g2 = cur.g2;
+            float A0 = (ck.y - pf.x) * g0;
+            A0 = __builtin_fmaf(ck.z - pf.y, g1, A0);
+            A0 = __builtin_fmaf(ck.w - pf.z, g2, A0);
+            if constexpr (DEPTH) A0 = __builtin_fmaf(cur.ckd - cur.pfd, cur.gd, A0);
+            const uint32_t pos = half ? (uint32_t)SC_HALF + __builtin_amdgcn_mbcnt_hi(balh[1], 0u) : __builtin_amdgcn_mbcnt_lo(balh[0], 0u);
+            S.ta[pos] = make_float2(ck.x, A0);
+            S.rg[pos] = make_float2(g0, g1);
+            S.bx[pos] = make_float2(g2, (float)lx);
+            S.py[pos] = make_float2((float)ly, DEPTH ? cur.gd : 0.f);
+            S.hm[pos] = make_uint2(mlo, mhi);
+        }
+        if ((lane & 31) == 0) {
+            const int z = half * SC_HALF + __popc(half ? balh[1] : balh[0]);
+            S.ta[z] = S.rg[z] = S.bx[z] = S.py[z] = make_float2(0.f, 0.f);
+            S.hm[z] = make_uint2(0u, 0u);
+        }
+#pragma unroll
+        for (int h = 0; h < 2; h++) {
+            const bool mine = lane < 32 ? ((S_lo[h] >> lane) & 1u) : ((S_hi[h] >> (lane - 32)) & 1u);
+            const uint32_t k = __builtin_amdgcn_mbcnt_hi(S_hi[h], __builtin_amdgcn_mbcnt_lo(S_lo[h], 0u));
+            if (mine) S.list[64 * h + k] = (uint32_t)lane;
+        }
+        __builtin_amdgcn_fence(__ATOMIC_RELEASE, "wavefront");
+        __builtin_amdgcn_wave_barrier();
+        for (int h = 0; h < 2; h++) {
+            const int npx = __popc(h ? balh[1] : balh[0]);
+            if (npx == 0 || ((GS_SCAN_SKIP & 1) && a.T > -1)) continue;
+            const int ne = h ? __popc(S_lo[1]) + __popc(S_hi[1]) : __popc(S_lo[0]) + __popc(S_hi[0]);
+            switch ((ne + 15) >> 4) {
+            case 1: block_pass<1, DEPTH>(S, s_accz, lane, h * SC_HALF, 64 * h, npx, ne, c099); break;
+            case 2: block_pass<2, DEPTH>(S, s_accz, lane, h * SC_HALF, 64 * h, npx, ne, c099); break;
+            case 3: block_pass<3, DEPTH>(S, s_accz, lane, h * SC_HALF, 64 * h, npx, ne, c099); break;
+            default: block_pass<4, DEPTH>(S, s_accz, lane, h * SC_HALF, 64 * h, npx, ne, c099); break;
+            }
+        }
+    }
+    __builtin_amdgcn_fence(__ATOMIC_RELEASE, "wavefront");
+    __builtin_amdgcn_wave_barrier();
+
+#ifndef GS_SCAN_ZERO_ROWS
+#define GS_SCAN_ZERO_ROWS 0
+#endif
+    const bool blended = GS_SCAN_ZERO_ROWS || (lane < 32 ? ((any_lo >> lane) & 1u) : ((any_hi >> (lane - 32)) & 1u));
+    if (valid && !blended && !((GS_SCAN_SKIP & 8) && a.T > -1)) a.dead[slot] = 1;
+    if (valid && blended && !((GS_SCAN_SKIP & 16) && a.T > -1)) {
+        const float4 e0 = S.ent[SC_ENT_F4 * lane], e1 = S.ent[SC_ENT_F4 * lane + 1], e2 = S.ent[SC_ENT_F4 * lane + 2];
+        const ScanEntry L = {e0.x, e0.y, e0.z, e0.w, e1.x, e1.y, e1.z, e1.w, e2.x};
+        const float rop = e2.y;
+        const uint32_t slot = __float_as_uint(e2.z);
+        const float* s = S.acc + 9 * lane;
+        const float Sx = s[0], Sy = s[1], cxx = s[2], cxy = s[3], cyy = s[4], op = s[5], cr = s[6], cg = s[7], cb = s[8];
+        const float kx = 0.5f * (float)a.W / LOG2E, ky = 0.5f * (float)a.H / LOG2E;
+        const float gx = __builtin_fmaf(2.0f * L.hA, Sx, L.nB * Sy) * kx;
+        const float gy = __builtin_fmaf(2.0f * L.hC, Sy, L.nB * Sx) * ky;
+        float* o = a.partials + GS_PROW * (size_t)slot;
+        *reinterpret_cast<gs_v4f_u*>(o) = (gs_v4f_u){gx, gy, -0.5f * cxx, -0.5f * cxy};
+        *reinterpret_cast<gs_v4f_u*>(o + 4) = (gs_v4f_u){-0.5f * cyy, op * rop, cr, cg};
+        o[8] = cb;
+        if constexpr (DEPTH) a.partials_z[slot] = s_accz[lane];
+    }
diff --git a/gaussian-lic_amd/csrc/render_bwd_scan_common.h b/gaussian-lic_amd/csrc/render_bwd_scan_common.h
--- /dev/null
+++ b/gaussian-lic_amd/csrc/render_bwd_scan_common.h
@@ -0,0 +1,212 @@
+#pragma once
+#include "gslic_common.h"
+#include "kernels.h"
+#include <stdlib.h>
+
+#ifndef GS_SCAN_SKIP
+#define GS_SCAN_SKIP 0
+#endif
+
+namespace gslic {
+
+typedef float v2f_s __attribute__((ext_vector_type(2)));
+
+template <int CTRL, int ROW_MASK = 0xf>
+__device__ __forceinline__ float dpp_f(float old, float src)
+{
+    return __int_as_float(__builtin_amdgcn_update_dpp(__float_as_int(old), __float_as_int(src), CTRL, ROW_MASK, 0xf, false));
+}
+template <int CTRL, int ROW_MASK = 0xf>
+__device__ __forceinline__ uint32_t dpp_u(uint32_t old, uint32_t src)
+{
+    return (uint32_t)__builtin_amdgcn_update_dpp((int)old, (int)src, CTRL, ROW_MASK, 0xf, false);
+}
+#ifdef GS_SCAN_SAFE
+__device__ __forceinline__ float row_scan_mul(float x)
+{
+    const int i = lane_id() & 15;
+#pragma unroll
+    for (int d = 1; d < 16; d <<= 1) { const float o = __shfl_up(x, d, 16); if (i >= d) x *= o; }
+    return x;
+}
+__device__ __forceinline__ float row_scan_add(float x)
+{
+    const int i = lane_id() & 15;
+#pragma unroll
+    for (int d = 1; d < 16; d <<= 1) { const float o = __shfl_up(x, d, 16); if (i >= d) x += o; }
+    return x;
+}
+__device__ __forceinline__ float row_last(float x) { return __shfl(x, 15, 16); }
+__device__ __forceinline__ uint32_t wave_or(uint32_t v)
+{
+#pragma unroll
+    for (int d = 32; d >= 1; d >>= 1) v |= (uint32_t)__shfl_xor((int)v, d, 64);
+    return readlane_u(v, 0);
+}
+#else
+#ifndef GS_DPP_WAIT
+#define GS_DPP_WAIT "s_nop 1\n\t"
+#endif
+__device__ __forceinline__ float row_scan_mul(float x)
+{
+    asm(GS_DPP_WAIT "v_mul_f32_dpp %0, %0, %0 row_shr:1 row_mask:0xf bank_mask:0xf\n\t"
+        GS_DPP_WAIT "v_mul_f32_dpp %0, %0, %0 row_shr:2 row_mask:0xf bank_mask:0xf\n\t"
+        GS_DPP_WAIT "v_mul_f32_dpp %0, %0, %0 row_shr:4 row_mask:0xf bank_mask:0xf\n\t"
+        GS_DPP_WAIT "v_mul_f32_dpp %0, %0, %0 row_shr:8 row_mask:0xf bank_mask:0xf"
+        : "+v"(x));
+    return x;
+}
+__device__ __forceinline__ float row_scan_add(float x)
+{
+    asm(GS_DPP_WAIT "v_add_f32_dpp %0, %0, %0 row_shr:1 row_mask:0xf bank_mask:0xf\n\t"
+        GS_DPP_WAIT "v_add_f32_dpp %0, %0, %0 row_shr:2 row_mask:0xf bank_mask:0xf\n\t"
+        GS_DPP_WAIT "v_add_f32_dpp %0, %0, %0 row_shr:4 row_mask:0xf bank_mask:0xf\n\t"
+        GS_DPP_WAIT "v_add_f32_dpp %0, %0, %0 row_shr:8 row_mask:0xf bank_mask:0xf"
+        : "+v"(x));
+    return x;
+}
+__device__ __forceinline__ float row_last(float x) { return dpp_f<0x15f>(x, x); }
+__device__ __forceinline__ uint32_t wave_or(uint32_t v)
+{
+    v |= dpp_u<0x111>(0u, v);
+    v |= dpp_u<0x112>(0u, v);
+    v |= dpp_u<0x114>(0u, v);
+    v |= dpp_u<0x118>(0u, v);
+    v |= dpp_u<0x142, 0xa>(0u, v);
+    v |= dpp_u<0x143, 0xc>(0u, v);
+    return readlane_u(v, 63);
+}
+#endif
+
+__device__ __forceinline__ void half_or(uint32_t v, uint32_t& lo_half, uint32_t& hi_half)
+{
+#ifdef GS_SCAN_SAFE
+#pragma unroll
+    for (int d = 16; d >= 1; d >>= 1) v |= (uint32_t)__shfl_xor((int)v, d, 64);
+    lo_half = readlane_u(v, 0); hi_half = readlane_u(v, 32);
+#else
+    v |= dpp_u<0x111>(0u, v);
+    v |= dpp_u<0x112>(0u, v);
+    v |= dpp_u<0x114>(0u, v);
+    v |= dpp_u<0x118>(0u, v);
+    v |= dpp_u<0x142, 0xa>(0u, v);
+    lo_half = readlane_u(v, 31); hi_half = readlane_u(v, 63);
+#endif
+}
+
+struct ScanEntry {
+    float d0x, d0y;
+    float hA, hC, nB;
+    float lop;
+    float cr, cg, cb;
+    float z;
+};
+
+constexpr int SC_HALF = 32 + 1;
+constexpr int SC_NENT = 2 * SC_HALF;
+constexpr int SC_ENT_F4 = 3;
+
+struct ScanLds {
+    float4 ent[64 * SC_ENT_F4];
+    float acc[64 * 9];
+    uint32_t list[2 * 64];
+    float2 ta[SC_NENT], rg[SC_NENT], bx[SC_NENT], py[SC_NENT];
+    uint2 hm[SC_NENT];
+};
+
+template <int NG, bool DEPTH>
+__device__ __forceinline__ void block_pass(ScanLds& S, float* accz, const int lane, const int rb, const int lb, const int npx_, const int ne, float c099)
+{
+    const int npx = rb + npx_;
+    const int slot_i = lane & 15, row = lane >> 4;
+    ScanEntry E[NG];
+    uint32_t ent[NG], kbit[NG], klo[NG];
+    v2f_s acc_S[NG], acc_cxy[NG], acc_rg[NG];
+    float acc_cw[NG], acc_op[NG], acc_b[NG], acc_z[NG];
+#pragma unroll
+    for (int g = 0; g < NG; g++) {
+        acc_S[g] = acc_cxy[g] = acc_rg[g] = (v2f_s){0.f, 0.f};
+        acc_cw[g] = acc_op[g] = acc_b[g] = acc_z[g] = 0.f;
+        E[g] = {0.f, 0.f, 0.f, 0.f, 0.f, -__builtin_inff(), 0.f, 0.f, 0.f, 0.f};
+        ent[g] = 0u; kbit[g] = 0u; klo[g] = 0u;
+        const int k = 16 * g + slot_i;
+        if (k < ne) {
+            const uint32_t e = S.list[lb + k];
+            const float4 e0 = S.ent[SC_ENT_F4 * e], e1 = S.ent[SC_ENT_F4 * e + 1], e2 = S.ent[SC_ENT_F4 * e + 2];
+            E[g] = {e0.x, e0.y, e0.z, e0.w, e1.x, e1.y, e1.z, e1.w, e2.x, DEPTH ? e2.w : 0.f};
+            ent[g] = e; kbit[g] = e & 31u; klo[g] = e < 32u ? 0xffffffffu : 0u;
+        }
+    }
+    const int nchunk = ((GS_SCAN_SKIP & 4) && c099 > 0.f) ? 0 : (npx_ + 3) >> 2;
+    int off = rb + row;
+    for (int c = 0; c < nchunk; c++, off += 4) {
+        const int idx = off < npx ? off : npx;
+        const float2 ta = S.ta[idx], rg = S.rg[idx], bx = S.bx[idx], pyv = S.py[idx];
+        const uint2 hm = S.hm[idx];
+        float Tin = ta.x, Ain = ta.y;
+        const float pxf = bx.y, pyf = pyv.x, gD = pyv.y;
+#pragma unroll
+        for (int g = 0; g < NG; g++) {
+            const float dx = E[g].d0x - pxf, dy = E[g].d0y - pyf;
+            float p2 = __builtin_fmaf(__builtin_fmaf(E[g].hA, dx, E[g].nB * dy), dx, E[g].lop);
+            p2 = __builtin_fmaf(E[g].hC * dy, dy, p2);
+            const float araw = __builtin_amdgcn_exp2f(p2);
+            uint32_t sel_, m_;
+            asm("v_bfi_b32 %0, %1, %2, %3" : "=v"(sel_) : "v"(klo[g]), "v"(hm.x), "v"(hm.y));
+            asm("v_bfe_i32 %0, %1, %2, 1" : "=v"(m_) : "v"(sel_), "v"(kbit[g]));
+            const float ah = __uint_as_float(__float_as_uint(araw) & m_);
+            float alpha;
+            asm("v_min_f32 %0, %1, %2" : "=v"(alpha) : "v"(ah), "v"(c099));
+            const float om = 1.0f - alpha;
+            const float rinv = __builtin_amdgcn_rcpf(om);
+            const float Tincl = Tin * row_scan_mul(om);
+            const float Ti = Tincl * rinv;
+            const float Ta = Ti * alpha;
+            float cgd = E[g].cr * rg.x;
+            cgd = __builtin_fmaf(E[g].cg, rg.y, cgd);
+            cgd = __builtin_fmaf(E[g].cb, bx.x, cgd);
+            if constexpr (DEPTH) cgd = __builtin_fmaf(E[g].z, gD, cgd);
+            const float Ap = Ain + row_scan_add(Ta * cgd);
+            const float dLda = __builtin_fmaf(rinv, Ap, Ti * cgd);
+            const float w = ah * dLda;
+            acc_rg[g] = __builtin_elementwise_fma((v2f_s){Ta, Ta}, (v2f_s){rg.x, rg.y}, acc_rg[g]);
+            acc_b[g] = __builtin_fmaf(Ta, bx.x, acc_b[g]);
+            if constexpr (DEPTH) acc_z[g] = __builtin_fmaf(Ta, gD, acc_z[g]);
+            const v2f_s d = {dx, dy};
+            const v2f_s wd = (v2f_s){w, w} * d;
+            acc_S[g] += wd;
+            acc_cxy[g] = __builtin_elementwise_fma((v2f_s){wd.x, wd.x}, d, acc_cxy[g]);
+            acc_cw[g] = __builtin_fmaf(wd.y, dy, acc_cw[g]);
+            acc_op[g] += w;
+            if (g + 1 < NG) { Tin = row_last(Tincl); Ain = row_last(Ap); }
+        }
+    }
+#pragma unroll
+    for (int g = 0; g < NG; g++) {
+        float v[9] = {acc_S[g].x, acc_S[g].y, acc_cxy[g].x, acc_cxy[g].y, acc_cw[g], acc_op[g], acc_rg[g].x, acc_rg[g].y, acc_b[g]};
+#pragma unroll
+        for (int k = 0; k < 9; k++) {
+            v[k] += __shfl_xor(v[k], 16, 64);
+            v[k] += __shfl_xor(v[k], 32, 64);
+        }
+        if (row == 0 && 16 * g + slot_i < ne) {
+#pragma unroll
+            for (int k = 0; k < 9; k++) S.acc[9 * ent[g] + k] += v[k];
+        }
+        if constexpr (DEPTH) {
+            float vz = acc_z[g];
+            vz += __shfl_xor(vz, 16, 64);
+            vz += __shfl_xor(vz, 32, 64);
+            if (row == 0 && 16 * g + slot_i < ne) accz[ent[g]] += vz;
+        }
+    }
+}
+
+#ifndef GS_SCAN_WAVES
+#define GS_SCAN_WAVES 4
+#endif
+#ifndef GS_SCAN_WAVES_DEPTH
+#define GS_SCAN_WAVES_DEPTH GS_SCAN_WAVES
+#endif
+
+}
diff --git a/include/gslic_hip.h b/include/gslic_hip.h
--- a/include/gslic_hip.h
+++ b/include/gslic_hip.h
@@ -321,6 +321,8 @@
 
 int gslic_set_binning_mode(int32_t mode);
 
+int gslic_set_occluded_adam(int32_t on);
+
 #define GSLIC_BINNING_PATH_NONE 0
 #define GSLIC_BINNING_PATH_RADIX 1
 #define GSLIC_BINNING_PATH_ATOMIC 2
```
